# SKA-INAF/caesar-yolo

Measured on AMD Instinct MI355X. Metric: 512x512 tiles/sec over 16k x 16k FITS, higher is better.
Workload: dtype f16

## Files before the change

### caesar_yolo_amd/csrc/conv_igemm.hip

```cpp
#include "cy_kernels.h"
#include <cmath>
#include <cstdlib>
#include <cstring>
#include <vector>

namespace cy {

typedef _Float16 f16;
typedef f16 f16x8 __attribute__((ext_vector_type(8)));
typedef f16 f16x4 __attribute__((ext_vector_type(4)));
typedef float f32x4 __attribute__((ext_vector_type(4)));
typedef unsigned int u32x4 __attribute__((ext_vector_type(4)));
typedef unsigned int u32x2 __attribute__((ext_vector_type(2)));

#define CY_OOB 0xFFFFFF00u
#define CY_WAIT_VM(N) asm volatile("s_waitcnt vmcnt(%0)" ::"n"(N) : "memory")

#ifndef CY_STAMPS_ENABLED
#define CY_STAMPS_ENABLED 0
#endif
__device__ unsigned long long g_stamps[8];
constexpr int WG_STAMP_SLOTS = 4096;
__device__ unsigned long long g_wg_stamps[WG_STAMP_SLOTS * 4];
__device__ __forceinline__ unsigned long long stamp_now() {
// ... 955 lines not shown
            const unsigned off = poff[j] == CY_OOB ? CY_OOB : poff[j] + (unsigned)(ch * 128);
            char* dst = Pbuf + buf * P_BYTES + (wi < NWI ? wi : NWI) * 1024;
            __builtin_amdgcn_raw_ptr_buffer_load_lds(rs0, (lds_void*)dst, 16, off, 0, 0, 0);
        }
    };
    auto dma_w = [&](int n) {
        const int ch = n / 9, tap = n - ch * 9;
#pragma unroll
        for (int j = 0; j < WROUNDS; ++j) {
            const unsigned off = woff[j] + (unsigned)((ch * 9 + tap) * cpad * 128);
            char* dst = Wbuf + (n % RING) * W_BYTES + ((j * NW + wave) % WPIECES) * 1024;
            __builtin_amdgcn_raw_ptr_buffer_load_lds(rsw, (lds_void*)dst, 16, off, 0, 0, 0);
        }
    };

    f32x4 acc[NI][4];
#pragma unroll
    for (int ni = 0; ni < NI; ++ni)
#pragma unroll
        for (int mi = 0; mi < 4; ++mi) acc[ni][mi] = f32x4{0.f, 0.f, 0.f, 0.f};
    const int fr = lane & 15, fq = lane >> 4;
    f16x8 xa0[4], wb0[NI], xa1[4], wb1[NI];

    auto read_frags = [&](const char* P, const char* Wb, int kh, int kw, int kk, f16x8* xa, f16x8* wb) {
        const int qf = fq + 4 * kk;
#pragma unroll
        for (int mi = 0; mi < 4; ++mi) {
            const int r = (wm * 4 + mi + kh) * (TW + 2) + kw + fr;
            xa[mi] = *reinterpret_cast<const f16x8*>(P + r * 128 + ((qf ^ (r & 7)) << 4));
        }
#pragma unroll
        for (int ni = 0; ni < NI; ++ni) {
            const int r = wn * (NI * 16) + ni * 16 + fr;
            wb[ni] = *reinterpret_cast<const f16x8*>(Wb + r * 128 + ((qf ^ (r & 7)) << 4));
        }
    };
    auto mfma_all = [&](const f16x8* xa, const f16x8* wb) {
#pragma unroll
        for (int ni = 0; ni < NI; ++ni)
#pragma unroll
            for (int mi = 0; mi < 4; ++mi)
                acc[ni][mi] = __builtin_amdgcn_mfma_f32_16x16x32_f16(wb[ni], xa[mi], acc[ni][mi], 0, 0, 0);
    };

    dma_patch(0, 0);
    dma_w(0);
    if (total > 1) dma_w(1);
    CY_WAIT_VM(0);
    __builtin_amdgcn_s_barrier();
    if (grp == 1) __builtin_amdgcn_s_barrier();

    int it = 0;
#pragma unroll 1
    for (int ch = 0; ch < chunks; ++ch) {
        const char* P = Pbuf + (ch & 1) * P_BYTES;
#pragma unroll
        for (int tap = 0; tap < 9; ++tap, ++it) {
            const char* Wb = Wbuf + (it % RING) * W_BYTES;
            const int kh = tap / 3, kw = tap - kh * 3;
            const bool pre_p = tap == 1 && ch + 1 < chunks, pre_w = it + 2 < total;
            if (pre_w) dma_w(it + 2);
            if (pre_p) dma_patch((ch + 1) & 1, ch + 1);
            read_frags(P, Wb, kh, kw, 0, xa0, wb0);
            if (pre_p) { CY_WAIT_VM(WROUNDS + PROUNDS); }
            else if (pre_w) { CY_WAIT_VM(WROUNDS); }
            else { CY_WAIT_VM(0); }
            __builtin_amdgcn_sched_barrier(0);
            __builtin_amdgcn_s_barrier();
            read_frags(P, Wb, kh, kw, 1, xa1, wb1);
            __builtin_amdgcn_sched_barrier(0);
            if (a.dbg & 32) __builtin_amdgcn_s_setprio(1);
            mfma_all(xa0, wb0);
            asm volatile("s_waitcnt lgkmcnt(0)" ::: "memory");
            __builtin_amdgcn_sched_barrier(0);
            mfma_all(xa1, wb1);
            if (a.dbg & 32) __builtin_amdgcn_s_setprio(0);
            __builtin_amdgcn_sched_barrier(0);
            __builtin_amdgcn_s_barrier();
        }
    }
    if (grp == 0) __builtin_amdgcn_s_barrier();

    const int cbase = n0 + ((wn * NI) >> 2) * 64 + fq * 16 + ((wn * NI) & 3) * 4;
    float bv[NI * 4];
#pragma unroll
    for (int j = 0; j < NI * 4; ++j) bv[j] = a.bias[cbase + j];
#pragma unroll
    for (int mi = 0; mi < 4; ++mi) {
        const int y = y0 + wm * 4 + mi, x = x0 + fr;
        if (y >= H || x >= W) continue;
        const long pix = ((long)b * H + y) * W + x;
        float v[NI * 4];
#pragma unroll
        for (int ni = 0; ni < NI; ++ni)
#pragma unroll
            for (int j = 0; j < 4; ++j) {
                float t = acc[ni][mi][j] + bv[ni * 4 + j];
                if (a.act) t = silu_fast(t);
                v[ni * 4 + j] = t;
            }
        if (cbase + NI * 4 <= a.Cout) {
            f16* dst = reinterpret_cast<f16*>(a.out) + pix * a.out_ct + a.out_coff + cbase;
            if (a.res) {
                const f16* rp = reinterpret_cast<const f16*>(a.res) + pix * a.res_ct + a.res_coff + cbase;
#pragma unroll
                for (int h8 = 0; h8 < NI / 2; ++h8) {
                    const f16x8 rv = *reinterpret_cast<const f16x8*>(rp + 8 * h8);
#pragma unroll
                    for (int j = 0; j < 8; ++j) v[8 * h8 + j] += (float)rv[j];
                }
            }
#pragma unroll
            for (int h8 = 0; h8 < NI / 2; ++h8) {
                f16x8 o;
#pragma unroll
                for (int j = 0; j < 8; ++j) o[j] = (f16)v[8 * h8 + j];
                *reinterpret_cast<f16x8*>(dst + 8 * h8) = o;
            }
        } else {
#pragma unroll
            for (int j = 0; j < NI * 4; ++j) {
                const int c = cbase + j;
                if (c >= a.Cout) continue;
                float t = v[j];
                if (a.res) t += (float)(reinterpret_cast<const f16*>(a.res)[pix * a.res_ct + a.res_coff + c]);
                reinterpret_cast<f16*>(a.out)[pix * a.out_ct + a.out_coff + c] = (f16)t;
            }
        }
    }
}

template <int NI>
static hipError_t launch_pp(const ConvArgs& a, hipStream_t s) {
    constexpr int BN = 2 * NI * 16, PR = 18 * 18, NWI = (PR + 7) / 8;
    const size_t lds = 2 * (NWI + 1) * 1024 + 4 * BN * 128;
    static bool attr_set = false;
    if (!attr_set) {
        hipFuncSetAttribute(reinterpret_cast<const void*>(conv3x3_pp_kernel<NI>), hipFuncAttributeMaxDynamicSharedMemorySize, (int)lds);
        attr_set = true;
    }
    const int blocks = a.B * ((a.Hi + 15) / 16) * ((a.Wi + 15) / 16) * ((pad64(a.Cout) + BN - 1) / BN);
    hipLaunchKernelGGL((conv3x3_pp_kernel<NI>), dim3(blocks), dim3(512), lds, s, a);
    return hipGetLastError();
}

template <int KC, bool ACT, bool RES>
__global__ __launch_bounds__(512) void conv3x3_c64_kernel(const ConvArgs a) {
    constexpr int TH = 16, TW = 16, NG = 4, NI = 4;
    constexpr int RB = KC * 2, RPP = 1024 / RB, NCH = KC / 8, KK = KC / 32;
    constexpr int PR = (TH + 2) * (TW + 2), NWI = (PR + RPP - 1) / RPP, PROUNDS = (NWI + NG - 1) / NG;
    auto swz = [](int chunk, int row) { return KC == 64 ? (chunk ^ (row & 7)) : (chunk ^ (((row >> 2) & 1) << 1)); };
    constexpr int P_BYTES = (NWI + 1) * 1024;
    extern __shared__ __attribute__((aligned(16))) char smem[];
    typedef __attribute__((address_space(3))) void lds_void;
    const int tid = threadIdx.x, lane = tid & 63;
    const int wave = __builtin_amdgcn_readfirstlane(tid >> 6);
    const int grp = wave >> 2, wm = wave & 3;
    const int fr = lane & 15, fq = lane >> 4;
    const int H = a.Hi, W = a.Wi;
    const int tiles_x = (W + TW - 1) / TW, tiles_y = (H + TH - 1) / TH;
    const int npatch = a.B * tiles_y * tiles_x;
    const unsigned bias_bytes = (unsigned)((W + 1) * a.in0_ct) * 2u;
    const auto rs0 = __builtin_amdgcn_make_buffer_rsrc(const_cast<char*>(reinterpret_cast<const char*>(a.in0)) - bias_bytes, 0,
                                                       a.in0_bytes + 2 * bias_bytes, 0x00020000);

    constexpr int W_BYTES = 9 * 64 * RB, WPIECES = W_BYTES / 1024, PPT = 64 / RPP;
    char* const Wl = smem;
    char* const P = smem + W_BYTES + grp * P_BYTES;
    {
        const auto rsw = KC == 64 ? __builtin_amdgcn_make_buffer_rsrc(const_cast<void*>(a.wgt), 0, a.wgt_bytes, 0x00020000)
                                  : __builtin_amdgcn_make_buffer_rsrc(const_cast<void*>(a.wgt32), 0, a.wgt32_bytes, 0x00020000);
#pragma unroll
        for (int j = 0; j < (WPIECES + 7) / 8; ++j) {
            const int pc = j * 8 + wave;
            if (pc >= WPIECES) break;
            const int tap = pc / PPT, row = (pc % PPT) * RPP + lane / NCH;
            const int q = swz(lane % NCH, row);
            const unsigned off = (unsigned)((tap * 128 + row) * RB + q * 16);
            __builtin_amdgcn_raw_ptr_buffer_load_lds(rsw, (lds_void*)(Wl + pc * 1024), 16, off, 0, 0, 0);
        }
    }
    const int cbase = fq * 16;
    f32x2 bv[8];
#pragma unroll
    for (int j = 0; j < 8; ++j) bv[j] = f32x2{a.bias[cbase + 2 * j], a.bias[cbase + 2 * j + 1]};

    unsigned rel[PROUNDS];
#pragma unroll
    for (int j = 0; j < PROUNDS; ++j) {
        const int wi = j * NG + wm;
        const int r = wi * RPP + lane / NCH;
        const int ry = r / (TW + 2), rx = r - ry * (TW + 2);
        const int q = swz(lane % NCH, r);
        rel[j] = r < PR ? (unsigned)(((ry * W + rx) * a.in0_ct + q * 8) * 2) : CY_OOB;
    }
    const int rlane = lane / NCH;
    auto dma_patch = [&](int pidx) {
        const int tx = pidx % tiles_x, ty = (pidx / tiles_x) % tiles_y, b = pidx / (tiles_x * tiles_y);
        const int y0 = ty * TH, x0 = tx * TW;
        const unsigned so = bias_bytes + (unsigned)((((b * H + y0 - 1) * W + x0 - 1) * a.in0_ct + a.in0_coff) * 2);
        const bool interior = y0 >= 1 && x0 >= 1 && y0 + TH + 1 <= H && x0 + TW + 1 <= W;
        if (interior) {
#pragma unroll
            for (int j = 0; j < PROUNDS; ++j) {
                const int wi = j * NG + wm;
                dma_piece(rs0, (lds_ptr_t*)(P + (wi < NWI ? wi : NWI) * 1024), rel[j], so);
            }
        } else {
            const int ylo = y0 >= 1 ? 0 : 1, yhi = H - y0 + 1, xlo = x0 >= 1 ? 0 : 1, xhi = W - x0 + 1;
#pragma unroll
            for (int j = 0; j < PROUNDS; ++j) {
                const int wi = j * NG + wm;
                const int r = wi * RPP + rlane, ry = (r * 3641) >> 16, rx = r - ry * (TW + 2);
                const bool ok = ry >= ylo && ry < yhi && rx >= xlo && rx < xhi;
                dma_piece(rs0, (lds_ptr_t*)(P + (wi < NWI ? wi : NWI) * 1024), ok ? rel[j] : CY_OOB, so);
            }
        }
    };

    const int NP = (int)blockIdx.x < npatch ? (npatch - 1 - (int)blockIdx.x) / (int)gridDim.x + 1 : 0;
    if (grp < NP) dma_patch(blockIdx.x + grp * gridDim.x);
    __builtin_amdgcn_s_waitcnt(0x0F70);
    __builtin_amdgcn_s_barrier();

    const int R0 = wm * 4 * (TW + 2) + fr;
    unsigned xb[8], wb0[KK];
#pragma unroll
    for (int k8 = 0; k8 < 8; ++k8) xb[k8] = (unsigned)(R0 * RB + (swz(fq, (R0 + k8) & 7) << 4));
#pragma unroll
    for (int kk = 0; kk < KK; ++kk) wb0[kk] = (unsigned)(fr * RB + (swz(fq + 4 * kk, fr) << 4));
    f32x4 acc[NI][4];
    const bool vec_out = cbase + 16 <= a.Cout;
    const int out_lane = fr * a.out_ct + cbase, res_lane = fr * a.res_ct + cbase;
    for (int ph = 0; ph <= NP; ++ph) {
        if ((ph & 1) == grp) {
            if (ph < NP) {
#pragma unroll
                for (int ni = 0; ni < NI; ++ni)
#pragma unroll
                    for (int mi = 0; mi < 4; ++mi) acc[ni][mi] = f32x4{0.f, 0.f, 0.f, 0.f};
                f16x8 xa[2][4], wb[2][NI];
                auto load_group = [&](int g, f16x8* x, f16x8* w) {
                    const int tap = g / KK, kk = g % KK, kh = tap / 3, kw = tap - kh * 3;
#pragma unroll
                    for (int mi = 0; mi < 4; ++mi) {
                        const int c = (mi + kh) * (TW + 2) + kw;
                        x[mi] = *reinterpret_cast<const f16x8*>(P + xb[(c + 4 * kk) & 7] + c * RB);
                    }
#pragma unroll
                    for (int ni = 0; ni < NI; ++ni)
                        w[ni] = *reinterpret_cast<const f16x8*>(Wl + wb0[kk] + (tap * 64 + ni * 16) * RB);
                };
                load_group(0, xa[0], wb[0]);
#pragma unroll
                for (int g = 0; g < 9 * KK; ++g) {
                    if (g + 1 < 9 * KK) load_group(g + 1, xa[(g + 1) & 1], wb[(g + 1) & 1]);
                    __builtin_amdgcn_sched_barrier(0);
#pragma unroll
                    for (int ni = 0; ni < NI; ++ni)
#pragma unroll
                        for (int mi = 0; mi < 4; ++mi)
                            acc[ni][mi] = __builtin_amdgcn_mfma_f32_16x16x32_f16(wb[g & 1][ni], xa[g & 1][mi], acc[ni][mi], 0, 0, 0);
                    __builtin_amdgcn_sched_barrier(0);
                }
                asm volatile("s_waitcnt lgkmcnt(0)" ::: "memory");
            }
        } else if (ph >= 1) {
            f16x8 rres[4][2];
            const int pidx = blockIdx.x + (ph - 1) * gridDim.x;
            const int tx = pidx % tiles_x, ty = (pidx / tiles_x) % tiles_y, b = pidx / (tiles_x * tiles_y);
            const int yw = ty * TH + wm * 4, x = tx * TW + fr;
            const long rowpix = ((long)b * H + yw) * W + tx * TW;
            const bool xok = x < W;
            if (RES) {
#pragma unroll
                for (int mi = 0; mi < 4; ++mi) {
                    const bool ok = yw + mi < H && xok && vec_out;
                    const f16* rp = reinterpret_cast<const f16*>(a.res) + ((rowpix + (yw + mi < H ? (long)mi * W : 0)) * a.res_ct + a.res_coff) + (ok ? res_lane : 0);
                    rres[mi][0] = *reinterpret_cast<const f16x8*>(rp);
                    rres[mi][1] = *reinterpret_cast<const f16x8*>(rp + 8);
                }
            }
            if (ph + 1 < NP) dma_patch(blockIdx.x + (ph + 1) * gridDim.x);
            if (ACT) {
#pragma unroll
                for (int ni = 0; ni < NI; ++ni)
#pragma unroll
                    for (int mi = 0; mi < 4; ++mi)
#pragma unroll
                        for (int h = 0; h < 2; ++h) {
                            f32x2 t = f32x2{acc[ni][mi][2 * h], acc[ni][mi][2 * h + 1]} + bv[ni * 2 + h];
                            f32x2 e = t * f32x2{-1.44269504088896341f, -1.44269504088896341f};
                            e = f32x2{__builtin_amdgcn_exp2f(e[0]), __builtin_amdgcn_exp2f(e[1])} + f32x2{1.0f, 1.0f};
                            t = t * f32x2{__builtin_amdgcn_rcpf(e[0]), __builtin_amdgcn_rcpf(e[1])};
                            acc[ni][mi][2 * h] = t[0]; acc[ni][mi][2 * h + 1] = t[1];
                        }
            } else {
#pragma unroll
                for (int ni = 0; ni < NI; ++ni)
#pragma unroll
                    for (int mi = 0; mi < 4; ++mi)
#pragma unroll
                        for (int j = 0; j < 4; ++j) acc[ni][mi][j] += bv[ni * 2 + (j >> 1)][j & 1];
            }
#pragma unroll
            for (int mi = 0; mi < 4; ++mi) {
                if (yw + mi >= H) break;
                if (!xok) continue;
                if (vec_out) {
                    f16* dst = reinterpret_cast<f16*>(a.out) + ((rowpix + (long)mi * W) * a.out_ct + a.out_coff) + out_lane;
                    float v[16];
#pragma unroll
                    for (int ni = 0; ni < NI; ++ni)
#pragma unroll
                        for (int j = 0; j < 4; ++j) v[ni * 4 + j] = acc[ni][mi][j];
                    if (RES) {
#pragma unroll
                        for (int j = 0; j < 8; ++j) { v[j] += (float)rres[mi][0][j]; v[8 + j] += (float)rres[mi][1][j]; }
                    }
                    f16x8 o0, o1;
#pragma unroll
                    for (int j = 0; j < 8; ++j) { o0[j] = (f16)v[j]; o1[j] = (f16)v[8 + j]; }
                    *reinterpret_cast<f16x8*>(dst) = o0;
                    *reinterpret_cast<f16x8*>(dst + 8) = o1;
                } else {
                    const long pix = rowpix + (long)mi * W + fr;
#pragma unroll
                    for (int j = 0; j < 16; ++j) {
                        const int c = cbase + j;
                        if (c >= a.Cout) continue;
                        float t = acc[j >> 2][mi][j & 3];
                        if (RES) t += (float)(reinterpret_cast<const f16*>(a.res)[pix * a.res_ct + a.res_coff + c]);
                        reinterpret_cast<f16*>(a.out)[pix * a.out_ct + a.out_coff + c] = (f16)t;
                    }
                }
            }
            CY_WAIT_VM(0);
        }
        __builtin_amdgcn_sched_barrier(0);
        __builtin_amdgcn_s_barrier();
        __builtin_amdgcn_sched_barrier(0);
    }
}

template <int KC>
static hipError_t launch_c64(const ConvArgs& a, hipStream_t s) {
    constexpr int RPP = 1024 / (KC * 2), NWI = (18 * 18 + RPP - 1) / RPP;
    const size_t lds = 9 * 64 * KC * 2 + 2 * (NWI + 1) * 1024;
    static bool attr_set = false;
    if (!attr_set) {
        hipFuncSetAttribute(reinterpret_cast<const void*>(conv3x3_c64_kernel<KC, true, false>), hipFuncAttributeMaxDynamicSharedMemorySize, (int)lds);
        hipFuncSetAttribute(reinterpret_cast<const void*>(conv3x3_c64_kernel<KC, true, true>), hipFuncAttributeMaxDynamicSharedMemorySize, (int)lds);
        hipFuncSetAttribute(reinterpret_cast<const void*>(conv3x3_c64_kernel<KC, false, false>), hipFuncAttributeMaxDynamicSharedMemorySize, (int)lds);
        hipFuncSetAttribute(reinterpret_cast<const void*>(conv3x3_c64_kernel<KC, false, true>), hipFuncAttributeMaxDynamicSharedMemorySize, (int)lds);
        attr_set = true;
    }
    const int npatch = a.B * ((a.Hi + 15) / 16) * ((a.Wi + 15) / 16);
    const int grid = npatch < 256 ? npatch : 256;
    if (a.act && a.res) hipLaunchKernelGGL((conv3x3_c64_kernel<KC, true, true>), dim3(grid), dim3(512), lds, s, a);
    else if (a.act) hipLaunchKernelGGL((conv3x3_c64_kernel<KC, true, false>), dim3(grid), dim3(512), lds, s, a);
    else if (a.res) hipLaunchKernelGGL((conv3x3_c64_kernel<KC, false, true>), dim3(grid), dim3(512), lds, s, a);
    else hipLaunchKernelGGL((conv3x3_c64_kernel<KC, false, false>), dim3(grid), dim3(512), lds, s, a);
    return hipGetLastError();
}

__global__ __launch_bounds__(512) void conv3x3_halo2_kernel(const ConvArgs a) {
    constexpr int TH = 16, TW = 16, NW = 8, BN = 128;
    constexpr int PR = (TH + 2) * (TW + 2), NWI = (PR + 7) / 8, PROUNDS = (NWI + NW - 1) / NW;
    constexpr int P_BYTES = PROUNDS * NW * 1024, SLAB = BN * 128, W_BYTES = 2 * SLAB;
    extern __shared__ __attribute__((aligned(16))) char smem[];
    char* const Pbuf = smem;
    char* const Wbuf = smem + 2 * P_BYTES;
    typedef __attribute__((address_space(3))) void lds_void;
    const int tid = threadIdx.x, lane = tid & 63;
    const int wave = __builtin_amdgcn_readfirstlane(tid >> 6);
    const int wm = wave >> 1, wn = wave & 1;
    const int H = a.Hi, W = a.Wi;
    const int tiles_x = (W + TW - 1) / TW, tiles_y = (H + TH - 1) / TH;
    const int cpad = pad128(a.Cout);
    const int ntn = (pad64(a.Cout) + BN - 1) / BN;
    const int id = xcd_remap(blockIdx.x, gridDim.x);
    const int nt = id % ntn;
    int rest = id / ntn;
    const int tx = rest % tiles_x; rest /= tiles_x;
    const int ty = rest % tiles_y;
    const int b = rest / tiles_y;
    const int y0 = ty * TH, x0 = tx * TW, n0 = nt * BN;
    const int chunks = a.Cin / 64, pairs = chunks / 2;

    const auto rs0 = __builtin_amdgcn_make_buffer_rsrc(const_cast<void*>(a.in0), 0, a.in0_bytes, 0x00020000);
    const auto rsw = __builtin_amdgcn_make_buffer_rsrc(const_cast<void*>(a.wgt), 0, a.wgt_bytes, 0x00020000);
    unsigned poff[PROUNDS];
#pragma unroll
    for (int j = 0; j < PROUNDS; ++j) {
        const int r = (j * NW + wave) * 8 + (lane >> 3);
        const int ry = r / (TW + 2), rx = r - ry * (TW + 2);
        const int y = y0 + ry - 1, x = x0 + rx - 1;
        const int q = (lane & 7) ^ (r & 7);
        const bool ok = r < PR && (unsigned)y < (unsigned)H && (unsigned)x < (unsigned)W;
        poff[j] = ok ? (unsigned)(((b * H + y) * W + x) * a.in0_ct + a.in0_coff + q * 8) * 2u : CY_OOB;
    }
    unsigned woff[2];
#pragma unroll
    for (int j = 0; j < 2; ++j) {
        const int row = (j * NW + wave) * 8 + (lane >> 3);
        woff[j] = (unsigned)((n0 + row) * 128 + ((lane & 7) ^ (row & 7)) * 16);
    }
    auto dma_patch = [&](int buf, int ch) {
#pragma unroll
        for (int j = 0; j < PROUNDS; ++j) {
            __builtin_amdgcn_raw_ptr_buffer_load_lds(rs0, (lds_void*)(Pbuf + buf * P_BYTES + (j * NW + wave) * 1024), 16, poff[j], ch * 128, 0, 0);
        }
    };
    auto dma_slab = [&](int buf, int t, int ch, int tap) {
#pragma unroll
        for (int j = 0; j < 2; ++j) {
            __builtin_amdgcn_raw_ptr_buffer_load_lds(rsw, (lds_void*)(Wbuf + buf * W_BYTES + t * SLAB + (j * NW + wave) * 1024), 16, woff[j], (ch * 9 + tap) * cpad * 128, 0, 0);
        }
    };
    f32x4 acc[4][4];
#pragma unroll
    for (int ni = 0; ni < 4; ++ni)
#pragma unroll
        for (int mi = 0; mi < 4; ++mi) acc[ni][mi] = f32x4{0.f, 0.f, 0.f, 0.f};
    const int fr = lane & 15, fq = lane >> 4;
    auto compute = [&](const char* P, const char* Wb, int kh, int kw) {
#pragma unroll
        for (int kk = 0; kk < 2; ++kk) {
            const int qf = fq + 4 * kk;
            f16x8 xa[4], wb[4];
#pragma unroll
            for (int mi = 0; mi < 4; ++mi) {
                const int r = (wm * 4 + mi + kh) * (TW + 2) + kw + fr;
                xa[mi] = *reinterpret_cast<const f16x8*>(P + r * 128 + ((qf ^ (r & 7)) << 4));
            }
#pragma unroll
            for (int ni = 0; ni < 4; ++ni) {
                const int r = wn * 64 + ni * 16 + fr;
                wb[ni] = *reinterpret_cast<const f16x8*>(Wb + r * 128 + ((qf ^ (r & 7)) << 4));
            }
#pragma unroll
            for (int ni = 0; ni < 4; ++ni)
#pragma unroll
                for (int mi = 0; mi < 4; ++mi)
                    acc[ni][mi] = __builtin_amdgcn_mfma_f32_16x16x32_f16(wb[ni], xa[mi], acc[ni][mi], 0, 0, 0);
        }
    };

    dma_patch(0, 0);
    dma_slab(0, 0, 0, 0);
    dma_slab(0, 1, 0, 1);
    __syncthreads();
    int g = 0;
    const bool stamps = CY_STAMPS_ENABLED && (a.dbg & 64) != 0;
    unsigned long long acc_dma = 0, acc_cmp = 0, acc_wait = 0, acc_bar = 0;
    const unsigned long long t_begin = stamps ? stamp_now() : 0;
    unsigned long long t0s = t_begin;
#pragma unroll 1
    for (int cp = 0; cp < pairs; ++cp) {
#pragma unroll
        for (int st = 0; st < 9; ++st, ++g) {
            if (st < 8) {
                const int u0 = 2 * (st + 1), u1 = u0 + 1;
                dma_slab((g + 1) & 1, 0, 2 * cp + u0 / 9, u0 % 9);
                dma_slab((g + 1) & 1, 1, 2 * cp + u1 / 9, u1 % 9);
            } else if (cp + 1 < pairs) {
                dma_slab((g + 1) & 1, 0, 2 * cp + 2, 0);
                dma_slab((g + 1) & 1, 1, 2 * cp + 2, 1);
            }
            if (st == 0) dma_patch(1, 2 * cp + 1);
            if (st == 5 && cp + 1 < pairs) dma_patch(0, 2 * cp + 2);
            unsigned long long t1 = 0, t2 = 0, t3 = 0;
            if (stamps) { __builtin_amdgcn_sched_barrier(0); t1 = stamp_now(); __builtin_amdgcn_sched_barrier(0); }
#pragma unroll
            for (int t = 0; t < 2; ++t) {
                const int u = 2 * st + t, tap = u % 9;
                compute(Pbuf + (u / 9) * P_BYTES, Wbuf + (g & 1) * W_BYTES + t * SLAB, tap / 3, tap % 3);
            }
            if (stamps) {
                asm volatile("s_waitcnt lgkmcnt(0)" ::: "memory");
                __builtin_amdgcn_sched_barrier(0); t2 = stamp_now(); __builtin_amdgcn_sched_barrier(0);
                CY_WAIT_VM(0);
                __builtin_amdgcn_sched_barrier(0); t3 = stamp_now(); __builtin_amdgcn_sched_barrier(0);
            }
            __syncthreads();
            if (stamps) {
                __builtin_amdgcn_sched_barrier(0);
                const unsigned long long t4 = stamp_now();
                acc_dma += t1 - t0s; acc_cmp += t2 - t1; acc_wait += t3 - t2; acc_bar += t4 - t3;
                t0s = t4;
            }
        }
    }

    if (stamps && lane == 0) {
        const unsigned long long t_end = stamp_now();
        atomicAdd(&g_stamps[0], acc_dma); atomicAdd(&g_stamps[1], acc_cmp); atomicAdd(&g_stamps[2], acc_wait);
        atomicAdd(&g_stamps[3], acc_bar); atomicAdd(&g_stamps[4], t_end - t_begin); atomicAdd(&g_stamps[5], (unsigned long long)(pairs * 9));
        atomicAdd(&g_stamps[6], 1ull);
    }
    const int cbase = n0 + wn * 64 + fq * 16;
    float bv[16];
#pragma unroll
    for (int j = 0; j < 16; ++j) bv[j] = a.bias[cbase + j];
#pragma unroll
    for (int mi = 0; mi < 4; ++mi) {
        const int y = y0 + wm * 4 + mi, x = x0 + fr;
        if (y >= H || x >= W) continue;
        const long pix = ((long)b * H + y) * W + x;
// ... 293 lines not shown
    for (int mi = 0; mi < MIW; ++mi) {
        const int y = y0 + wm * RPW + (mi >> 1), x = DUAL ? fr : x0 + (mi & 1) * 16 + fr;
        const int bb = DUAL ? 2 * b + (mi & 1) : b;
        if (y >= H || x >= W || bb >= a.B) continue;
        const long pix = ((long)bb * H + y) * W + x;
        float v[16];
        bias_act16(acc[0][mi], acc[1][mi], acc[2][mi], acc[3][mi], bv, a.act != 0, v);
        if (cbase + 16 <= a.Cout) {
            f16* dst = reinterpret_cast<f16*>(a.out) + pix * a.out_ct + a.out_coff + cbase;
            if (res_vec) {
#pragma unroll
                for (int j = 0; j < 8; ++j) { v[j] += (float)rv[mi][0][j]; v[8 + j] += (float)rv[mi][1][j]; }
            }
            f16x8 o0, o1;
#pragma unroll
            for (int j = 0; j < 8; ++j) { o0[j] = (f16)v[j]; o1[j] = (f16)v[8 + j]; }
            *reinterpret_cast<f16x8*>(dst) = o0;
            *reinterpret_cast<f16x8*>(dst + 8) = o1;
        } else {
#pragma unroll
            for (int j = 0; j < 16; ++j) {
                const int c = cbase + j;
                if (c >= a.Cout) continue;
                float t = v[j];
                if (a.res) t += (float)(reinterpret_cast<const f16*>(a.res)[pix * a.res_ct + a.res_coff + c]);
                reinterpret_cast<f16*>(a.out)[pix * a.out_ct + a.out_coff + c] = (f16)t;
            }
        }
    }
    }
    if (stamps) {
        const unsigned long long t_st = stamp_real();
        asm volatile("s_waitcnt vmcnt(0)" ::: "memory");
        const unsigned long long t_end = stamp_real();
        if (tid == 0) {
            unsigned long long* rec = g_wg_stamps + (size_t)(blockIdx.x % WG_STAMP_SLOTS) * 4;
            rec[0] = t_loop - t_entry; rec[1] = t_epi - t_loop; rec[2] = t_st - t_epi; rec[3] = c_epi - c_loop;
        }
    }
}

template <int WN, bool DUAL = false, bool SPLIT = false>
static hipError_t launch_wide(const ConvArgs& a, hipStream_t s) {
    constexpr int PR = 18 * (DUAL ? 36 : 34), NPC = (PR + 15) / 16, PROUNDS = (NPC + 7) / 8, BN = 64 * WN;
    const size_t lds = 2 * PROUNDS * 8 * 1024 + 3 * 2 * BN * 64 + 1024;
    static bool attr_set = false;
    if (!attr_set) {
        hipFuncSetAttribute(reinterpret_cast<const void*>(conv3x3_wide_kernel<true, WN, DUAL, 2, SPLIT>), hipFuncAttributeMaxDynamicSharedMemorySize, (int)lds);
        attr_set = true;
    }
    const int bx = DUAL ? (a.B + 1) / 2 : a.B * ((a.Wi + 31) / 32);
    const int blocks = bx * ((a.Hi + 15) / 16) * ((pad64(a.Cout) + BN - 1) / BN);
    hipLaunchKernelGGL((conv3x3_wide_kernel<true, WN, DUAL, 2, SPLIT>), dim3(blocks), dim3(512), lds, s, a);
    return hipGetLastError();
}

struct StripGeo { int RS, IS, NE; unsigned long long mRS, mIS; };
__device__ __forceinline__ int strip_div(int e, unsigned long long m) { return (int)(((unsigned long long)(unsigned)e * m) >> 40); }

template <bool SPLIT, bool RES, int STRIP = 0>
__global__ __launch_bounds__(512) void conv3x3_widep_kernel(const ConvArgs a, const int total, const StripGeo sg) {
    constexpr int NST = 9, TH = 16, TW = 32, NW = 8, BN = 128, PWID = TW + 2;
    constexpr int NDW = 4;
    constexpr int RPW = 4, MIW = 8, WPS = 2 * (NW / NDW);
    constexpr int PR = (TH + 2) * PWID, NPC = (PR + 15) / 16, PROUNDS = STRIP ? STRIP : (NPC + NDW - 1) / NDW;
    constexpr int P_BYTES = PROUNDS * NDW * 1024, SLAB = BN * 64, W_BYTES = 2 * SLAB, RING = 3;
    extern __shared__ __attribute__((aligned(16))) char smem[];
    char* const Pbuf = smem;
    char* const Wbuf = smem + 2 * P_BYTES;
    const int tid = threadIdx.x, lane = tid & 63;
    const int wave = __builtin_amdgcn_readfirstlane(tid >> 6);
    const int wm = wave >> 1, wn = wave & 1;
    const int H = a.Hi, W = a.Wi;
    const int tiles_x = (W + TW - 1) / TW, tiles_y = (H + TH - 1) / TH;
    const int cpad = pad128(a.Cout);
    const int ntn = (pad64(a.Cout) + BN - 1) / BN;
    const int ppairs = a.Cin / 64;
    const int pairs = SPLIT ? a.split * ppairs : ppairs;
    const auto rs0 = __builtin_amdgcn_make_buffer_rsrc(const_cast<void*>(a.in0), 0, a.in0_bytes, 0x00020000);
    const auto rsw = __builtin_amdgcn_make_buffer_rsrc(const_cast<void*>(a.wgt32), 0, a.wgt32_bytes, 0x00020000);
    const auto rsb = __builtin_amdgcn_make_buffer_rsrc(const_cast<float*>(a.bias), 0, (unsigned)pad64(a.Cout) * 4u, 0x00020000);
    const auto rss = __builtin_amdgcn_make_buffer_rsrc(const_cast<float*>(SPLIT ? a.oscale : a.bias), 0, (unsigned)pad64(a.Cout) * 4u, 0x00020000);
    const unsigned out_bytes = (unsigned)((long)a.B * H * W * a.out_ct * 2);
    const auto rso = __builtin_amdgcn_make_buffer_rsrc(a.out, 0, out_bytes, 0x00020000);
    const auto rsr = __builtin_amdgcn_make_buffer_rsrc(const_cast<void*>(RES ? a.res : a.in0), 0,
                                                       RES ? (unsigned)((long)a.B * H * W * a.res_ct * 2) : 0u, 0x00020000);
    const int fr = lane & 15, fq = lane >> 4;

    int pb_, py0, px0, pn0;
    auto geometry = [&](int v) {
        const int id = xcd_remap(v, total);
        pn0 = (id % ntn) * BN;
        int rest = id / ntn;
        if constexpr (STRIP != 0) { px0 = rest * 512; py0 = 0; pb_ = 0; return; }
        px0 = (rest % tiles_x) * TW; rest /= tiles_x;
        py0 = (rest % tiles_y) * TH;
        pb_ = rest / tiles_y;
    };
    const bool no_dma = CY_STAMPS_ENABLED && (a.dbg & 1), no_rd = CY_STAMPS_ENABLED && (a.dbg & 2), no_mma = CY_STAMPS_ENABLED && (a.dbg & 4);
    const bool dmaw = wave < NDW && !no_dma;
    auto dma_patch = [&](int buf, int slab, int gb, int gy0, int gx0) {
        if (!dmaw) return;
        int l4 = lane >> 2;
        asm volatile("" : "+v"(l4));
        const unsigned lq = (unsigned)(lane & 3);
        unsigned slab_so = (unsigned)slab * 64u;
        if constexpr (SPLIT) {
            int lo;
            slab_so = (unsigned)x3_chunk(slab, 2 * ppairs, lo) * 64u;
            if (lo) slab_so += (unsigned)a.in0_lo * 2u;
        }
        if constexpr (STRIP != 0) {
            const int hl = 514 + 2 * sg.RS;
#pragma unroll
            for (int j = 0; j < PROUNDS; ++j) {
                const int le = (j * NDW + wave) * 16 + l4;
                const int e = gx0 - sg.RS - 1 + le;
                const bool in = le < hl && (unsigned)e < (unsigned)sg.NE;
                const int ec = in ? e : 0;
                const int bb = strip_div(ec, sg.mIS), r = ec - bb * sg.IS;
                const int y = strip_div(r, sg.mRS), x = r - y * sg.RS;
                const unsigned q = lq ^ (unsigned)(((le >> 2) & 1) << 1);
                const bool ok = in && y < H && x < W;
                const unsigned off = ok ? (unsigned)(((bb * H + y) * W + x) * a.in0_ct + a.in0_coff + (int)q * 8) * 2u : CY_OOB;
                dma_piece(rs0, (lds_ptr_t*)(Pbuf + buf * P_BYTES + (j * NDW + wave) * 1024), off, slab_so);
            }
            return;
        }
#pragma unroll
        for (int j = 0; j < PROUNDS; ++j) {
            const int r = (j * NDW + wave) * 16 + l4;
            const int ry = (r * 1928) >> 16, rx = r - ry * PWID;
            const int y = gy0 + ry - 1, x = gx0 + rx - 1;
            const unsigned q = lq ^ (unsigned)(((r >> 2) & 1) << 1);
            const bool ok = r < PR && (unsigned)y < (unsigned)H && (unsigned)x < (unsigned)W;
            const unsigned off = ok ? (unsigned)(((gb * H + y) * W + x) * a.in0_ct + a.in0_coff + (int)q * 8) * 2u : CY_OOB;
            dma_piece(rs0, (lds_ptr_t*)(Pbuf + buf * P_BYTES + (j * NDW + wave) * 1024), off, slab_so);
        }
    };
    unsigned woff = 0;
    auto weight_lane_offset = [&]() { const int row = wave * 32 + (lane >> 2); woff = (unsigned)(row * 64 + ((lane & 3) ^ (((row >> 2) & 1) << 1)) * 16); };
    auto dma_stage = [&](int ring, int slab0, int u0, int n0) {
        if (!dmaw) return;
#pragma unroll
        for (int t = 0; t < 2; ++t) {
            const int u = u0 + t, sl = slab0 + u / 9, tap = u % 9;
#pragma unroll
            for (int h = 0; h < 2; ++h)
                dma_piece(rsw, (lds_ptr_t*)(Wbuf + ring * W_BYTES + t * SLAB + (wave * 2 + h) * 1024), woff,
                          (unsigned)((sl * 9 + tap) * cpad * 64 + n0 * 64 + h * 1024));
        }
    };
    float* const bias_lds = reinterpret_cast<float*>(smem + 2 * P_BYTES + RING * W_BYTES);
    auto dma_bias = [&](int slot, int n0) {
        if (wave != 0) return;
        dma_piece(rsb, (lds_ptr_t*)(bias_lds + slot * 512), lane * 16 < BN * 4 ? (unsigned)(n0 * 4 + lane * 16) : CY_OOB, 0);
        if constexpr (SPLIT) dma_piece(rss, (lds_ptr_t*)(bias_lds + slot * 512 + 256), lane * 16 < BN * 4 ? (unsigned)(n0 * 4 + lane * 16) : CY_OOB, 0);
    };

    f32x4 acc[4][MIW];
    unsigned pb[STRIP ? 9 : 8], wl = 0;
    const int rw0 = wm * RPW * PWID;
    auto fragment_bases = [&]() {
        int lz = lane;
        asm volatile("" : "+v"(lz));
        const int r_ = lz & 15, q_ = lz >> 4;
        if constexpr (STRIP != 0) {
#pragma unroll
            for (int t = 0; t < 9; ++t) {
                const int R0 = (t / 3) * sg.RS + (t % 3) + wm * 128 + r_;
                pb[t] = (unsigned)(R0 * 64 + ((q_ ^ (((R0 >> 2) & 1) << 1)) << 4));
            }
        } else {
#pragma unroll
            for (int c = 0; c < 8; ++c)
                pb[c] = (unsigned)(rw0 * 64 + r_ * 64 + ((q_ ^ ((((c + r_ + (rw0 & 7)) >> 2) & 1) << 1)) << 4));
        }
        wl = (unsigned)(2 * P_BYTES + (wn * 64 + r_) * 64 + ((q_ ^ (((r_ >> 2) & 1) << 1)) << 4));
    };
    f16x8 xa[2][4], wb[2][4];
    auto load_x = [&](f16x8* dst, int pbuf_off, int kh, int kw, int half) {
        if (no_rd) return;
#pragma unroll
        for (int m = 0; m < 4; ++m) {
            const int mi = half * 4 + m;
            if constexpr (STRIP != 0) {
                dst[m] = *reinterpret_cast<const f16x8*>(smem + pb[kh * 3 + kw] + (pbuf_off + mi * 1024));
            } else {
                const int base = ((mi >> 1) + kh) * PWID + (mi & 1) * 16 + kw;
                dst[m] = *reinterpret_cast<const f16x8*>(smem + pb[base & 7] + (pbuf_off + base * 64));
            }
        }
    };
    auto load_w = [&](f16x8* dst, int wbuf_off) {
        if (no_rd) return;
#pragma unroll
        for (int ni = 0; ni < 4; ++ni) dst[ni] = *reinterpret_cast<const f16x8*>(smem + wl + (wbuf_off + ni * 1024));
    };
    auto mma = [&](const f16x8* w, const f16x8* x, int half) {
        if (no_mma) return;
#pragma unroll
        for (int ni = 0; ni < 4; ++ni)
#pragma unroll
            for (int m = 0; m < 4; ++m)
                acc[ni][half * 4 + m] = __builtin_amdgcn_mfma_f32_16x16x32_f16(w[ni], x[m], acc[ni][half * 4 + m], 0, 0, 0);
    };
    auto stage_compute = [&](int st) {
        const int u0 = 2 * st, u1 = u0 + 1, t0 = u0 % 9, t1 = u1 % 9;
        const int p0 = (u0 / 9) * P_BYTES, p1 = (u1 / 9) * P_BYTES, w0 = (st % 3) * W_BYTES, w1 = w0 + SLAB;
        load_w(wb[0], w0);
        load_x(xa[0], p0, t0 / 3, t0 % 3, 0);
        load_x(xa[1], p0, t0 / 3, t0 % 3, 1);
        mma(wb[0], xa[0], 0);
        __builtin_amdgcn_sched_barrier(0);
        load_w(wb[1], w1);
        load_x(xa[0], p1, t1 / 3, t1 % 3, 0);
        mma(wb[0], xa[1], 1);
        __builtin_amdgcn_sched_barrier(0);
        load_x(xa[1], p1, t1 / 3, t1 % 3, 1);
        mma(wb[1], xa[0], 0);
        __builtin_amdgcn_sched_barrier(0);
    };

    const bool stamps = CY_STAMPS_ENABLED && (a.dbg & 64) != 0;
    unsigned long long t_l0 = 0, t_l1 = 0, t_rw = 0, t_ep = 0;
    const unsigned long long t_begin = stamps ? stamp_real() : 0;
    int v = blockIdx.x, n = 0;
    if (v >= total) return;
    geometry(v);
    weight_lane_offset();
    dma_bias(0, pn0);
    dma_patch(0, 0, pb_, py0, px0);
    dma_stage(0, 0, 0, pn0);
    dma_stage(1, 0, 2, pn0);
    CY_WAIT_VM(WPS);
    __builtin_amdgcn_s_barrier();
#pragma unroll 1
    for (;;) {
        const int b = pb_, y0 = py0, x0 = px0, n0 = pn0;
        const int vn = v + (int)gridDim.x;
        const bool next = vn < total;
        if (stamps) {
            const unsigned long long t = stamp_real();
            if (n == 2 && tid == 0) {
                unsigned long long* rec = g_wg_stamps + (size_t)(blockIdx.x % WG_STAMP_SLOTS) * 4;
                rec[0] = t_rw - t_l1; rec[1] = t_l1 - t_l0; rec[2] = t_ep - t_rw;
            }
            t_l0 = t;
        }
        fragment_bases();
#pragma unroll
        for (int ni = 0; ni < 4; ++ni)
#pragma unroll
            for (int mi = 0; mi < MIW; ++mi) acc[ni][mi] = f32x4{0.f, 0.f, 0.f, 0.f};
#pragma unroll 1
        for (int cp = 0; cp < pairs; ++cp) {
            const bool more = cp + 1 < pairs;
            const bool chain = more || next;
#pragma unroll
            for (int st = 0; st < NST; ++st) {
                const bool has_w = st + 2 < NST || chain;
                if (st + 2 < NST) dma_stage((st + 2) % 3, 2 * cp, 2 * (st + 2), n0);
                else if (more) dma_stage((st + 2) % 3, 2 * cp + 2, 2 * (st + 2 - NST), n0);
                else if (next) dma_stage((st + 2) % 3, 0, 2 * (st + 2 - NST), pn0);
                if (st == 0) dma_patch(1, 2 * cp + 1, b, y0, x0);
                if (st == 1 && !more && next) { geometry(vn); dma_bias((n + 1) & 1, pn0); }
                if (st == 5 && more) dma_patch(0, 2 * cp + 2, b, y0, x0);
                if (st == 5 && !more && next) dma_patch(0, 0, pb_, py0, px0);
                stage_compute(st);
                asm volatile("s_waitcnt lgkmcnt(0)" ::: "memory");
                if (st == 0 || st == 1) { CY_WAIT_VM(WPS + PROUNDS); }
                else if (st == 5 || st == 6) { if (chain) { CY_WAIT_VM(WPS + PROUNDS); } else { CY_WAIT_VM(WPS); } }
                else if (has_w) { CY_WAIT_VM(WPS); }
                else { CY_WAIT_VM(0); }
                __builtin_amdgcn_sched_barrier(0);
                __builtin_amdgcn_s_barrier();
                __builtin_amdgcn_sched_barrier(0);
                mma(wb[1], xa[1], 1);
            }
        }
        if (stamps) t_l1 = stamp_real();
        const float* bl = bias_lds + (n & 1) * 512 + wn * 64 + fq * 16;
        float bv[16];
        if constexpr (!SPLIT) {
#pragma unroll
            for (int j = 0; j < 4; ++j) {
                const f32x4 t = *reinterpret_cast<const f32x4*>(bl + j * 4);
                bv[j * 4] = t[0]; bv[j * 4 + 1] = t[1]; bv[j * 4 + 2] = t[2]; bv[j * 4 + 3] = t[3];
            }
        }
        const int cbase = n0 + wn * 64 + fq * 16;
        const bool chan_ok = cbase + 16 <= a.Cout;
        const int xl = x0 + fr;
        const unsigned pix0 = (unsigned)((b * H + y0 + wm * RPW) * W + xl);
        const bool okx0 = xl < W && chan_ok, okx1 = xl + 16 < W && chan_ok;
        const unsigned cb2 = (unsigned)cbase * 2u;
        const int e0 = x0 + wm * 128 + fr;
        auto pixel = [&](int mi, unsigned& pix) -> bool {
            if constexpr (STRIP != 0) {
                const int e = e0 + 16 * mi;
                const int ec = e < sg.NE ? e : 0;
                const int bb = strip_div(ec, sg.mIS), r = ec - bb * sg.IS;
                const int yy = strip_div(r, sg.mRS), xx = r - yy * sg.RS;
                pix = (unsigned)((bb * H + yy) * W + xx);
                return e < sg.NE && yy < H && xx < W && chan_ok;
            } else {
                pix = pix0 + (unsigned)((mi >> 1) * W + (mi & 1) * 16);
                return (y0 + wm * RPW + (mi >> 1) < H) && ((mi & 1) ? okx1 : okx0);
            }
        };
        if constexpr (SPLIT) {
            f16x8 rq[3][4];
            auto res_load = [&](int mi) {
                unsigned pix;
                const bool ok = pixel(mi, pix);
                const unsigned ro = ok ? (pix * (unsigned)a.res_ct + (unsigned)a.res_coff) * 2u + cb2 : CY_OOB;
                rq[mi % 3][0] = __builtin_bit_cast(f16x8, load_b128(rsr, ro, 0));
                rq[mi % 3][1] = __builtin_bit_cast(f16x8, load_b128(rsr, ro, 16));
                rq[mi % 3][2] = __builtin_bit_cast(f16x8, load_b128(rsr, ro, a.res_lo * 2));
                rq[mi % 3][3] = __builtin_bit_cast(f16x8, load_b128(rsr, ro, a.res_lo * 2 + 16));
            };
            if (RES) { res_load(0); res_load(1); }
            if (stamps) t_rw = stamp_real();
#pragma unroll
            for (int mi = 0; mi < MIW; ++mi) {
                if (RES && mi + 2 < MIW) res_load(mi + 2);
                float bg[16], sc[16];
#pragma unroll
                for (int j = 0; j < 4; ++j) {
                    const f32x4 t = *reinterpret_cast<const f32x4*>(bl + j * 4), u = *reinterpret_cast<const f32x4*>(bl + 256 + j * 4);
                    bg[j * 4] = t[0]; bg[j * 4 + 1] = t[1]; bg[j * 4 + 2] = t[2]; bg[j * 4 + 3] = t[3];
                    sc[j * 4] = u[0]; sc[j * 4 + 1] = u[1]; sc[j * 4 + 2] = u[2]; sc[j * 4 + 3] = u[3];
                }
                float vv[16];
                scale_bias_act16(acc[0][mi], acc[1][mi], acc[2][mi], acc[3][mi], bg, sc, a.act != 0, vv);
                if (RES) {
#pragma unroll
                    for (int j = 0; j < 8; ++j) {
                        vv[j] += (float)rq[mi % 3][0][j] + (float)rq[mi % 3][2][j];
                        vv[8 + j] += (float)rq[mi % 3][1][j] + (float)rq[mi % 3][3][j];
                    }
                }
                f16x8 h0, h1, l0, l1;
#pragma unroll
                for (int j = 0; j < 8; ++j) {
                    h0[j] = (f16)vv[j]; h1[j] = (f16)vv[8 + j];
                    l0[j] = (f16)(vv[j] - (float)h0[j]); l1[j] = (f16)(vv[8 + j] - (float)h1[j]);
                }
                unsigned pix;
                const bool ok = pixel(mi, pix);
                const unsigned so = ok ? (pix * (unsigned)a.out_ct + (unsigned)a.out_coff) * 2u + cb2 : CY_OOB;
                __builtin_amdgcn_raw_buffer_store_b128(__builtin_bit_cast(u32x4, h0), rso, so, 0, 0);
                __builtin_amdgcn_raw_buffer_store_b128(__builtin_bit_cast(u32x4, h1), rso, so, 16, 0);
                __builtin_amdgcn_raw_buffer_store_b128(__builtin_bit_cast(u32x4, l0), rso, so, a.out_lo * 2, 0);
                __builtin_amdgcn_raw_buffer_store_b128(__builtin_bit_cast(u32x4, l1), rso, so, a.out_lo * 2 + 16, 0);
            }
        } else {
        f16x8 rv[MIW][2];
        if (RES) {
#pragma unroll
            for (int mi = 0; mi < MIW; ++mi) {
                unsigned pix;
                const bool ok = pixel(mi, pix);
                const unsigned ro = ok ? (pix * (unsigned)a.res_ct + (unsigned)a.res_coff) * 2u + cb2 : CY_OOB;
                rv[mi][0] = __builtin_bit_cast(f16x8, load_b128(rsr, ro, 0));
                rv[mi][1] = __builtin_bit_cast(f16x8, load_b128(rsr, ro, 16));
            }
            CY_WAIT_VM(0);
        }
        if (stamps) t_rw = stamp_real();
#pragma unroll
        for (int mi = 0; mi < MIW; ++mi) {
            float vv[16];
            bias_act16(acc[0][mi], acc[1][mi], acc[2][mi], acc[3][mi], bv, a.act != 0, vv);
            if (RES) {
#pragma unroll
                for (int j = 0; j < 8; ++j) { vv[j] += (float)rv[mi][0][j]; vv[8 + j] += (float)rv[mi][1][j]; }
            }
            f16x8 o0, o1;
#pragma unroll
            for (int j = 0; j < 8; ++j) { o0[j] = (f16)vv[j]; o1[j] = (f16)vv[8 + j]; }
            unsigned pix;
            const bool ok = pixel(mi, pix);
            const unsigned so = ok ? (pix * (unsigned)a.out_ct + (unsigned)a.out_coff) * 2u + cb2 : CY_OOB;
            __builtin_amdgcn_raw_buffer_store_b128(__builtin_bit_cast(u32x4, o0), rso, so, 0, 0);
            __builtin_amdgcn_raw_buffer_store_b128(__builtin_bit_cast(u32x4, o1), rso, so, 16, 0);
        }
        }
        if (stamps) t_ep = stamp_real();
        if (stamps && !next && tid == 0) g_wg_stamps[(size_t)(blockIdx.x % WG_STAMP_SLOTS) * 4 + 3] = t_ep - t_begin;
        if (!next) break;
        v = vn; ++n;
    }
}

template <int STRIP, bool SPLIT = false>
static hipError_t launch_widep_t(const ConvArgs& a, hipStream_t s, int total, const StripGeo& sg) {
    constexpr int PR = 18 * 34, NPC = (PR + 15) / 16, PROUNDS = STRIP ? STRIP : (NPC + 3) / 4;
    const size_t lds = 2 * PROUNDS * 4 * 1024 + 3 * 2 * 128 * 64 + 4096;
    static bool attr_set = false;
    if (!attr_set) {
        hipFuncSetAttribute(reinterpret_cast<const void*>(conv3x3_widep_kernel<SPLIT, false, STRIP>), hipFuncAttributeMaxDynamicSharedMemorySize, (int)lds);
        hipFuncSetAttribute(reinterpret_cast<const void*>(conv3x3_widep_kernel<SPLIT, true, STRIP>), hipFuncAttributeMaxDynamicSharedMemorySize, (int)lds);
        attr_set = true;
    }
    static const int ncu = [] { int dev = 0, n = 256; hipGetDevice(&dev); hipDeviceGetAttribute(&n, hipDeviceAttributeMultiprocessorCount, dev); return n > 0 ? n : 256; }();
    const int grid = total < ncu ? total : ncu;
    if (a.res) hipLaunchKernelGGL((conv3x3_widep_kernel<SPLIT, true, STRIP>), dim3(grid), dim3(512), lds, s, a, total, sg);
    else hipLaunchKernelGGL((conv3x3_widep_kernel<SPLIT, false, STRIP>), dim3(grid), dim3(512), lds, s, a, total, sg);
    return hipGetLastError();
}

static hipError_t launch_widep(const ConvArgs& a, hipStream_t s) {
    const int total = a.B * ((a.Wi + 31) / 32) * ((a.Hi + 15) / 16) * ((pad64(a.Cout) + 127) / 128);
    return a.split ? launch_widep_t<0, true>(a, s, total, StripGeo{}) : launch_widep_t<0>(a, s, total, StripGeo{});
}

static double wide2d_cover(int H, int W) { return (double)((H + 15) / 16 * 16) * ((W + 31) / 32 * 32) / ((double)H * W); }
static double strip_cover(int H, int W) { return (double)(H + 1) * (W + 1) / ((double)H * W); }
static bool strip_small(const ConvArgs& a) { return a.Wi >= 3 && a.Wi <= 12 && a.Hi >= 3 && a.Hi <= 126; }
static bool strip_fits(const ConvArgs& a) {
    return ((a.Wi >= 17 && a.Hi >= 17 && a.Wi <= 126) || strip_small(a)) && a.Cout % 16 == 0 && (long)a.B * (a.Hi + 1) * (a.Wi + 1) < (1L << 22);
}

static hipError_t launch_strip(const ConvArgs& a, hipStream_t s) {
    StripGeo sg;
    sg.RS = a.Wi + 1; sg.IS = (a.Hi + 1) * sg.RS; sg.NE = a.B * sg.IS;
    sg.mRS = ((1ull << 40) + sg.RS - 1) / sg.RS; sg.mIS = ((1ull << 40) + sg.IS - 1) / sg.IS;
    const int total = ((sg.NE + 511) / 512) * ((pad64(a.Cout) + 127) / 128);
    if (a.split) return a.Wi <= 62 ? launch_widep_t<10, true>(a, s, total, sg) : launch_widep_t<12, true>(a, s, total, sg);
    return a.Wi <= 62 ? launch_widep_t<10>(a, s, total, sg) : launch_widep_t<12>(a, s, total, sg);
}

template <int NB, int MI, int RING, bool K3, bool SPLIT = false, int NDW = 8, bool FUSE2 = false>
__global__ __launch_bounds__(512, (NB * MI <= 4 && RING == 2) ? 2 : 1) void conv1x1_direct_kernel(const ConvArgs a) {
    static_assert(!FUSE2 || (NB == 4 && !SPLIT), "back-to-back fusion: 256-channel tile, fp16 context");
    constexpr int NW = 8, BN = 64 * NB, BM = NW * MI * 16, W_BYTES = BN * 128, DIST = RING - 1;
    constexpr int WPW = BN / 8 / NDW, APW = 2 * MI, PER = WPW + APW;
    extern __shared__ __attribute__((aligned(16))) char smem[];
    const bool stamps = CY_STAMPS_ENABLED && (a.dbg & 64) != 0;
    const unsigned long long t_entry = stamps ? stamp_real() : 0;
    typedef __attribute__((address_space(3))) void lds_void;
    const int tid = threadIdx.x, lane = tid & 63;
    const int wave = __builtin_amdgcn_readfirstlane(tid >> 6);
    const int fr = lane & 15, fq = lane >> 4;
    const int HoWo = a.Ho * a.Wo, M = a.B * HoWo;
    const int cpad = pad128(a.Cout);
    const int ntn = (pad64(a.Cout) + BN - 1) / BN;
    const int id = xcd_remap(blockIdx.x, gridDim.x);
    const int m0 = (id / ntn) * BM, n0 = (id % ntn) * BN;
    constexpr int taps = K3 ? 9 : 1, pad = K3 ? 1 : 0, kk3 = K3 ? 3 : 1;
    const int pchunks = (a.Cin / 64) * taps, c0chunks = a.c1 ? a.c0 / 64 : pchunks;
    const int chunks = SPLIT ? a.split * pchunks : pchunks;
    const unsigned bias_bytes = K3 ? (unsigned)((a.Wi + 1) * a.in0_ct) * 2u : 0u;

    const auto rs0 = __builtin_amdgcn_make_buffer_rsrc(const_cast<char*>(reinterpret_cast<const char*>(a.in0)) - bias_bytes, 0,
                                                       a.in0_bytes + 2 * bias_bytes, 0x00020000);
    const auto rs1 = __builtin_amdgcn_make_buffer_rsrc(const_cast<void*>(a.c1 ? a.in1 : a.in0), 0,
                                                       a.c1 ? a.in1_bytes : a.in0_bytes, 0x00020000);
    const auto rsw = __builtin_amdgcn_make_buffer_rsrc(const_cast<void*>(a.wgt), 0, a.wgt_bytes, 0x00020000);
    unsigned v0[MI], v1[MI], vmask[MI];
#pragma unroll
    for (int mi = 0; mi < MI; ++mi) {
        const int m = m0 + (wave * MI + mi) * 16 + fr;
        v0[mi] = v1[mi] = CY_OOB;
        vmask[mi] = 0;
        if (m < M) {
            const int b = m / HoWo, r = m - b * HoWo, ho = r / a.Wo, wo = r - ho * a.Wo;
            int p0;
            if (a.up0) p0 = (b * (a.Hi >> 1) + (ho >> 1)) * (a.Wi >> 1) + (wo >> 1);
            else p0 = (b * a.Hi + ho * a.s) * a.Wi + wo * a.s;
            v0[mi] = (unsigned)(p0 * a.in0_ct + a.in0_coff + fq * 8) * 2u;
            v1[mi] = (unsigned)(m * a.in1_ct + a.in1_coff + fq * 8) * 2u;
            unsigned vm = 0;
#pragma unroll
            for (int kh = 0; kh < kk3; ++kh)
#pragma unroll
                for (int kw = 0; kw < kk3; ++kw)
                    if ((unsigned)(ho * a.s + kh - pad) < (unsigned)a.Hi && (unsigned)(wo * a.s + kw - pad) < (unsigned)a.Wi)
                        vm |= 1u << (kh * kk3 + kw);
            vmask[mi] = vm;
        }
    }
    const bool no_dma = CY_STAMPS_ENABLED && (a.dbg & 1), no_rd = CY_STAMPS_ENABLED && (a.dbg & 2), no_mma = CY_STAMPS_ENABLED && (a.dbg & 4),
               no_px = CY_STAMPS_ENABLED && (a.dbg & 8);
    const bool reqw = wave < NDW;
    const unsigned woff0 = (unsigned)((n0 + wave * 8 + (lane >> 3)) * 128 + ((lane & 7) ^ (lane >> 3)) * 16);
    u32x4 xa[RING][MI][2];
    int ltap = 0, lslab = 0;
    auto load_a = [&](int slot, int cv) {
        if (no_px) return;
        int lo = 0;
        const int c = SPLIT ? x3_chunk(cv, pchunks, lo) : cv;
        const unsigned lo0 = SPLIT && lo ? (unsigned)a.in0_lo * 2u : 0u, lo1 = SPLIT && lo ? (unsigned)a.in1_lo * 2u : 0u;
        if (c >= c0chunks) {
#pragma unroll
            for (int mi = 0; mi < MI; ++mi)
#pragma unroll
                for (int kk = 0; kk < 2; ++kk)
                    xa[slot][mi][kk] = load_b128(rs1, v1[mi], ((c - c0chunks) * 64 + kk * 32) * 2 + lo1);
        } else if constexpr (!K3) {
#pragma unroll
            for (int mi = 0; mi < MI; ++mi)
#pragma unroll
                for (int kk = 0; kk < 2; ++kk)
                    xa[slot][mi][kk] = load_b128(rs0, v0[mi], (c * 64 + kk * 32) * 2 + lo0);
        } else {
            const int kh = ltap / 3, kw = ltap - kh * 3;
            const unsigned so = bias_bytes + (unsigned)((((kh - 1) * a.Wi + (kw - 1)) * a.in0_ct + lslab * 64) * 2) + lo0;
#pragma unroll
            for (int mi = 0; mi < MI; ++mi) {
                const unsigned vo = ((vmask[mi] >> ltap) & 1u) ? v0[mi] : CY_OOB;
#pragma unroll
                for (int kk = 0; kk < 2; ++kk) xa[slot][mi][kk] = load_b128(rs0, vo, so + kk * 64);
            }
            if (++ltap == 9) { ltap = 0; ++lslab; if (SPLIT && lslab * 9 == pchunks) lslab = 0; }
        }
    };
    auto dma_w = [&](int slot, int c) {
        if ((NDW < NW && !reqw) || no_dma) return;
#pragma unroll
        for (int j = 0; j < WPW; ++j)
            dma_piece(rsw, (lds_ptr_t*)(smem + slot * W_BYTES + (j * NDW + wave) * 1024), woff0, c * cpad * 128 + j * NDW * 1024);
    };
    auto wait_w = [&](int n) {
        if (NDW < NW && !reqw) return;
        if (n == APW + 2 * PER) { CY_WAIT_VM(APW + 2 * PER); }
        else if (n == APW + PER) { CY_WAIT_VM(APW + PER); }
        else { CY_WAIT_VM(APW); }
    };
    f32x4 acc[NB * 4][MI];
#pragma unroll
    for (int ni = 0; ni < NB * 4; ++ni)
#pragma unroll
        for (int mi = 0; mi < MI; ++mi) acc[ni][mi] = f32x4{0.f, 0.f, 0.f, 0.f};
    auto compute_x = [&](int slot, const u32x4 (&xs)[MI][2]) {
        const char* Wb = smem + slot * W_BYTES;
        f16x8 wb[2][4];
        auto load_wb = [&](f16x8* dst, int gi) {
            if (no_rd) return;
            const int kk = gi / NB, g = gi % NB, qf = fq + 4 * kk;
#pragma unroll
            for (int ni = 0; ni < 4; ++ni) {
                const int r = g * 64 + ni * 16 + fr;
                dst[ni] = *reinterpret_cast<const f16x8*>(Wb + r * 128 + ((qf ^ (r & 7)) << 4));
            }
        };
        load_wb(wb[0], 0);
#pragma unroll
        for (int gi = 0; gi < 2 * NB; ++gi) {
            const int kk = gi / NB, g = gi % NB;
            if (gi + 1 < 2 * NB) load_wb(wb[(gi + 1) & 1], gi + 1);
// ... 767 lines not shown
            if (n < cout && k < 27) { const int tap = k / 3, c = k % 3; v = W[((size_t)n * 3 + c) * 9 + tap]; }
            o[row * 32 + k] = (f16)v;
        }
    }
}

constexpr int SD_TH = 8, SD_TW = 32, SD_PH = 2 * SD_TH + 1, SD_PW = 2 * SD_TW + 1, SD_EVEN = SD_TW + 1;
constexpr int SD_ROWS = SD_PH * SD_PW, SD_FRAGS = (SD_ROWS + 15) / 16, SD_LDS = SD_FRAGS * 16 * 128;

__device__ __forceinline__ u32x2 load_b64(__amdgpu_buffer_rsrc_t rs, unsigned voff) {
    return __builtin_amdgcn_raw_buffer_load_b64(rs, voff, 0, 0);
}

__global__ __launch_bounds__(512) void stem_down_kernel(const StemDownArgs a) {
    extern __shared__ __attribute__((aligned(16))) char smem[];
    const int tid = threadIdx.x, lane = tid & 63, fr = lane & 15, fq = lane >> 4;
    const int wave = __builtin_amdgcn_readfirstlane(tid >> 6);
    const int wn = wave & 1, wm = wave >> 1;
    const int tiles_x = (a.Wo + SD_TW - 1) / SD_TW, tiles_y = (a.Ho + SD_TH - 1) / SD_TH;
    int id = xcd_remap(blockIdx.x, gridDim.x);
    const int tx = id % tiles_x; id /= tiles_x;
    const int ty = id % tiles_y;
    const int b = id / tiles_y;
    const int oy0 = ty * SD_TH, ox0 = tx * SD_TW;
    const int sy0 = 2 * oy0 - 1, sx0 = 2 * ox0 - 1;
    const auto rsi = __builtin_amdgcn_make_buffer_rsrc(const_cast<void*>(a.in), 0, a.in_bytes, 0x00020000);
    const auto rsw = __builtin_amdgcn_make_buffer_rsrc(const_cast<void*>(a.wgt32), 0, a.wgt32_bytes, 0x00020000);

    constexpr int SD_RING = 4;
    f16x8 wa[SD_RING][4];
    const unsigned wl = (unsigned)((wn * 64 + fr) * 64 + fq * 16);
    auto load_wa = [&](f16x8* dst, int step) {
        const int h = step & 1, tap = step >> 1;
#pragma unroll
        for (int ni = 0; ni < 4; ++ni) dst[ni] = __builtin_bit_cast(f16x8, load_b128(rsw, wl + ni * 1024, (h * 9 + tap) * 8192));
    };
#pragma unroll
    for (int st = 0; st < SD_RING - 1; ++st) load_wa(wa[st], st);

    if (!(a.dbg & 1)) {
        const f16* wp = reinterpret_cast<const f16*>(a.wpk2);
        f16x8 sw0[4], sw1[4];
#pragma unroll
        for (int ni = 0; ni < 4; ++ni) {
            sw0[ni] = *reinterpret_cast<const f16x8*>(wp + (ni * 16 + fr) * 64 + fq * 8);
            sw1[ni] = *reinterpret_cast<const f16x8*>(wp + (ni * 16 + fr) * 64 + 32 + fq * 8);
        }
        float bv[16];
#pragma unroll
        for (int j = 0; j < 16; ++j) bv[j] = a.bias0[fq * 16 + j];
        const int t0 = 2 * fq, t1 = 2 * fq + 1;
        const int dh0 = t0 / 3 - 1, dw0 = t0 % 3 - 1, dh1 = t1 / 3 - 1, dw1 = t1 % 3 - 1;
        const int d0 = (dh0 * a.Wi + dw0) * 8, d1 = (dh1 * a.Wi + dw1) * 8, d2 = (a.Wi + 1) * 8;
        constexpr int NG = (SD_FRAGS + 7) / 8;
        u32x2 q0[NG], q1[NG], q2[NG];
        unsigned inmask = 0;
#pragma unroll
        for (int gi = 0; gi < NG; ++gi) {
            const int g = gi * 8 + wave, p = g * 16 + fr;
            const int sy = p / SD_PW, q = p - sy * SD_PW;
            const int sx = q < SD_EVEN ? 2 * q : 2 * (q - SD_EVEN) + 1;
            const int Y = sy0 + sy, X = sx0 + sx;
            const bool inmap = p < SD_ROWS && (unsigned)Y < (unsigned)a.H1 && (unsigned)X < (unsigned)a.W1;
            inmask |= inmap ? (1u << gi) : 0u;
            const int hc = 2 * Y, wc = 2 * X;
            const int base = ((b * a.Hi + hc) * a.Wi + wc) * 8;
            const bool ok0 = inmap && ((hc + dh0) | (wc + dw0)) >= 0, ok1 = inmap && ((hc + dh1) | (wc + dw1)) >= 0;
            q0[gi] = load_b64(rsi, ok0 ? (unsigned)(base + d0) : CY_OOB);
            q1[gi] = load_b64(rsi, ok1 ? (unsigned)(base + d1) : CY_OOB);
            q2[gi] = load_b64(rsi, (inmap && fq == 0) ? (unsigned)(base + d2) : CY_OOB);
        }
#pragma unroll
        for (int gi = 0; gi < NG; ++gi) {
            const int g = gi * 8 + wave;
            if (g >= SD_FRAGS) break;
            const int p = g * 16 + fr;
            const bool inmap = (inmask >> gi) & 1u;
            const u32x4 u0 = {q0[gi].x, q0[gi].y & 0xFFFFu, q1[gi].x, q1[gi].y & 0xFFFFu};
            const u32x4 u1 = {q2[gi].x, q2[gi].y & 0xFFFFu, 0u, 0u};
            const f16x8 x0 = __builtin_bit_cast(f16x8, u0), x1 = __builtin_bit_cast(f16x8, u1);
            f32x4 acc[4];
#pragma unroll
            for (int ni = 0; ni < 4; ++ni) {
                acc[ni] = __builtin_amdgcn_mfma_f32_16x16x32_f16(sw0[ni], x0, f32x4{0.f, 0.f, 0.f, 0.f}, 0, 0, 0);
                acc[ni] = __builtin_amdgcn_mfma_f32_16x16x32_f16(sw1[ni], x1, acc[ni], 0, 0, 0);
            }
            f16x8 o0, o1;
            float v16[16];
            bias_act16(acc[0], acc[1], acc[2], acc[3], bv, true, v16);
#pragma unroll
            for (int j = 0; j < 8; ++j) { o0[j] = (f16)v16[j]; o1[j] = (f16)v16[8 + j]; }
            const unsigned keep = inmap ? 0xFFFFFFFFu : 0u;
            const u32x4 k4 = {keep, keep, keep, keep};
            char* row = smem + p * 128;
            *reinterpret_cast<u32x4*>(row + (((2 * fq) ^ (p & 7)) << 4)) = __builtin_bit_cast(u32x4, o0) & k4;
            *reinterpret_cast<u32x4*>(row + (((2 * fq + 1) ^ (p & 7)) << 4)) = __builtin_bit_cast(u32x4, o1) & k4;
        }
    }
    __syncthreads();

    f32x4 acc[4][4];
#pragma unroll
    for (int ni = 0; ni < 4; ++ni)
#pragma unroll
        for (int m = 0; m < 4; ++m) acc[ni][m] = f32x4{0.f, 0.f, 0.f, 0.f};
    const int pl = wm * 4 * SD_PW + fr;
    if (!(a.dbg & 2))
#pragma unroll
    for (int step = 0; step < 18; ++step) {
        const int tap = step >> 1, h = step & 1, kh = tap / 3, kw = tap % 3;
        if (step + SD_RING - 1 < 18) load_wa(wa[(step + SD_RING - 1) % SD_RING], step + SD_RING - 1);
        __builtin_amdgcn_sched_barrier(0);
        f16x8 xb[4];
#pragma unroll
        for (int m = 0; m < 4; ++m) {
            const int cm = (2 * (m >> 1) + kh) * SD_PW + (m & 1) * 16 + (kw == 1 ? SD_EVEN : (kw == 2 ? 1 : 0));
            const int p = pl + cm;
            xb[m] = *reinterpret_cast<const f16x8*>(smem + p * 128 + (((h * 4 + fq) ^ (p & 7)) << 4));
        }
#pragma unroll
        for (int ni = 0; ni < 4; ++ni)
#pragma unroll
            for (int m = 0; m < 4; ++m)
                acc[ni][m] = __builtin_amdgcn_mfma_f32_16x16x32_f16(wa[step % SD_RING][ni], xb[m], acc[ni][m], 0, 0, 0);
        __builtin_amdgcn_sched_barrier(0);
    }

    const int cbase = wn * 64 + fq * 16;
    float bv[16];
#pragma unroll
    for (int j = 0; j < 16; ++j) bv[j] = a.bias1[cbase + j];
#pragma unroll
    for (int m = 0; m < 4; ++m) {
        const int oy = oy0 + wm * 2 + (m >> 1), ox = ox0 + (m & 1) * 16 + fr;
        if (oy >= a.Ho || ox >= a.Wo || (a.dbg & 4)) continue;
        const long pix = ((long)b * a.Ho + oy) * a.Wo + ox;
        f16x8 o0, o1;
        float v16[16];
        bias_act16(acc[0][m], acc[1][m], acc[2][m], acc[3][m], bv, true, v16);
#pragma unroll
        for (int j = 0; j < 8; ++j) { o0[j] = (f16)v16[j]; o1[j] = (f16)v16[8 + j]; }
        f16* dst = reinterpret_cast<f16*>(a.out) + pix * a.out_ct + a.out_coff + cbase;
        *reinterpret_cast<f16x8*>(dst) = o0;
        *reinterpret_cast<f16x8*>(dst + 8) = o1;
    }
}

constexpr int S2_TH = 8, S2_TW = 16, S2_PH = 2 * S2_TH + 1, S2_PW = 2 * S2_TW + 1, S2_EVEN = S2_TW + 1;
constexpr int S2_ROWS = S2_PH * S2_PW, S2_FRAGS = (S2_ROWS + 15) / 16, S2_BUF = S2_FRAGS * 16 * 128, S2_LDS = 2 * S2_BUF;
static_assert(S2_FRAGS % 4 == 0, "fragments split evenly over the four waves of a group");

__global__ __launch_bounds__(512) void stem_down2_kernel(const StemDownArgs a) {
    extern __shared__ __attribute__((aligned(16))) char smem[];
    const int tid = threadIdx.x, lane = tid & 63, fr = lane & 15, fq = lane >> 4;
    const int wave = __builtin_amdgcn_readfirstlane(tid >> 6);
    const int grp = wave >> 2, w4 = wave & 3, wn = w4 & 1, wm = w4 >> 1;
    char* const buf = smem + grp * S2_BUF;
    const int tiles_x = (a.Wo + S2_TW - 1) / S2_TW, tiles_y = (a.Ho + S2_TH - 1) / S2_TH;
    const int npatch = a.B * tiles_y * tiles_x;
    const int NP = (int)blockIdx.x < npatch ? (npatch - 1 - (int)blockIdx.x) / (int)gridDim.x + 1 : 0;
    const auto rsi = __builtin_amdgcn_make_buffer_rsrc(const_cast<void*>(a.in), 0, a.in_bytes, 0x00020000);
    const auto rsw = __builtin_amdgcn_make_buffer_rsrc(const_cast<void*>(a.wgt32), 0, a.wgt32_bytes, 0x00020000);

    constexpr int RING = 4;
    f16x8 wa[RING][2];
    const unsigned wl = (unsigned)((w4 * 32 + fr) * 64 + fq * 16);
    auto load_wa = [&](f16x8* dst, int step) {
        const int h = step & 1, tap = step >> 1;
#pragma unroll
        for (int ni = 0; ni < 2; ++ni) dst[ni] = __builtin_bit_cast(f16x8, load_b128(rsw, wl + ni * 1024, (h * 9 + tap) * 8192));
    };
    const f16* wp = reinterpret_cast<const f16*>(a.wpk2);
    const int t0 = 2 * fq, t1 = 2 * fq + 1;
    const int dh0 = t0 / 3 - 1, dw0 = t0 % 3 - 1, dh1 = t1 / 3 - 1, dw1 = t1 % 3 - 1;
    const int d0 = (dh0 * a.Wi + dw0) * 8, d1 = (dh1 * a.Wi + dw1) * 8, d2 = (a.Wi + 1) * 8;

    auto coords = [&](int n, int& b, int& oy0, int& ox0) {
        int id = (int)blockIdx.x + n * (int)gridDim.x;
        const int tx = id % tiles_x; id /= tiles_x;
        oy0 = (id % tiles_y) * S2_TH; ox0 = tx * S2_TW; b = id / tiles_y;
    };

    auto fill = [&](int n) {
        int b, oy0, ox0;
        coords(n, b, oy0, ox0);
        const int sy0 = 2 * oy0 - 1, sx0 = 2 * ox0 - 1;
        f16x8 sw0[4], sw1[4];
#pragma unroll
        for (int ni = 0; ni < 4; ++ni) {
            sw0[ni] = *reinterpret_cast<const f16x8*>(wp + (ni * 16 + fr) * 64 + fq * 8);
            sw1[ni] = *reinterpret_cast<const f16x8*>(wp + (ni * 16 + fr) * 64 + 32 + fq * 8);
        }
        float bv0[16];
#pragma unroll
        for (int j = 0; j < 16; ++j) bv0[j] = a.bias0[fq * 16 + j];
        constexpr int NG = S2_FRAGS / 4;
        u32x2 q0[NG], q1[NG], q2[NG];
        unsigned inmask = 0;
#pragma unroll
        for (int gi = 0; gi < NG; ++gi) {
            const int g = gi * 4 + w4, p = g * 16 + fr;
            const int sy = p / S2_PW, q = p - sy * S2_PW;
            const int sx = q < S2_EVEN ? 2 * q : 2 * (q - S2_EVEN) + 1;
            const int Y = sy0 + sy, X = sx0 + sx;
            const bool inmap = p < S2_ROWS && (unsigned)Y < (unsigned)a.H1 && (unsigned)X < (unsigned)a.W1;
            inmask |= inmap ? (1u << gi) : 0u;
            const int hc = 2 * Y, wc = 2 * X;
            const int base = ((b * a.Hi + hc) * a.Wi + wc) * 8;
            const bool ok0 = inmap && ((hc + dh0) | (wc + dw0)) >= 0, ok1 = inmap && ((hc + dh1) | (wc + dw1)) >= 0;
            q0[gi] = load_b64(rsi, ok0 ? (unsigned)(base + d0) : CY_OOB);
            q1[gi] = load_b64(rsi, ok1 ? (unsigned)(base + d1) : CY_OOB);
            q2[gi] = load_b64(rsi, (inmap && fq == 0) ? (unsigned)(base + d2) : CY_OOB);
        }
#pragma unroll
        for (int gi = 0; gi < NG; ++gi) {
            const int g = gi * 4 + w4, p = g * 16 + fr;
            const bool inmap = (inmask >> gi) & 1u;
            const u32x4 u0 = {q0[gi].x, q0[gi].y & 0xFFFFu, q1[gi].x, q1[gi].y & 0xFFFFu};
            const u32x4 u1 = {q2[gi].x, q2[gi].y & 0xFFFFu, 0u, 0u};
            const f16x8 x0 = __builtin_bit_cast(f16x8, u0), x1 = __builtin_bit_cast(f16x8, u1);
            f32x4 acc[4];
#pragma unroll
            for (int ni = 0; ni < 4; ++ni) {
                acc[ni] = __builtin_amdgcn_mfma_f32_16x16x32_f16(sw0[ni], x0, f32x4{0.f, 0.f, 0.f, 0.f}, 0, 0, 0);
                acc[ni] = __builtin_amdgcn_mfma_f32_16x16x32_f16(sw1[ni], x1, acc[ni], 0, 0, 0);
            }
            f16x8 o0, o1;
            float v16[16];
            bias_act16(acc[0], acc[1], acc[2], acc[3], bv0, true, v16);
#pragma unroll
            for (int j = 0; j < 8; ++j) { o0[j] = (f16)v16[j]; o1[j] = (f16)v16[8 + j]; }
            const unsigned keep = inmap ? 0xFFFFFFFFu : 0u;
            const u32x4 k4 = {keep, keep, keep, keep};
            char* row = buf + p * 128;
            *reinterpret_cast<u32x4*>(row + (((2 * fq) ^ (p & 7)) << 4)) = __builtin_bit_cast(u32x4, o0) & k4;
            *reinterpret_cast<u32x4*>(row + (((2 * fq + 1) ^ (p & 7)) << 4)) = __builtin_bit_cast(u32x4, o1) & k4;
        }
#pragma unroll
        for (int st = 0; st < RING - 1; ++st) load_wa(wa[st], st);
    };

    auto conv_store = [&](int n) {
        int b, oy0, ox0;
        coords(n, b, oy0, ox0);
        f32x4 acc[2][8];
#pragma unroll
        for (int ni = 0; ni < 2; ++ni)
#pragma unroll
            for (int m = 0; m < 8; ++m) acc[ni][m] = f32x4{0.f, 0.f, 0.f, 0.f};
        unsigned xrow[8];
#pragma unroll
        for (int c = 0; c < 8; ++c) xrow[c] = (unsigned)(fr * 128 + ((fq ^ ((fr + c) & 7)) << 4));
#pragma unroll
        for (int step = 0; step < 18; ++step) {
            const int tap = step >> 1, h = step & 1, kh = tap / 3, kw = tap % 3;
            if (step + RING - 1 < 18) load_wa(wa[(step + RING - 1) % RING], step + RING - 1);
            __builtin_amdgcn_sched_barrier(0);
#pragma unroll
            for (int mh = 0; mh < 2; ++mh) {
                f16x8 xb[4];
#pragma unroll
                for (int m4 = 0; m4 < 4; ++m4) {
                    const int m = mh * 4 + m4;
                    const int cm = (2 * m + kh) * S2_PW + (kw == 1 ? S2_EVEN : (kw == 2 ? 1 : 0));
                    xb[m4] = *reinterpret_cast<const f16x8*>(buf + ((xrow[cm & 7] ^ (unsigned)(h * 64)) + cm * 128));
                }
#pragma unroll
                for (int ni = 0; ni < 2; ++ni)
#pragma unroll
                    for (int m4 = 0; m4 < 4; ++m4)
                        acc[ni][mh * 4 + m4] = __builtin_amdgcn_mfma_f32_16x16x32_f16(wa[step % RING][ni], xb[m4], acc[ni][mh * 4 + m4], 0, 0, 0);
                __builtin_amdgcn_sched_barrier(0);
            }
        }
        const int cbase = (w4 >> 1) * 64 + fq * 16 + (w4 & 1) * 8;
        f32x2 bv[4];
#pragma unroll
        for (int j = 0; j < 4; ++j) bv[j] = f32x2{a.bias1[cbase + 2 * j], a.bias1[cbase + 2 * j + 1]};
#pragma unroll
        for (int m = 0; m < 8; ++m) {
            const int oy = oy0 + m, ox = ox0 + fr;
            if (oy >= a.Ho || ox >= a.Wo) continue;
            const long pix = ((long)b * a.Ho + oy) * a.Wo + ox;
            f16x8 o;
#pragma unroll
            for (int ni = 0; ni < 2; ++ni)
#pragma unroll
                for (int hh = 0; hh < 2; ++hh) {
                    f32x2 t = f32x2{acc[ni][m][2 * hh], acc[ni][m][2 * hh + 1]} + bv[ni * 2 + hh];
                    f32x2 e = t * f32x2{-1.44269504088896341f, -1.44269504088896341f};
                    e = f32x2{__builtin_amdgcn_exp2f(e[0]), __builtin_amdgcn_exp2f(e[1])} + f32x2{1.0f, 1.0f};
                    t = t * f32x2{__builtin_amdgcn_rcpf(e[0]), __builtin_amdgcn_rcpf(e[1])};
                    o[ni * 4 + 2 * hh] = (f16)t[0]; o[ni * 4 + 2 * hh + 1] = (f16)t[1];
                }
            *reinterpret_cast<f16x8*>(reinterpret_cast<f16*>(a.out) + pix * a.out_ct + a.out_coff + cbase) = o;
        }
    };

    auto phase_barrier = [&]() {
        __builtin_amdgcn_sched_barrier(0);
        __syncthreads();
        __builtin_amdgcn_sched_barrier(0);
    };
    if (grp) phase_barrier();
#pragma unroll 1
    for (int n = grp; n < NP; n += 2) {
        fill(n);
        phase_barrier();
        conv_store(n);
        phase_barrier();
    }
    if (((NP + grp) & 1) == 0) phase_barrier();
}

long stem_down_blocks(const StemDownArgs& a) {
    return (long)a.B * ((a.Ho + SD_TH - 1) / SD_TH) * ((a.Wo + SD_TW - 1) / SD_TW);
}

hipError_t launch_stem_down(const StemDownArgs& a, hipStream_t s) {
    if (a.Hi != 2 * a.H1 || a.Wi != 2 * a.W1) return hipErrorInvalidValue;
    static bool attr_set = false;
    if (!attr_set) {
        hipFuncSetAttribute(reinterpret_cast<const void*>(stem_down_kernel), hipFuncAttributeMaxDynamicSharedMemorySize, SD_LDS);
        attr_set = true;
    }
    StemDownArgs b2 = a; b2.dbg = dev_knob("CY_SD_DBG", 0);
    const int v = env_knob("CY_STEM_V", 0);
    const long np = (long)a.B * ((a.Ho + S2_TH - 1) / S2_TH) * ((a.Wo + S2_TW - 1) / S2_TW);
    if (v == 2 || (v == 0 && np >= 512)) {
        static bool set2 = false;
        if (!set2) { hipFuncSetAttribute(reinterpret_cast<const void*>(stem_down2_kernel), hipFuncAttributeMaxDynamicSharedMemorySize, S2_LDS); set2 = true; }
        hipLaunchKernelGGL(stem_down2_kernel, dim3((unsigned)(np < 256 ? np : 256)), dim3(512), S2_LDS, s, b2);
        return hipGetLastError();
    }
    hipLaunchKernelGGL(stem_down_kernel, dim3((unsigned)stem_down_blocks(a)), dim3(512), SD_LDS, s, b2);
    return hipGetLastError();
}

void pack_stem_weights2(const float* W, int cout, void* dst) {
    f16* o = reinterpret_cast<f16*>(dst);
    for (int row = 0; row < 64; ++row) {
        const int ni = (row >> 4) & 3, rr = row & 15;
        const int n = (rr >> 2) * 16 + ni * 4 + (rr & 3);
        for (int k = 0; k < 64; ++k) {
            const int tap = k < 32 ? k / 4 : 8, c = k < 32 ? k % 4 : k - 32;
            float v = 0.0f;
            if (n < cout && c < 3 && k < 36) v = W[((size_t)n * 3 + c) * 9 + tap];
            o[row * 64 + k] = (f16)v;
        }
    }
}

template <typename T>
__global__ __launch_bounds__(256) void pool5_kernel(const PoolArgs a) {
    constexpr int V = 16 / sizeof(T);
    typedef T vec __attribute__((ext_vector_type(V)));
    const int cv = a.C / V;
    const long total = (long)a.B * a.H * a.W * cv;
    for (long idx = (long)xcd_contiguous(blockIdx.x, gridDim.x) * 256 + threadIdx.x; idx < total; idx += (long)gridDim.x * 256) {
        const int c = (int)(idx % cv) * V;
        const long pix = idx / cv;
        const int w = (int)(pix % a.W), h = (int)((pix / a.W) % a.H), b = (int)(pix / ((long)a.W * a.H));
        const T* base = reinterpret_cast<const T*>(a.src) + a.src_coff + c;
        vec m = *reinterpret_cast<const vec*>(base + (((long)b * a.H + h) * a.W + w) * a.ct);
#pragma unroll
        for (int dh = -2; dh <= 2; ++dh) {
            int hh = h + dh;
            hh = hh < 0 ? 0 : (hh >= a.H ? a.H - 1 : hh);
#pragma unroll
            for (int dw = -2; dw <= 2; ++dw) {
                if (dh == 0 && dw == 0) continue;
                int ww = w + dw;
                ww = ww < 0 ? 0 : (ww >= a.W ? a.W - 1 : ww);
                const vec v = *reinterpret_cast<const vec*>(base + (((long)b * a.H + hh) * a.W + ww) * a.ct);
#pragma unroll
                for (int j = 0; j < V; ++j) m[j] = v[j] > m[j] ? v[j] : m[j];
            }
        }
        *reinterpret_cast<vec*>(reinterpret_cast<T*>(a.dst) + pix * a.ct + a.dst_coff + c) = m;
    }
}

__global__ __launch_bounds__(256) void pool5_x3_kernel(const PoolArgs a) {
    const int cv = a.C / 8;
    const long total = (long)a.B * a.H * a.W * cv;
    for (long idx = (long)xcd_contiguous(blockIdx.x, gridDim.x) * 256 + threadIdx.x; idx < total; idx += (long)gridDim.x * 256) {
        const int c = (int)(idx % cv) * 8;
        const long pix = idx / cv;
        const int w = (int)(pix % a.W), h = (int)((pix / a.W) % a.H), b = (int)(pix / ((long)a.W * a.H));
        float m[8]; f16x8 mh, ml;
        bool first = true;
        for (int dh = -2; dh <= 2; ++dh)
            for (int dw = -2; dw <= 2; ++dw) {
                const int hh = h + dh, ww = w + dw;
                if ((unsigned)hh >= (unsigned)a.H || (unsigned)ww >= (unsigned)a.W) continue;
                const f16* sp = reinterpret_cast<const f16*>(a.src) + (((long)b * a.H + hh) * a.W + ww) * a.ct + a.src_coff + c;
                const f16x8 vh = *reinterpret_cast<const f16x8*>(sp), vl = *reinterpret_cast<const f16x8*>(sp + a.lo);
#pragma unroll
                for (int j = 0; j < 8; ++j) {
                    const float v = (float)vh[j] + (float)vl[j];
                    if (first || v > m[j]) { m[j] = v; mh[j] = vh[j]; ml[j] = vl[j]; }
                }
                first = false;
            }
        f16* dp = reinterpret_cast<f16*>(a.dst) + pix * a.ct + a.dst_coff + c;
        *reinterpret_cast<f16x8*>(dp) = mh;
        *reinterpret_cast<f16x8*>(dp + a.lo) = ml;
    }
}

hipError_t launch_pool5(Precision p, const PoolArgs& a, hipStream_t s) {
    if (p == PREC_F16X3) {
        if (a.C % 8 || a.lo <= 0) return hipErrorInvalidValue;
        const long total = (long)a.B * a.H * a.W * (a.C / 8);
        hipLaunchKernelGGL(pool5_x3_kernel, dim3((unsigned)((total + 255) / 256)), dim3(256), 0, s, a);
        return hipGetLastError();
    }
    const int V = p == PREC_F16 ? 8 : 4;
    if (a.C % V) return hipErrorInvalidValue;
    const long total = (long)a.B * a.H * a.W * (a.C / V);
    const int grid = (int)((total + 255) / 256);
    if (p == PREC_F16) hipLaunchKernelGGL(pool5_kernel<f16>, dim3(grid), dim3(256), 0, s, a);
    else hipLaunchKernelGGL(pool5_kernel<float>, dim3(grid), dim3(256), 0, s, a);
    return hipGetLastError();
}

}
```

### caesar_yolo_amd/csrc/cy_kernels.h

```cpp
#pragma once
#include <hip/hip_runtime.h>
#include <stdint.h>
#include <stdlib.h>

namespace cy {

#ifndef CY_DEV_KNOBS
#define CY_DEV_KNOBS 0
#endif
inline int env_knob(const char* name, int dflt) { const char* e = getenv(name); return e ? atoi(e) : dflt; }
inline int dev_knob(const char* name, int dflt) { return CY_DEV_KNOBS ? env_knob(name, dflt) : dflt; }

enum Precision { PREC_F16 = 0, PREC_F32 = 1, PREC_F16X3 = 2 };

struct ConvArgs {
    const void* in0; int in0_ct, in0_coff, c0, up0;
    const void* in1; int in1_ct, in1_coff, c1;
    const void* wgt;
    const void* wgt32; uint32_t wgt32_bytes;
    const float* bias;
    void* out; int out_ct, out_coff;
    int out_bs, out_ro;
    int out_f32;
    const void* res; int res_ct, res_coff;
    int B, Hi, Wi, Ho, Wo, Cin, Cout, k, s, act;
    uint32_t in0_bytes, in1_bytes, wgt_bytes;
    int dbg;
    int split, in0_lo, in1_lo, out_lo, res_lo;
    const float* oscale;
    const void* wgt2; uint32_t wgt2_bytes; const float* bias2; int act2, cout2;
    void* out2; int out2_ct, out2_coff;
};

struct StemArgs {
    const void* in; void* out; const float* w; const float* bias;
    const void* wpk;
    int B, Hi, Wi, Ho, Wo, Cout, out_ct, out_coff;
    int out_lo;
};

struct StemDownArgs {
    const void* in; uint32_t in_bytes; int B, Hi, Wi;
    const void* wpk2; const float* bias0;
    const void* wgt32; uint32_t wgt32_bytes; const float* bias1;
    void* out; int out_ct, out_coff;
    int H1, W1, Ho, Wo;
    int dbg;
};

struct BneckArgs {
    const void* in; int in_ct, in_coff; uint32_t in_bytes;
    void* out; int out_ct, out_coff;
    const void* wfrag;
    const float* bias1; const float* bias2;
    int B, H, W, shortcut;
    int dbg;
};
constexpr size_t BNECK_WFRAG_BYTES = 2 * 4 * 18 * 1024;
hipError_t launch_bneck64(const BneckArgs& a, hipStream_t s);
void pack_bneck_weights(const float* W1, const float* W2, void* dst);

struct PoolArgs {
    const void* src; void* dst; int ct, src_coff, dst_coff, C, B, H, W;
    int lo;
};

struct DwArgs {
    const void* in; int in_ct, in_coff; void* out; int out_ct, out_coff; const void* res; int res_ct, res_coff;
    const float* w; const float* bias; int B, H, W, C, act;
    int blk, gstride, goff;
    int in_lo, out_lo, res_lo;
    int xcd;
};
struct AttnArgs {
    const void* qkv; int ct, coff; void* out; int out_ct, out_coff; int B, N, heads, kd, hd; float scale;
    int lo, out_lo;
};
hipError_t launch_dwconv(Precision p, const DwArgs& a, hipStream_t s);
hipError_t launch_attention(Precision p, const AttnArgs& a, hipStream_t s);

hipError_t launch_conv(Precision p, const ConvArgs& a, hipStream_t s);
enum ConvVariant { CONV_GENERIC_128 = 0, CONV_GENERIC_64, CONV_HALO8_128, CONV_PP_64, CONV_C64_PERSIST, CONV_GENERIC_BIG, CONV_WIDE_128, CONV_DIRECT_256, CONV_DIRECT_128, CONV_WIDE_64, CONV_WIDE_DUAL, CONV_STRIP_128, CONV_HEAD_1X1, CONV_NUM_VARIANTS };
int conv_variant(Precision p, const ConvArgs& a);
const char* conv_variant_name(int v);
bool head_pair_ok(Precision p, const ConvArgs& a, const ConvArgs& b);
hipError_t launch_head_pair(Precision p, const ConvArgs& a, const ConvArgs& b, hipStream_t s);
void debug_read_stamps(unsigned long long* out8, bool reset);
void debug_read_wg_stamps(unsigned long long* out, int n);
void debug_read_pre_stamps(unsigned long long* out8, bool reset);
void debug_fastdiv(const double* d_a, const double* d_b, double* d_fast, double* d_ref, int n);
hipError_t launch_stem(Precision p, const StemArgs& a, hipStream_t s);
hipError_t launch_stem_down(const StemDownArgs& a, hipStream_t s);
long stem_down_blocks(const StemDownArgs& a);
bool batch_invariant();
void pack_stem_weights2(const float* W, int cout, void* dst);
hipError_t launch_pool5(Precision p, const PoolArgs& a, hipStream_t s);

size_t packed_weight_bytes(Precision p, int cout, int cin, int k, int chunk_bytes = 128);
void pack_weights(Precision p, const float* W, int cout, int cin, int k, void* dst, int chunk_bytes = 128);
void pack_weights_fused2(const float* W2, int cout2, int cin2, void* dst);
int x3_passes(const float* W, int cout, int cin, int k, const float* scale);
size_t packed_weight_bytes_x3(int cout, int cin, int k, int chunk_bytes = 128, int passes = 3);
void pack_weights_x3(const float* W, int cout, int cin, int k, void* dst, float* oscale, int chunk_bytes = 128, int passes = 3, const float* scale = nullptr);
hipError_t launch_x3_split(const float* in, void* out, long npix, int C, hipStream_t s);
hipError_t launch_x3_merge(const void* in, float* out, long npix, int C, hipStream_t s);
void pack_stem_weights(const float* W, int cout, void* dst);
__device__ __forceinline__ int xcd_contiguous(int bid, int nwg) {
    const int q = nwg >> 3, r = nwg & 7, x = bid & 7;
    return (x < r ? x * (q + 1) : r * (q + 1) + (x - r) * q) + (bid >> 3);
}
__host__ __device__ inline int pad64(int c) { return (c + 63) / 64 * 64; }
__host__ __device__ inline int pad128(int c) { return (c + 127) / 128 * 128; }

struct DecodeArgs {
    const float* pred;
    int B, A, nc;
    int lvl_h[3], lvl_w[3];
    float conf;
    float* cand;
    int* cand_anchor;
    int* cand_count;
    int cap;
};
hipError_t launch_decode(const DecodeArgs& a, hipStream_t s);

struct NmsArgs {
    const float* cand; const int* cand_anchor; const int* cand_count; int cap;
    int B; float iou; int max_det;
    float gain; int padw, padh, w0, h0;
    float* det;
    int* det_anchor;
    int* det_count;
    uint64_t* keys;
    uint64_t* mask;
    int* counters;
};
hipError_t launch_nms(const NmsArgs& a, hipStream_t s);

struct MergeArgs {
    const float* det; const int* det_count; int B, max_det;
    float score_thr; double soft, hard;
    float* out; int* out_count; int* out_src;
    int* err;
    int* counters;
};
hipError_t launch_iou_merge(const MergeArgs& a, hipStream_t s);
hipError_t launch_compact_records(const float* g, long long rows, const long long* perm, int T, int stride, int* hdr, float* out, hipStream_t s);

enum PreOp { OP_BKG = 1, OP_SHIFT = 2, OP_CLIP = 3, OP_ZSCALE = 4, OP_HISTEQ = 5, OP_MINMAX = 6 };
struct PreStage { int op; double p0, p1, p2; int flag; };
constexpr int MAX_STAGES = 8;
constexpr int MAX_PRE_BATCH = 256;
struct PreProgram { int n; PreStage st[MAX_STAGES]; };
struct PreArgs {
    const float* mosaic; int MH, MW;
    int txy[2 * 256];
    int B, th, tw;
    PreProgram prog[3]; int nprog;
    double* params;
    double* histeq;
    int* status;
    void* out; int out_prec; int H, W, top, left;
    double* scratch;
    int new_h, new_w;
    int* counters;
    int variant;
    int fuse01;
};
hipError_t launch_preproc(const PreArgs& a, hipStream_t s);
hipError_t launch_preproc_planes(const PreArgs& a, hipStream_t s);
hipError_t launch_letterbox_pack(const PreArgs& a, hipStream_t s);
hipError_t launch_mosaic_prepare(float* data, size_t n, int big_endian, hipStream_t s);

struct AugView {
    void* out;
    int ch, cw, Hp, Wp;
    int flip;
};
struct AugPackArgs {
    const float* src; int B, H, W;
    AugView v[3]; int nview;
    int out_prec;
};
hipError_t launch_augment_pack(const AugPackArgs& a, hipStream_t s);

struct AugDecodeView {
    const float* pred; int A; int lvl_h[3], lvl_w[3];
    float s; int flip; int lo, hi, off;
};
struct AugDecodeArgs {
    AugDecodeView v[3]; int nview;
    int B, nc; float conf; float W0;
    float* cand; int* cand_anchor; int* cand_count; int cap;
};
hipError_t launch_decode_augmented(const AugDecodeArgs& a, hipStream_t s);

constexpr int MEAS_FIELDS = 12;
struct MeasureArgs {
    const float* img; int MH, MW;
    const int* win;
// ... 23 lines not shown
```

### caesar_yolo_amd/csrc/cy_runtime.hip

```cpp
#include "../../include/caesar_yolo_hip.h"
#include "cy_kernels.h"
#include "cy_plan.h"
#include <algorithm>
#include <cmath>
#include <cstdio>
#include <cstdlib>
#include <cstring>
#include <string>
#include <vector>

using namespace cy;

struct DevConv { void* w = nullptr; float* bias = nullptr; size_t wbytes = 0; float* stem_w = nullptr; void* w32 = nullptr; size_t w32bytes = 0;
                 float* oscale = nullptr;
                 void* w2f = nullptr; size_t w2fbytes = 0;
                 int passes = 3;
                 float* dw_w = nullptr;
                 void* bneck = nullptr; };

struct cy_ctx {
    int device = 0;
    cy_config cfg{};
    Precision prec = PREC_F16;
    std::string err;
    bool loaded = false;
    Plan plan;
    std::vector<std::string> names;
    std::vector<DevConv> dconv;
    char* ws = nullptr; size_t ws_bytes = 0;
    char* ws2 = nullptr; size_t ws2_bytes = 0; hipStream_t s_fwd2 = nullptr; hipEvent_t ev_split[2] = {nullptr, nullptr};
    char* ws3 = nullptr; size_t ws3_bytes = 0; hipStream_t s_small = nullptr;
    std::vector<size_t> toff; std::vector<size_t> tbytes;
    int lastB = 0, lastH = 0, lastW = 0;
    struct StageBufs {
        void* netin = nullptr; float* pred = nullptr;
        float* cand = nullptr; int* cand_anchor = nullptr; int* cand_count = nullptr; uint64_t* keys = nullptr;
        float* det = nullptr; int* det_anchor = nullptr; int* det_count = nullptr; int* merge_err = nullptr; int* out_src = nullptr;
        double* pre_params = nullptr; double* pre_histeq = nullptr; double* pre_scratch = nullptr;
    } sb[3];
    int slot = 0;
    StageBufs& S() { return sb[slot]; }
    struct AugBufs {
        void* view[2] = {nullptr, nullptr}; float* pred[2] = {nullptr, nullptr}; float* src32 = nullptr;
        float* cand = nullptr; int* cand_anchor = nullptr; uint64_t* keys = nullptr;
    } ab[3];
    bool aug = false;
    int acap = 0, acap_pow2 = 0;
    AugBufs& AB() { return ab[slot]; }
    size_t pre_scratch_elems = 0;
    int cap = 0, cap_pow2 = 0;
    hipStream_t s_pre = nullptr, s_post = nullptr;
    hipEvent_t ev_call = nullptr, ev_pre[3] = {nullptr, nullptr, nullptr}, ev_fwd[3] = {nullptr, nullptr, nullptr}, ev_post[3] = {nullptr, nullptr, nullptr};
    unsigned long batches = 0;
    unsigned long small_batches = 0;
    bool mosaic_dirty = true;
    const void* seen_mosaic[16] = {nullptr}; int n_seen = 0;
    int* counters = nullptr;
    double measure_ms = -1.0;
    double islands_ms = -1.0;
    bool profiling = false;
    bool split_last = false;
    bool stem_fused_last = false;
    int pw_fused_conv = -1;
    bool bneck_fused_last = false;
    int prof_stride = 1; unsigned long fwd_calls = 0;
    std::vector<hipEvent_t> ev_pool; size_t ev_used = 0;
    struct ProfRec { size_t e0, e1; int kind; double flops; int conv; int lane; };
    std::vector<ProfRec> prof;
};

namespace {
thread_local std::string g_err;
int fail(cy_ctx* c, int code, const std::string& m) { if (c) c->err = m; g_err = m; return code; }
#define HIPCHK(c, x) do { hipError_t e_ = (x); if (e_ != hipSuccess) return fail(c, CY_ERR_HIP, std::string(#x) + ": " + hipGetErrorString(e_)); } while (0)
inline size_t align_up(size_t v, size_t a) { return (v + a - 1) / a * a; }
inline size_t esize(Precision p) { return p == PREC_F16 ? 2 : 4; }
inline Precision io_prec(Precision p) { return p == PREC_F16X3 ? PREC_F32 : p; }
inline int cand_capacity(int n) { const int r = (n + 63) / 64 * 64; return r > CY_MAX_CAND ? CY_MAX_CAND : r; }
std::vector<float> dw_weights(const float* W, int C) {
    std::vector<float> dw(9 * (size_t)C);
    for (int ch = 0; ch < C; ++ch) for (int t = 0; t < 9; ++t) dw[(size_t)t * C + ch] = W[(size_t)ch * 9 + t];
    return dw;
}
const char* const ATTN_TOO_LARGE = "attention map too large for this kernel (stride-32 map of the input must have <= 10240 pixels)";

struct EntryScratch {
    std::vector<void*> p;
    ~EntryScratch() { for (void* q : p) hipFree(q); }
    hipError_t alloc(size_t bytes, void** out) {
        *out = nullptr;
        const hipError_t e = hipMalloc(out, bytes);
        if (e == hipSuccess) p.push_back(*out);
        return e;
    }
    hipError_t split(const void* t, long npix, int ct, void** out, hipStream_t s) {
        hipError_t e = alloc((size_t)npix * ct * 4, out);
        return e == hipSuccess ? launch_x3_split(reinterpret_cast<const float*>(t), *out, npix, ct, s) : e;
    }
};
int entry_done(cy_ctx* c, hipError_t e, hipStream_t s) {
    const hipError_t e2 = hipStreamSynchronize(s);
    if (e != hipSuccess) return fail(c, CY_ERR_HIP, hipGetErrorString(e));
    if (e2 != hipSuccess) return fail(c, CY_ERR_HIP, hipGetErrorString(e2));
    return CY_OK;
}
inline bool ch8(int v) { return v >= 0 && v % 8 == 0; }

int py_round_half_even(double x) {
    double f = std::floor(x), d = x - f;
    if (d > 0.5) return (int)f + 1;
    if (d < 0.5) return (int)f;
    return (((long)f) % 2 == 0) ? (int)f : (int)f + 1;
}

size_t tensor_elems_per_tile(const Plan& p, int H, int W) {
    size_t t = 0;
    for (auto& x : p.tensors) t += (size_t)(H >> x.level) * (W >> x.level) * x.C;
    return t;
}

void free_all(cy_ctx* c) {
    for (auto e : c->ev_pool) hipEventDestroy(e);
    c->ev_pool.clear(); c->ev_used = 0; c->prof.clear();
    for (auto& d : c->dconv) { if (d.w) hipFree(d.w); if (d.bias) hipFree(d.bias); if (d.stem_w) hipFree(d.stem_w); if (d.w32) hipFree(d.w32); if (d.dw_w) hipFree(d.dw_w); if (d.bneck) hipFree(d.bneck); if (d.oscale) hipFree(d.oscale); if (d.w2f) hipFree(d.w2f); }
    c->dconv.clear();
    if (c->ws) hipFree(c->ws);
    c->ws = nullptr;
    if (c->ws2) hipFree(c->ws2);
    c->ws2 = nullptr; c->ws2_bytes = 0;
    if (c->s_fwd2) { hipStreamDestroy(c->s_fwd2); c->s_fwd2 = nullptr; }
    if (c->ws3) hipFree(c->ws3);
    c->ws3 = nullptr; c->ws3_bytes = 0;
    c->s_small = nullptr;
    for (auto& e : c->ev_split) if (e) { hipEventDestroy(e); e = nullptr; }
    for (auto& b : c->sb) {
        void* ptrs[] = {b.netin, b.pred, b.cand, b.cand_anchor, b.cand_count, b.keys, b.det, b.det_anchor, b.det_count,
                        b.merge_err, b.out_src, b.pre_params, b.pre_histeq, b.pre_scratch};
        for (void* p : ptrs) if (p) hipFree(p);
        b = cy_ctx::StageBufs();
    }
    for (auto& b : c->ab) {
        void* ptrs[] = {b.view[0], b.view[1], b.pred[0], b.pred[1], b.src32, b.cand, b.cand_anchor, b.keys};
        for (void* p : ptrs) if (p) hipFree(p);
        b = cy_ctx::AugBufs();
    }
    c->aug = false; c->acap = 0; c->acap_pow2 = 0;
    if (c->counters) { hipFree(c->counters); c->counters = nullptr; }
    if (c->s_pre) { hipStreamDestroy(c->s_pre); c->s_pre = nullptr; }
    if (c->s_post) { hipStreamDestroy(c->s_post); c->s_post = nullptr; }
    hipEvent_t* evs[] = {&c->ev_call, &c->ev_pre[0], &c->ev_pre[1], &c->ev_pre[2], &c->ev_fwd[0], &c->ev_fwd[1], &c->ev_fwd[2], &c->ev_post[0], &c->ev_post[1], &c->ev_post[2]};
    for (hipEvent_t* e : evs) if (*e) { hipEventDestroy(*e); *e = nullptr; }
    c->batches = 0; c->small_batches = 0;
}

struct Reader {
    const unsigned char* p; size_t n, o = 0; bool bad = false;
    uint32_t u32() { if (o + 4 > n) { bad = true; return 0; } uint32_t v; memcpy(&v, p + o, 4); o += 4; return v; }
    std::string str(uint32_t len) { if (o + len > n) { bad = true; return ""; } std::string s((const char*)p + o, len); o += (len + 3) / 4 * 4; return s; }
    const float* f32(size_t cnt) { if (o + 4 * cnt > n) { bad = true; return nullptr; } const float* r = (const float*)(p + o); o += 4 * cnt; return r; }
};

int parse_plan_v2(cy_ctx* c, Reader& r, Plan* plan, uint32_t* nconv_out, std::vector<std::string>* names, uint32_t* version) {
    *version = r.u32();
    if (*version != 2 && *version != 3) return fail(c, CY_ERR_IO, "unsupported CYW2 version");
    if (r.o + 12 > r.n) return fail(c, CY_ERR_IO, "truncated weight file");
    plan->arch = std::string((const char*)r.p + r.o, strnlen((const char*)r.p + r.o, 8)); r.o += 8;
    plan->scale = (char)r.p[r.o]; r.o += 4;
    const uint32_t nc = r.u32(), nnames = r.u32(), nt = r.u32(), nops = r.u32(), nconv = r.u32();
    for (int l = 0; l < 3; ++l) plan->feat_level[l] = (int)r.u32();
    if (r.bad || nc < 1 || nc > 1000 || nt < 2 || nt > 4096 || nops < 1 || nops > 8192 || nconv < 1 || nconv > 4096)
        return fail(c, CY_ERR_IO, "implausible CYW2 header");
    plan->nc = (int)nc;
    for (uint32_t i = 0; i < nnames; ++i) { uint32_t l = r.u32(); names->push_back(r.str(l)); }
    for (uint32_t i = 0; i < nt; ++i) { const int lev = (int)r.u32(), C = (int)r.u32(); plan->tensors.push_back({lev, C}); }
    for (uint32_t i = 0; i < nops; ++i) {
        int v[20];
        for (int j = 0; j < 20; ++j) v[j] = (int)r.u32();
        Op o{};
        o.kind = (OpKind)v[0]; o.conv = v[1]; o.in0 = v[2]; o.in0_coff = v[3]; o.c0 = v[4]; o.up0 = v[5];
        o.in1 = v[6]; o.in1_coff = v[7]; o.c1 = v[8]; o.out = v[9]; o.out_coff = v[10]; o.res = v[11]; o.res_coff = v[12];
        o.pred_level = v[13]; o.pred_coff = v[14]; o.p0 = v[15]; o.p1 = v[16]; o.p2 = v[17]; o.p3 = v[18];
        auto tok = [&](int t, bool opt) { return (opt && t < 0) || (t >= 0 && t < (int)nt); };
        if (r.bad || v[0] < 0 || v[0] > OPK_ATTN || !tok(o.in0, false) || !tok(o.in1, true) || !tok(o.out, true) || !tok(o.res, true) ||
            (o.kind != OPK_POOL && o.kind != OPK_ATTN && (o.conv < 0 || o.conv >= (int)nconv)) ||
            (o.out < 0 && (o.pred_level < 0 || o.pred_level > 2)))
            return fail(c, CY_ERR_IO, "malformed op in CYW2 plan");
        plan->ops.push_back(o);
    }
    if (r.bad) return fail(c, CY_ERR_IO, "truncated weight file");
    for (auto& t : plan->tensors) if (t.level < 0 || t.level > 5 || t.C < 1 || t.C > 65536) return fail(c, CY_ERR_IO, "malformed tensor in CYW2 plan");
    *nconv_out = nconv;
    plan->ok = true;
    return CY_OK;
}

bool bneck_pair(const Plan& p, size_t i) {
    if (i + 1 >= p.ops.size()) return false;
    const Op& o = p.ops[i]; const Op& n = p.ops[i + 1];
    if (o.kind != OPK_CONV || n.kind != OPK_CONV || o.conv < 0 || n.conv < 0 || o.out < 0 || n.out < 0) return false;
    const ConvDesc& d1 = p.convs[o.conv]; const ConvDesc& d2 = p.convs[n.conv];
    auto c64 = [](const ConvDesc& d) { return d.k == 3 && d.s == 1 && d.cin == 64 && d.cout == 64 && d.act && d.groups == 1; };
    if (!c64(d1) || !c64(d2)) return false;
    if (o.in1 >= 0 || o.up0 || o.res >= 0 || o.c0 != 64 || n.in1 >= 0 || n.up0 || n.c0 != 64) return false;
    if (n.in0 != o.out || n.in0_coff != o.out_coff) return false;
    if (p.tensors[o.in0].level != p.tensors[o.out].level || p.tensors[o.in0].level != p.tensors[n.out].level) return false;
    if (n.res >= 0 && (n.res != o.in0 || n.res_coff != o.in0_coff)) return false;
    if (n.out == o.in0 && n.out_coff == o.in0_coff) return false;
    for (size_t j = i + 2; j < p.ops.size(); ++j) {
        const Op& q = p.ops[j];
        if (q.in0 == o.out || q.in1 == o.out || q.res == o.out) return false;
        if (q.out == o.out) return q.out_coff == o.out_coff && q.conv >= 0 && p.convs[q.conv].cout == 64;
    }
    return true;
}

bool pw_pair(const Plan& p, size_t i) {
    if (i + 1 >= p.ops.size()) return false;
    const Op& o = p.ops[i]; const Op& n = p.ops[i + 1];
    if (o.kind != OPK_CONV || n.kind != OPK_CONV || o.conv < 0 || n.conv < 0 || o.out < 0 || n.out < 0) return false;
    const ConvDesc& d1 = p.convs[o.conv]; const ConvDesc& d2 = p.convs[n.conv];
    if (d1.groups != 1 || d2.groups != 1 || d1.cout != 256 || !d1.act || d1.cin % 64) return false;
    if (!((d1.k == 3 && d1.s == 2 && d1.cin >= 128) || (d1.k == 1 && d1.s == 1))) return false;
    if (d2.k != 1 || d2.s != 1 || d2.cin != 256 || d2.cout > 256 || d2.cout % 16) return false;
    if (o.in1 >= 0 || o.up0 || o.res >= 0 || n.in1 >= 0 || n.up0 || n.res >= 0 || n.c0 != 256) return false;
    if (n.in0 != o.out || n.in0_coff != o.out_coff || p.tensors[o.out].level != p.tensors[n.out].level) return false;
    if (n.out == o.out) return false;
    int readers = 0;
    for (const Op& q : p.ops) readers += (q.in0 == o.out) + (q.in1 == o.out) + (q.res == o.out);
    if (readers != 1) return false;
    for (size_t j = i + 2; j < p.ops.size(); ++j)
        if (p.ops[j].out == o.out) break;
    return true;
}

std::string validate_plan(const Plan& p) {
    auto T = [&](int t) -> const Tensor& { return p.tensors[t]; };
    auto inside = [&](int t, int coff, int n) { return coff >= 0 && n >= 1 && (long)coff + n <= T(t).C; };
    for (size_t i = 0; i < p.ops.size(); ++i) {
        const Op& o = p.ops[i];
        const std::string at = " in op " + std::to_string(i);
        if (o.kind == OPK_POOL) {
            if (o.out < 0 || !inside(o.in0, o.in0_coff, o.c0) || !inside(o.out, o.out_coff, o.c0) || T(o.in0).level != T(o.out).level)
                return "pool slice outside its tensor" + at;
            continue;
        }
        if (o.kind == OPK_ATTN) {
            const long need = (long)o.p0 * (2L * o.p1 + o.p2);
            if (o.out < 0 || o.p0 < 1 || o.p1 < 1 || o.p2 < 1 || need > 65536 || !inside(o.in0, o.in0_coff, (int)need) ||
                (long)o.p0 * o.p2 > 65536 || !inside(o.out, o.out_coff, o.p0 * o.p2))
                return "attention slice outside its tensor" + at;
            continue;
        }
        const ConvDesc& d = p.convs[o.conv];
        if (o.kind == OPK_DWCONV) {
            const int last = d.cout - 1;
            const long cin_last = o.p0 > 0 ? (long)(last / o.p0) * o.p1 + o.p2 + last % o.p0 : last;
            if (o.out < 0 || o.p0 < 0 || o.p1 < 0 || o.p2 < 0 || (o.p0 > 0 && o.p0 % 8) || o.in0_coff < 0 ||
                o.in0_coff + cin_last + 1 > T(o.in0).C || !inside(o.out, o.out_coff, d.cout) ||
                (o.res >= 0 && !inside(o.res, o.res_coff, d.cout)))
                return "depth-wise slice outside its tensor" + at;
            continue;
        }
        if (o.kind == OPK_STEM) {
            if (o.out < 0 || !inside(o.out, o.out_coff, d.cout) || T(o.in0).C != 4 || d.cin != 3) return "malformed stem" + at;
            continue;
        }
        if (!inside(o.in0, o.in0_coff, o.c0) || (o.in1 >= 0 ? !inside(o.in1, o.in1_coff, o.c1) : o.c1 != 0) || o.c0 + o.c1 != d.cin)
            return "conv input slice does not match " + d.name + at;
        if (o.in1 >= 0 && (d.k != 1 || o.c0 % 64)) return "two-segment input needs a 1x1 conv and a 64-aligned boundary" + at;
        if (o.up0 && (d.k != 1 || T(o.in0).level < 1)) return "upsampled input needs a 1x1 conv" + at;
        if (o.out >= 0 && !inside(o.out, o.out_coff, d.cout)) return "conv output slice outside its tensor" + at;
        if (o.out < 0 && (o.pred_coff < 0 || o.pred_coff + d.cout > 64 + p.nc)) return "head slice outside the prediction row" + at;
        if (o.res >= 0 && (!inside(o.res, o.res_coff, d.cout) || (o.out >= 0 && T(o.res).level != T(o.out).level)))
            return "residual slice outside its tensor" + at;
    }
    return "";
}

int upload_weights(cy_ctx* c, const void* buf, size_t nbytes) {
    Reader r{(const unsigned char*)buf, nbytes};
    if (nbytes < 24 || (memcmp(buf, "CYW1", 4) != 0 && memcmp(buf, "CYW2", 4) != 0)) return fail(c, CY_ERR_IO, "not a CYW weight file");
    const bool v2 = memcmp(buf, "CYW2", 4) == 0;
    r.o = 4;
    Plan plan;
    uint32_t nc = 0, nconv = 0, fver = 0;
    std::vector<std::string> names;
    bool has_flags = false;
    if (v2) {
        plan.ok = false;
        int rc = parse_plan_v2(c, r, &plan, &nconv, &names, &fver);
        if (rc) return rc;
        nc = (uint32_t)plan.nc;
        has_flags = fver == 3;
    } else {
        fver = r.u32();
        if (fver != 1 && fver != 2) return fail(c, CY_ERR_IO, "unsupported CYW version");
        has_flags = fver == 2;
        const char scale = (char)r.p[r.o]; r.o += 4;
        nc = r.u32(); nconv = r.u32();
        const uint32_t nnames = r.u32();
        plan = build_plan(scale, (int)nc);
        if (!plan.ok) return fail(c, CY_ERR_UNSUPPORTED, plan.err);
        if (plan.convs.size() != nconv) return fail(c, CY_ERR_IO, "weight file conv count does not match the graph");
        for (uint32_t i = 0; i < nnames; ++i) { uint32_t l = r.u32(); names.push_back(r.str(l)); }
    }
    HIPCHK(c, hipSetDevice(c->device));
    free_all(c);
    c->dconv.resize(nconv);
    std::vector<const float*> Wsrc(nconv, nullptr);
    std::vector<char> packed;
    int stem_conv = -1;
    for (auto& o : plan.ops) if (o.kind == OPK_STEM) stem_conv = o.conv;
    for (uint32_t i = 0; i < nconv; ++i) {
        const uint32_t co = r.u32(), ci = r.u32(), k = r.u32(), s = r.u32(), act = r.u32();
        const uint32_t groups = v2 ? r.u32() : 1u;
        const uint32_t flags = has_flags ? r.u32() : 0u;
        const uint32_t nl = r.u32();
        const std::string name = r.str(nl);
        if (r.bad) return fail(c, CY_ERR_IO, "truncated weight file");
        if (v2) {
            if (co < 1 || ci < 1 || groups < 1 || ci % groups || (k != 1 && k != 3) || (s != 1 && s != 2))
                return fail(c, CY_ERR_IO, "malformed conv header: " + name);
            ConvDesc d; d.name = name; d.cin = (int)ci; d.cout = (int)co; d.k = (int)k; d.s = (int)s; d.act = (int)act; d.groups = (int)groups;
            plan.convs.push_back(d);
        } else {
            const ConvDesc& d = plan.convs[i];
            if (name != d.name || (int)co != d.cout || (int)ci != d.cin || (int)k != d.k || (int)s != d.s || (int)act != d.act)
                return fail(c, CY_ERR_IO, "weight file layer " + name + " does not match graph layer " + d.name);
        }
        const float* W = r.f32((size_t)co * (ci / groups) * k * k);
        const float* b = r.f32(co);
        const float* wscale = (flags & 1u) ? r.f32(co) : nullptr;
        if (r.bad) return fail(c, CY_ERR_IO, "truncated weight file");
        Wsrc[i] = W;
        DevConv& dc = c->dconv[i];
        const int cp = (co + 127) / 128 * 128;
        std::vector<float> bias(cp, 0.0f);
        memcpy(bias.data(), b, 4 * co);
        HIPCHK(c, hipMalloc(&dc.bias, 4 * cp));
        HIPCHK(c, hipMemcpy(dc.bias, bias.data(), 4 * cp, hipMemcpyHostToDevice));
        if (groups > 1) {
            if (groups != ci || co != ci || k != 3 || s != 1 || co % 8) return fail(c, CY_ERR_UNSUPPORTED, "only depth-wise 3x3 stride-1 grouped convs are supported: " + name);
            const std::vector<float> dw = dw_weights(W, (int)co);
            HIPCHK(c, hipMalloc(&dc.dw_w, 4 * dw.size()));
            HIPCHK(c, hipMemcpy(dc.dw_w, dw.data(), 4 * dw.size(), hipMemcpyHostToDevice));
            continue;
        }
        if ((int)i == stem_conv) {
            if (co > 64 || co % 16) return fail(c, CY_ERR_UNSUPPORTED, "stem width not supported by the gfx950 stem kernel");
            std::vector<float> sw(27 * co);
            for (uint32_t o = 0; o < co; ++o) for (int cch = 0; cch < 3; ++cch) for (int t = 0; t < 9; ++t)
                sw[(size_t)(t * 3 + cch) * co + o] = W[((size_t)o * 3 + cch) * 9 + t];
            HIPCHK(c, hipMalloc(&dc.stem_w, 4 * sw.size()));
            HIPCHK(c, hipMemcpy(dc.stem_w, sw.data(), 4 * sw.size(), hipMemcpyHostToDevice));
            if (c->prec == PREC_F16 && co == 64) {
                std::vector<char> pk(64 * 32 * 2 + 64 * 64 * 2);
                pack_stem_weights(W, (int)co, pk.data());
                pack_stem_weights2(W, (int)co, pk.data() + 64 * 32 * 2);
                HIPCHK(c, hipMalloc(&dc.w, pk.size()));
                HIPCHK(c, hipMemcpy(dc.w, pk.data(), pk.size(), hipMemcpyHostToDevice));
            }
            continue;
        }
        if (ci % 8) return fail(c, CY_ERR_UNSUPPORTED, "conv input channels must be a multiple of 8: " + name);
        if (c->prec == PREC_F16X3) {
            std::vector<float> osc(cp);
            dc.passes = env_knob("CY_X3_PASSES", 0) == 3 ? 3 : x3_passes(W, (int)co, (int)ci, (int)k, wscale);
            dc.wbytes = packed_weight_bytes_x3(co, ci, k, 128, dc.passes);
            packed.resize(dc.wbytes);
            pack_weights_x3(W, co, ci, k, packed.data(), osc.data(), 128, dc.passes, wscale);
            HIPCHK(c, hipMalloc(&dc.w, dc.wbytes));
            HIPCHK(c, hipMemcpy(dc.w, packed.data(), dc.wbytes, hipMemcpyHostToDevice));
            HIPCHK(c, hipMalloc(&dc.oscale, 4 * cp));
            HIPCHK(c, hipMemcpy(dc.oscale, osc.data(), 4 * cp, hipMemcpyHostToDevice));
            if (k == 3 && s == 1 && ci % 64 == 0) {
                dc.w32bytes = packed_weight_bytes_x3(co, ci, k, 64, dc.passes);
                packed.resize(dc.w32bytes);
                pack_weights_x3(W, co, ci, k, packed.data(), osc.data(), 64, dc.passes, wscale);
                HIPCHK(c, hipMalloc(&dc.w32, dc.w32bytes));
                HIPCHK(c, hipMemcpy(dc.w32, packed.data(), dc.w32bytes, hipMemcpyHostToDevice));
            }
            continue;
        }
        dc.wbytes = packed_weight_bytes(c->prec, co, ci, k);
        packed.resize(dc.wbytes);
        pack_weights(c->prec, W, co, ci, k, packed.data());
        HIPCHK(c, hipMalloc(&dc.w, dc.wbytes));
        HIPCHK(c, hipMemcpy(dc.w, packed.data(), dc.wbytes, hipMemcpyHostToDevice));
        if (c->prec == PREC_F16 && k == 3 && ((s == 1 && ((ci % 64 == 0 && co >= 33) || (ci == 32 && co <= 64))) || (s == 2 && ci == 64 && co == 128))) {
            dc.w32bytes = packed_weight_bytes(c->prec, co, ci, k, 64);
            packed.resize(dc.w32bytes);
            pack_weights(c->prec, W, co, ci, k, packed.data(), 64);
            HIPCHK(c, hipMalloc(&dc.w32, dc.w32bytes));
            HIPCHK(c, hipMemcpy(dc.w32, packed.data(), dc.w32bytes, hipMemcpyHostToDevice));
        }
    }
    if (v2) {
        const std::string bad = validate_plan(plan);
        if (!bad.empty()) { free_all(c); return fail(c, CY_ERR_IO, "malformed CYW2 plan: " + bad); }
    }
    if (c->prec == PREC_F16) {
        for (size_t i = 0; i + 1 < plan.ops.size(); ++i) {
            if (!pw_pair(plan, i)) continue;
            const int c2 = plan.ops[i + 1].conv;
            const ConvDesc& d2 = plan.convs[c2];
            DevConv& dc2 = c->dconv[c2];
            dc2.w2fbytes = packed_weight_bytes(PREC_F16, d2.cout, d2.cin, 1);
            std::vector<char> pk(dc2.w2fbytes);
            pack_weights_fused2(Wsrc[c2], d2.cout, d2.cin, pk.data());
            HIPCHK(c, hipMalloc(&dc2.w2f, dc2.w2fbytes));
            HIPCHK(c, hipMemcpy(dc2.w2f, pk.data(), dc2.w2fbytes, hipMemcpyHostToDevice));
        }
        std::vector<char> wf(BNECK_WFRAG_BYTES);
        for (size_t i = 0; i + 1 < plan.ops.size(); ++i) {
            if (!bneck_pair(plan, i)) continue;
            const int c1 = plan.ops[i].conv, c2 = plan.ops[i + 1].conv;
            pack_bneck_weights(Wsrc[c1], Wsrc[c2], wf.data());
            HIPCHK(c, hipMalloc(&c->dconv[c1].bneck, wf.size()));
            HIPCHK(c, hipMemcpy(c->dconv[c1].bneck, wf.data(), wf.size(), hipMemcpyHostToDevice));
        }
    }
    c->plan = plan; c->names = names;
    const cy_config& g = c->cfg;
    const size_t es = esize(c->prec);
    size_t act = 0;
    for (auto& t : plan.tensors) act += align_up((size_t)g.max_batch * (g.max_h >> t.level) * (g.max_w >> t.level) * t.C * es, 256);
    c->ws_bytes = act;
    HIPCHK(c, hipMalloc(&c->ws, c->ws_bytes));
    const int A = cy_num_anchors(g.max_h, g.max_w);
    c->cap = cand_capacity(g.max_cand > 0 ? g.max_cand : A);
    c->cap_pow2 = 1; while (c->cap_pow2 < c->cap) c->cap_pow2 <<= 1;
    const size_t Bm = g.max_batch;
    c->pre_scratch_elems = Bm * 3 * (size_t)g.max_h * g.max_w;
    for (auto& b : c->sb) {
        HIPCHK(c, hipMalloc(&b.netin, Bm * g.max_h * g.max_w * 4 * es));
        HIPCHK(c, hipMalloc(&b.pred, Bm * A * (64 + nc) * sizeof(float)));
        HIPCHK(c, hipMalloc(&b.cand, Bm * c->cap * 6 * sizeof(float)));
        HIPCHK(c, hipMalloc(&b.cand_anchor, Bm * c->cap * sizeof(int)));
        HIPCHK(c, hipMalloc(&b.cand_count, Bm * sizeof(int)));
        HIPCHK(c, hipMalloc(&b.keys, Bm * c->cap_pow2 * sizeof(uint64_t)));
        HIPCHK(c, hipMalloc(&b.det, Bm * CY_MAX_DET * 6 * sizeof(float)));
        HIPCHK(c, hipMalloc(&b.det_anchor, Bm * CY_MAX_DET * sizeof(int)));
        HIPCHK(c, hipMalloc(&b.det_count, Bm * sizeof(int)));
        HIPCHK(c, hipMalloc(&b.merge_err, Bm * sizeof(int)));
        HIPCHK(c, hipMalloc(&b.out_src, Bm * CY_MAX_DET * sizeof(int)));
        HIPCHK(c, hipMalloc(&b.pre_params, Bm * 3 * CY_MAX_STAGES * 4 * sizeof(double)));
        HIPCHK(c, hipMalloc(&b.pre_histeq, Bm * 3 * 520 * sizeof(double)));
        HIPCHK(c, hipMalloc(&b.pre_scratch, c->pre_scratch_elems * sizeof(double)));
    }
    HIPCHK(c, hipMalloc(&c->counters, 4 * sizeof(int)));
    HIPCHK(c, hipMemset(c->counters, 0, 4 * sizeof(int)));
    int prio_lo = 0, prio_hi = 0;
    hipDeviceGetStreamPriorityRange(&prio_lo, &prio_hi);
    HIPCHK(c, hipStreamCreateWithPriority(&c->s_pre, hipStreamNonBlocking, prio_lo));
    HIPCHK(c, hipStreamCreateWithPriority(&c->s_post, hipStreamNonBlocking, prio_lo));
    hipEvent_t* evs[] = {&c->ev_call, &c->ev_pre[0], &c->ev_pre[1], &c->ev_pre[2], &c->ev_fwd[0], &c->ev_fwd[1], &c->ev_fwd[2], &c->ev_post[0], &c->ev_post[1], &c->ev_post[2]};
    for (hipEvent_t* e : evs) HIPCHK(c, hipEventCreateWithFlags(e, hipEventDisableTiming));
    c->loaded = true;
    return CY_OK;
}

int layout_tensors(cy_ctx* c, int B, int H, int W, size_t capacity) {
    const size_t es = esize(c->prec);
    c->toff.assign(c->plan.tensors.size(), 0);
    c->tbytes.assign(c->plan.tensors.size(), 0);
    size_t off = 0;
    for (size_t i = 0; i < c->plan.tensors.size(); ++i) {
        const Tensor& t = c->plan.tensors[i];
        const size_t b = (size_t)B * (H >> t.level) * (W >> t.level) * t.C * es;
        c->toff[i] = off; c->tbytes[i] = b;
        off += align_up(b, 256);
        if (b >= 0xFFFFFF00ull) return fail(c, CY_ERR_ARG, "a tensor exceeds the 4 GiB buffer-addressing limit; lower the batch");
    }
    if (off > capacity) return fail(c, CY_ERR_ARG, "batch/shape exceeds the workspace sized at cy_create");
    c->lastB = B; c->lastH = H; c->lastW = W;
    return CY_OK;
}
}

extern "C" {

int cy_create(int device, const cy_config* cfg, cy_ctx** out) {
    if (!cfg || !out) return fail(nullptr, CY_ERR_ARG, "null argument");
    if (cfg->max_batch < 1 || cfg->max_h < 32 || cfg->max_w < 32 || cfg->max_h % 32 || cfg->max_w % 32)
        return fail(nullptr, CY_ERR_ARG, "max_batch >= 1 and max_h/max_w multiples of 32 required");
    if (cfg->precision != CY_F16 && cfg->precision != CY_F32 && cfg->precision != CY_F16X3) return fail(nullptr, CY_ERR_ARG, "bad precision");
    const int A = cy_num_anchors(cfg->max_h, cfg->max_w);
    if (A > CY_MAX_CAND)
        return fail(nullptr, CY_ERR_ARG, "max_h x max_w = " + std::to_string(cfg->max_h) + " x " + std::to_string(cfg->max_w) + ": " +
                                             std::to_string(A) + " anchors, more than CY_MAX_CAND = " + std::to_string(CY_MAX_CAND) +
                                             " (16-bit anchor field of the NMS sort key)");
    if (cfg->max_cand > CY_MAX_CAND)
        return fail(nullptr, CY_ERR_ARG, "max_cand " + std::to_string(cfg->max_cand) + " exceeds CY_MAX_CAND = " + std::to_string(CY_MAX_CAND) +
                                             " (16-bit slot field of the NMS sort key)");
    int n = 0;
    const hipError_t e = hipGetDeviceCount(&n);
    if (e != hipSuccess || device < 0 || device >= n)
        return fail(nullptr, CY_ERR_HIP, std::string("no such HIP device (this library has no CPU fallback): hipGetDeviceCount -> ") +
                                             hipGetErrorString(e) + ", " + std::to_string(n) + " device(s), requested " + std::to_string(device));
    cy_ctx* c = new cy_ctx();
    c->device = device; c->cfg = *cfg; c->prec = cfg->precision == CY_F16 ? PREC_F16 : (cfg->precision == CY_F16X3 ? PREC_F16X3 : PREC_F32);
    *out = c;
    return CY_OK;
}

int cy_destroy(cy_ctx* c) {
    if (!c) return CY_OK;
    hipSetDevice(c->device);
    free_all(c);
    delete c;
    return CY_OK;
}

const char* cy_last_error(const cy_ctx* c) { return c ? c->err.c_str() : g_err.c_str(); }

int cy_load_weights_mem(cy_ctx* c, const void* buf, size_t nbytes) {
    if (!c || !buf) return fail(c, CY_ERR_ARG, "null argument");
    return upload_weights(c, buf, nbytes);
}

int cy_load_weights(cy_ctx* c, const char* path) {
    if (!c || !path) return fail(c, CY_ERR_ARG, "null argument");
    FILE* f = fopen(path, "rb");
    if (!f) return fail(c, CY_ERR_IO, std::string("cannot open ") + path);
    fseek(f, 0, SEEK_END); long n = ftell(f); fseek(f, 0, SEEK_SET);
    std::vector<char> buf(n);
    const size_t got = fread(buf.data(), 1, n, f);
    fclose(f);
    if ((long)got != n) return fail(c, CY_ERR_IO, "short read");
    return upload_weights(c, buf.data(), buf.size());
}

int cy_num_classes(const cy_ctx* c) { return c && c->loaded ? c->plan.nc : -1; }
int cy_weight_passes(const cy_ctx* c, int* out2) {
    if (!c || !c->loaded || !out2) return CY_ERR_ARG;
    out2[0] = out2[1] = 0;
    if (c->prec == PREC_F16X3)
        for (const auto& d : c->dconv) if (d.oscale) out2[d.passes == 2 ? 0 : 1] += 1;
    return CY_OK;
}
const char* cy_class_name(const cy_ctx* c, int i) {
    if (!c || !c->loaded || i < 0 || i >= (int)c->names.size()) return nullptr;
    return c->names[i].c_str();
}

int cy_plan_num_convs(char scale, int nc) { Plan p = build_plan(scale, nc); return p.ok ? (int)p.convs.size() : CY_ERR_ARG; }
int cy_plan_conv_desc(char scale, int nc, int idx, cy_conv_desc* out) {
    Plan p = build_plan(scale, nc);
    if (!p.ok || !out || idx < 0 || idx >= (int)p.convs.size()) return CY_ERR_ARG;
    const ConvDesc& d = p.convs[idx];
    memset(out, 0, sizeof(*out));
    strncpy(out->name, d.name.c_str(), sizeof(out->name) - 1);
    out->cin = d.cin; out->cout = d.cout; out->k = d.k; out->s = d.s; out->act = d.act;
    return CY_OK;
}

int cy_letterbox_geometry(int h0, int w0, int imgsz, cy_letterbox* o) {
    if (!o || h0 < 1 || w0 < 1 || imgsz < 32) return CY_ERR_ARG;
    const double r = std::fmin((double)imgsz / h0, (double)imgsz / w0);
    o->new_w = py_round_half_even(w0 * r); o->new_h = py_round_half_even(h0 * r);
    double dw = (imgsz - o->new_w) % 32, dh = (imgsz - o->new_h) % 32;
    if (dw < 0) dw += 32;
    if (dh < 0) dh += 32;
    dw /= 2; dh /= 2;
    o->top = py_round_half_even(dh - 0.1); o->left = py_round_half_even(dw - 0.1);
    const int bottom = py_round_half_even(dh + 0.1), right = py_round_half_even(dw + 0.1);
    o->H = o->new_h + o->top + bottom; o->W = o->new_w + o->left + right;
    return CY_OK;
}

int cy_num_anchors(int H, int W) { int n = 0; for (int s = 8; s <= 32; s *= 2) n += ((H + s - 1) / s) * ((W + s - 1) / s); return n; }
size_t cy_pred_elems(const cy_ctx* c, int B, int H, int W) {
    return c && c->loaded ? (size_t)B * cy_num_anchors(H, W) * (64 + c->plan.nc) : 0;
}

int cy_mosaic_prepare(cy_ctx* c, float* d_data, size_t n, int big_endian, void* stream) {
    if (!c || !d_data) return fail(c, CY_ERR_ARG, "null argument");
    HIPCHK(c, launch_mosaic_prepare(d_data, n, big_endian, (hipStream_t)stream));
    c->mosaic_dirty = true;
    return CY_OK;
}

static int forward_on(cy_ctx* c, const void* d_netin, int B, int H, int W, float* d_pred, hipStream_t s, char* ws, size_t ws_cap,
                      bool may_profile);

int cy_forward(cy_ctx* c, const void* d_netin, int B, int H, int W, float* d_pred, void* stream) {
    if (!c || !c->loaded) return fail(c, CY_ERR_STATE, "weights not loaded");
    c->split_last = false;
    return forward_on(c, d_netin, B, H, W, d_pred, (hipStream_t)stream, c->ws, c->ws_bytes, true);
}

static int ensure_side_forward_stream(cy_ctx* c) {
    if (c->s_fwd2) return CY_OK;
    HIPCHK(c, hipStreamCreateWithFlags(&c->s_fwd2, hipStreamNonBlocking));
    return CY_OK;
}
static int ensure_second_workspace(cy_ctx* c) {
    if (c->ws2) return CY_OK;
    c->ws2_bytes = c->ws_bytes / 2 + (1u << 20);
    HIPCHK(c, hipMalloc(&c->ws2, c->ws2_bytes));
    int rc = ensure_side_forward_stream(c);
    if (rc) return rc;
    for (auto& ev : c->ev_split) HIPCHK(c, hipEventCreateWithFlags(&ev, hipEventDisableTiming));
    return CY_OK;
}
static int ensure_small_lane(cy_ctx* c) {
    if (c->ws3) return CY_OK;
    c->ws3_bytes = c->ws_bytes / 3 + (1u << 20);
    HIPCHK(c, hipMalloc(&c->ws3, c->ws3_bytes));
    int rc = ensure_side_forward_stream(c);
    if (rc) return rc;
    c->s_small = c->s_fwd2;
    return CY_OK;
}
static int dual_mode() { const char* e = getenv("CY_DUAL_FORWARD"); return e ? atoi(e) : 1; }

static int forward_split(cy_ctx* c, const void* d_netin, int B, int H, int W, float* d_pred, hipStream_t sm) {
    const int mode = dual_mode();
    const bool split = c->prec == PREC_F16 && mode != 0 && B >= 2 && (mode > 1 || (B >= 64 && B < 240));
    c->split_last = split;
    if (!split) return forward_on(c, d_netin, B, H, W, d_pred, sm, c->ws, c->ws_bytes, true);
    int rc0 = ensure_second_workspace(c);
    if (rc0) return rc0;
    const int h = B - B / 2;
    const size_t in_half = (size_t)h * H * W * 4 * esize(c->prec);
    const size_t pred_half = (size_t)h * cy_num_anchors(H, W) * (64 + c->plan.nc);
    HIPCHK(c, hipEventRecord(c->ev_split[0], sm));
    HIPCHK(c, hipStreamWaitEvent(c->s_fwd2, c->ev_split[0], 0));
    int rc = forward_on(c, d_netin, h, H, W, d_pred, sm, c->ws, c->ws_bytes, true);
    if (rc) return rc;
    rc = forward_on(c, (const char*)d_netin + in_half, B - h, H, W, d_pred + pred_half, c->s_fwd2, c->ws2, c->ws2_bytes, false);
    if (rc) return rc;
    HIPCHK(c, hipEventRecord(c->ev_split[1], c->s_fwd2));
    HIPCHK(c, hipStreamWaitEvent(sm, c->ev_split[1], 0));
    return CY_OK;
}

static int forward_on(cy_ctx* c, const void* d_netin, int B, int H, int W, float* d_pred, hipStream_t s, char* ws, size_t ws_cap,
                      bool may_profile) {
    if (!d_netin || !d_pred || B < 1 || H % 32 || W % 32 || H < 32 || W < 32) return fail(c, CY_ERR_ARG, "bad forward arguments");
    int rc = layout_tensors(c, B, H, W, ws_cap);
    if (rc) return rc;
    const Plan& p = c->plan;
    const size_t es = esize(c->prec);
    const bool x3 = c->prec == PREC_F16X3;
    const int cm = x3 ? 2 : 1;
    const int A = cy_num_anchors(H, W);
    int a_off[3], acc = 0;
    for (int l = 0; l < 3; ++l) { a_off[l] = acc; acc += (H >> (3 + l)) * (W >> (3 + l)); }
    auto tptr = [&](int t) -> char* { return t == 0 ? (char*)const_cast<void*>(d_netin) : ws + c->toff[t]; };
    auto stamp = [&]() -> size_t {
        if (c->ev_used == c->ev_pool.size()) { hipEvent_t e; hipEventCreate(&e); c->ev_pool.push_back(e); }
        hipEventRecord(c->ev_pool[c->ev_used], s);
        return c->ev_used++;
    };
    const bool prof_now = may_profile && c->profiling && (c->fwd_calls++ % (unsigned long)c->prof_stride) == 0;
    size_t ev_prev = prof_now ? stamp() : 0;
    int cur_conv = -1;
    auto prof_done = [&](int kind, double flops) {
        if (!prof_now) return;
        const size_t e = stamp();
        c->prof.push_back({ev_prev, e, kind, flops, cur_conv, (c->ws3 && ws == c->ws3) ? 1 : 0});
        ev_prev = e;
    };
    const int fuse_env = getenv("CY_STEM_FUSE") ? atoi(getenv("CY_STEM_FUSE")) : 1;
    auto stem_fusable = [&](const Op& o, const Op& n) -> bool {
        if (c->prec != PREC_F16 || !fuse_env || o.kind != OPK_STEM || n.kind != OPK_CONV || n.conv < 0 || n.out < 0) return false;
        const ConvDesc& d0 = p.convs[o.conv]; const ConvDesc& d = p.convs[n.conv];
        if (d0.cout != 64 || !c->dconv[o.conv].w || !c->dconv[n.conv].w32) return false;
        if (d.k != 3 || d.s != 2 || d.cin != 64 || d.cout != 128 || !d.act) return false;
        if (n.in0 != o.out || n.in0_coff != o.out_coff || n.c0 != 64 || n.in1 >= 0 || n.res >= 0 || n.up0) return false;
        if (p.tensors[o.out].C != 64) return false;
        int readers = 0;
        for (const Op& q : p.ops) readers += (q.in0 == o.out) + (q.in1 == o.out) + (q.res == o.out);
        return readers == 1;
    };
    c->stem_fused_last = false;
    c->pw_fused_conv = -1;
    const int pw_env = env_knob("CY_FUSE_PW", 1);

    struct HeadPend { ConvArgs a; double flops; int conv; bool on; };
    HeadPend pend[3] = {};
    const int bneck_env = env_knob("CY_BNECK_FUSE", 0);
    auto run_op = [&](const Op& o, const Op* next, bool* fused) -> int {
        cur_conv = o.conv;
        if (bneck_env && c->prec == PREC_F16 && o.kind == OPK_CONV && next && c->dconv[o.conv].bneck &&
            bneck_pair(p, (size_t)(&o - p.ops.data()))) {
            const Op& n = *next;
            const Tensor& ti = p.tensors[o.in0]; const Tensor& to = p.tensors[n.out];
            BneckArgs a{};
            a.in = tptr(o.in0); a.in_ct = ti.C; a.in_coff = o.in0_coff;
            a.B = B; a.H = H >> ti.level; a.W = W >> ti.level;
            a.in_bytes = (uint32_t)((size_t)B * a.H * a.W * ti.C * es);
            a.out = tptr(n.out); a.out_ct = to.C; a.out_coff = n.out_coff;
            a.wfrag = c->dconv[o.conv].bneck; a.bias1 = c->dconv[o.conv].bias; a.bias2 = c->dconv[n.conv].bias;
            a.shortcut = n.res >= 0;
            HIPCHK(c, launch_bneck64(a, s));
            prof_done(CONV_NUM_VARIANTS + 4, 2.0 * (2.0 * B * a.H * a.W * 64.0 * 64.0 * 9.0));
            *fused = true; c->bneck_fused_last = true;
            return CY_OK;
        }
        if (o.kind == OPK_STEM && next && stem_fusable(o, *next)) {
            const Op& n = *next;
            const Tensor& ti = p.tensors[o.in0]; const Tensor& t1 = p.tensors[o.out]; const Tensor& to = p.tensors[n.out];
            StemDownArgs a{};
            a.B = B; a.Hi = H >> ti.level; a.Wi = W >> ti.level; a.H1 = H >> t1.level; a.W1 = W >> t1.level;
            a.Ho = a.H1 / 2; a.Wo = a.W1 / 2;
            a.in = tptr(o.in0); a.in_bytes = (uint32_t)((size_t)B * a.Hi * a.Wi * ti.C * es);
            a.wpk2 = reinterpret_cast<const char*>(c->dconv[o.conv].w) + 64 * 32 * 2; a.bias0 = c->dconv[o.conv].bias;
            a.wgt32 = c->dconv[n.conv].w32; a.wgt32_bytes = (uint32_t)c->dconv[n.conv].w32bytes; a.bias1 = c->dconv[n.conv].bias;
            a.out = tptr(n.out); a.out_ct = to.C; a.out_coff = n.out_coff;
            if (ti.C == 4 && (fuse_env > 1 || batch_invariant() || stem_down_blocks(a) >= 256)) {
                HIPCHK(c, launch_stem_down(a, s));
                prof_done(CONV_NUM_VARIANTS, 2.0 * B * a.H1 * a.W1 * 64 * 27.0 + 2.0 * B * a.Ho * a.Wo * 128.0 * 64 * 9);
                *fused = true; c->stem_fused_last = true;
                return CY_OK;
            }
        }
        if (o.kind == OPK_STEM) {
            const Tensor& ti = p.tensors[o.in0]; const Tensor& to = p.tensors[o.out];
            StemArgs a{};
            a.in = tptr(o.in0); a.out = tptr(o.out); a.w = c->dconv[o.conv].stem_w; a.bias = c->dconv[o.conv].bias; a.wpk = c->dconv[o.conv].w;
            a.B = B; a.Hi = H >> ti.level; a.Wi = W >> ti.level; a.Ho = H >> to.level; a.Wo = W >> to.level;
            a.Cout = p.convs[o.conv].cout; a.out_ct = cm * to.C; a.out_coff = o.out_coff; a.out_lo = x3 ? to.C : 0;
            HIPCHK(c, launch_stem(c->prec, a, s));
            prof_done(CONV_NUM_VARIANTS, 2.0 * B * a.Ho * a.Wo * a.Cout * 27.0);
        } else if (o.kind == OPK_POOL) {
            const Tensor& t = p.tensors[o.in0];
            PoolArgs a{};
            a.src = tptr(o.in0); a.dst = tptr(o.out); a.ct = cm * t.C; a.src_coff = o.in0_coff; a.dst_coff = o.out_coff; a.lo = x3 ? t.C : 0;
            a.C = o.c0; a.B = B; a.H = H >> t.level; a.W = W >> t.level;
            HIPCHK(c, launch_pool5(c->prec, a, s));
            prof_done(CONV_NUM_VARIANTS + 1, 0.0);
        } else if (o.kind == OPK_DWCONV) {
            const ConvDesc& d = p.convs[o.conv];
            const Tensor& ti = p.tensors[o.in0]; const Tensor& to = p.tensors[o.out];
            DwArgs a{};
            a.in = tptr(o.in0); a.in_ct = cm * ti.C; a.in_coff = o.in0_coff; a.out = tptr(o.out); a.out_ct = cm * to.C; a.out_coff = o.out_coff;
            a.in_lo = ti.C; a.out_lo = to.C;
            if (o.res >= 0) { a.res = tptr(o.res); a.res_ct = cm * p.tensors[o.res].C; a.res_coff = o.res_coff; a.res_lo = p.tensors[o.res].C; }
            a.w = c->dconv[o.conv].dw_w; a.bias = c->dconv[o.conv].bias;
            a.B = B; a.H = H >> ti.level; a.W = W >> ti.level; a.C = d.cout; a.act = d.act;
            a.blk = o.p0; a.gstride = o.p1; a.goff = o.p2;
            if (!a.w || ti.level != to.level) return fail(c, CY_ERR_STATE, "malformed depth-wise op");
            HIPCHK(c, launch_dwconv(c->prec, a, s));
            prof_done(CONV_NUM_VARIANTS + 2, 2.0 * B * a.H * a.W * (double)a.C * 9.0);
        } else if (o.kind == OPK_ATTN) {
            const Tensor& ti = p.tensors[o.in0]; const Tensor& to = p.tensors[o.out];
            AttnArgs a{};
            a.qkv = tptr(o.in0); a.ct = cm * ti.C; a.coff = o.in0_coff; a.out = tptr(o.out); a.out_ct = cm * to.C; a.out_coff = o.out_coff;
            a.lo = ti.C; a.out_lo = to.C;
            a.B = B; a.N = (H >> ti.level) * (W >> ti.level); a.heads = o.p0; a.kd = o.p1; a.hd = o.p2;
            a.scale = 1.0f / sqrtf((float)a.kd);
            if (a.heads < 1 || ti.level != to.level) return fail(c, CY_ERR_STATE, "malformed attention op");
            hipError_t e = launch_attention(c->prec, a, s);
            if (e == hipErrorInvalidValue) return fail(c, CY_ERR_UNSUPPORTED, ATTN_TOO_LARGE);
            HIPCHK(c, e);
            prof_done(CONV_NUM_VARIANTS + 3, 2.0 * B * a.heads * (double)a.N * a.N * (a.kd + a.hd));
        } else {
            const ConvDesc& d = p.convs[o.conv];
            ConvArgs a{};
            const Tensor& t0 = p.tensors[o.in0];
            auto span = [&](int t) -> uint32_t {
                const Tensor& tt = p.tensors[t];
                return (uint32_t)((size_t)B * (H >> tt.level) * (W >> tt.level) * tt.C * es);
            };
            a.in0 = tptr(o.in0); a.in0_ct = cm * t0.C; a.in0_coff = o.in0_coff; a.c0 = o.c0; a.up0 = o.up0;
            a.in0_bytes = span(o.in0);
            a.split = x3 ? c->dconv[o.conv].passes : 0; a.in0_lo = t0.C; a.oscale = c->dconv[o.conv].oscale;
            int lev_in = o.up0 ? t0.level - 1 : t0.level;
            if (o.in1 >= 0) {
                const Tensor& t1 = p.tensors[o.in1];
                a.in1 = tptr(o.in1); a.in1_ct = cm * t1.C; a.in1_coff = o.in1_coff; a.c1 = o.c1; a.in1_bytes = span(o.in1); a.in1_lo = t1.C;
                lev_in = t1.level;
            }
            a.wgt = c->dconv[o.conv].w; a.wgt_bytes = (uint32_t)c->dconv[o.conv].wbytes; a.bias = c->dconv[o.conv].bias;
            a.wgt32 = c->dconv[o.conv].w32; a.wgt32_bytes = (uint32_t)c->dconv[o.conv].w32bytes;
            a.B = B; a.Hi = H >> lev_in; a.Wi = W >> lev_in; a.k = d.k; a.s = d.s; a.act = d.act;
            a.Ho = d.s == 2 ? a.Hi / 2 : a.Hi; a.Wo = d.s == 2 ? a.Wi / 2 : a.Wi;
            a.Cin = d.cin; a.Cout = d.cout;
            if (o.out >= 0) {
                const Tensor& to = p.tensors[o.out];
                a.out = tptr(o.out); a.out_ct = cm * to.C; a.out_coff = o.out_coff; a.out_bs = a.Ho * a.Wo; a.out_ro = 0; a.out_f32 = 0; a.out_lo = to.C;
            } else {
                a.out = d_pred; a.out_ct = 64 + p.nc; a.out_coff = o.pred_coff; a.out_bs = A; a.out_ro = a_off[o.pred_level]; a.out_f32 = 1;
            }
            if (o.res >= 0) { a.res = tptr(o.res); a.res_ct = cm * p.tensors[o.res].C; a.res_coff = o.res_coff; a.res_lo = p.tensors[o.res].C; }
            double flops = 2.0 * B * a.Ho * a.Wo * (double)a.Cout * a.Cin * a.k * a.k;
            if (pw_env && c->prec == PREC_F16 && next && next->conv >= 0 && c->dconv[next->conv].w2f && conv_variant(c->prec, a) == CONV_DIRECT_256 &&
                pw_pair(p, (size_t)(&o - p.ops.data()))) {
                const Op& n = *next;
                const ConvDesc& d2 = p.convs[n.conv];
                const Tensor& to2 = p.tensors[n.out];
                a.wgt2 = c->dconv[n.conv].w2f; a.wgt2_bytes = (uint32_t)c->dconv[n.conv].w2fbytes; a.bias2 = c->dconv[n.conv].bias;
                a.act2 = d2.act; a.cout2 = d2.cout;
                a.out2 = tptr(n.out); a.out2_ct = to2.C; a.out2_coff = n.out_coff;
                flops += 2.0 * B * a.Ho * a.Wo * (double)d2.cout * d2.cin;
                *fused = true; c->pw_fused_conv = o.conv;
            }
            if (o.out < 0 && o.pred_coff == 0 && c->prec != PREC_F32 && env_knob("CY_HEAD_PAIR", 1) && conv_variant(c->prec, a) == CONV_HEAD_1X1) {
                HeadPend& h = pend[o.pred_level];
                if (h.on) { cur_conv = h.conv; HIPCHK(c, launch_conv(c->prec, h.a, s)); prof_done(conv_variant(c->prec, h.a), h.flops); cur_conv = o.conv; }
                h.a = a; h.flops = flops; h.conv = o.conv; h.on = true;
                return CY_OK;
            }
            if (o.out < 0 && o.pred_coff == 64 && pend[o.pred_level].on) {
                HeadPend& h = pend[o.pred_level];
                h.on = false;
                if (head_pair_ok(c->prec, h.a, a)) {
                    HIPCHK(c, launch_head_pair(c->prec, h.a, a, s));
                    prof_done(CONV_HEAD_1X1, flops + h.flops);
                    return CY_OK;
                }
                cur_conv = h.conv; HIPCHK(c, launch_conv(c->prec, h.a, s)); prof_done(conv_variant(c->prec, h.a), h.flops); cur_conv = o.conv;
            }
            HIPCHK(c, launch_conv(c->prec, a, s));
            prof_done(conv_variant(c->prec, a), flops);
        }
        return CY_OK;
    };
    for (size_t i = 0; i < p.ops.size(); ++i) {
        bool fused = false;
        rc = run_op(p.ops[i], i + 1 < p.ops.size() ? &p.ops[i + 1] : nullptr, &fused);
        if (rc) return rc;
        if (fused) ++i;
    }
    for (HeadPend& h : pend)
        if (h.on) { h.on = false; cur_conv = h.conv; HIPCHK(c, launch_conv(c->prec, h.a, s)); prof_done(conv_variant(c->prec, h.a), h.flops); }
    return CY_OK;
}

int cy_profile_enable(cy_ctx* c, int on) {
    if (!c) return CY_ERR_ARG;
    c->profiling = on != 0;
    c->prof_stride = on > 1 ? on : 1;
    c->fwd_calls = 0;
    c->prof.clear(); c->ev_used = 0;
    return CY_OK;
}

static int profile_summary_lane(cy_ctx* c, cy_prof_entry* out, int cap, int lane);
int cy_profile_summary(cy_ctx* c, cy_prof_entry* out, int cap) { return profile_summary_lane(c, out, cap, -1); }
int cy_profile_summary_lane(cy_ctx* c, cy_prof_entry* out, int cap, int lane) { return profile_summary_lane(c, out, cap, lane); }

static int profile_summary_lane(cy_ctx* c, cy_prof_entry* out, int cap, int lane) {
    const int n = CONV_NUM_VARIANTS + 5;
    if (!c || !out || cap < n) return fail(c, CY_ERR_ARG, "bad arguments");
    HIPCHK(c, hipDeviceSynchronize());
    for (int k = 0; k < n; ++k) {
        memset(&out[k], 0, sizeof(out[k]));
        static const char* const extra[5] = {"stem_kernel", "pool5_kernel", "dwconv3x3_kernel", "attention_kernel",
                                             "bneck64_kernel fused 3x3+3x3 64ch bottleneck, weights in registers"};
        const char* nm = k < CONV_NUM_VARIANTS ? conv_variant_name(k) : extra[k - CONV_NUM_VARIANTS];
        strncpy(out[k].kernel, nm, sizeof(out[k].kernel) - 1);
    }
    for (const auto& r : c->prof) {
        if (lane >= 0 && r.lane != lane) continue;
        float ms = 0.f;
        if (hipEventElapsedTime(&ms, c->ev_pool[r.e0], c->ev_pool[r.e1]) != hipSuccess) continue;
        out[r.kind].ms += ms; out[r.kind].flops += r.flops; out[r.kind].launches += 1;
    }
    return n;
}

int cy_profile_layers(cy_ctx* c, cy_prof_entry* out, int cap) {
    if (!c || !c->loaded || !out) return fail(c, CY_ERR_ARG, "bad arguments");
    const int n = (int)c->plan.convs.size();
    if (cap < n) return fail(c, CY_ERR_ARG, "need one entry per conv");
    HIPCHK(c, hipDeviceSynchronize());
    for (int i = 0; i < n; ++i) { memset(&out[i], 0, sizeof(out[i])); strncpy(out[i].kernel, c->plan.convs[i].name.c_str(), sizeof(out[i].kernel) - 1); }
    for (const auto& r : c->prof) {
        if (r.conv < 0) continue;
        float ms = 0.f;
        if (hipEventElapsedTime(&ms, c->ev_pool[r.e0], c->ev_pool[r.e1]) != hipSuccess) continue;
        out[r.conv].ms += ms; out[r.conv].flops += r.flops; out[r.conv].launches += 1;
    }
    return n;
}

int cy_debug_read_conv(cy_ctx* c, const char* conv_name, float* h_out, size_t cap, int* dims4) {
    if (!c || !c->loaded || !conv_name || !h_out) return fail(c, CY_ERR_ARG, "bad arguments");
    if (c->lastB == 0) return fail(c, CY_ERR_STATE, "no forward has run");
    if (c->split_last) return fail(c, CY_ERR_STATE, "the last batch ran as two half-batches (CY_DUAL_FORWARD=0 keeps it in one workspace)");
    const Plan& p = c->plan;
    for (const Op& o : p.ops) {
        if (o.conv < 0 || p.convs[o.conv].name != conv_name) continue;
        if (o.out < 0) return fail(c, CY_ERR_UNSUPPORTED, "head outputs are read from d_pred");
        if (c->bneck_fused_last && c->dconv[o.conv].bneck && env_knob("CY_BNECK_FUSE", 0))
            return fail(c, CY_ERR_STATE, "this bottleneck ran fused: its cv1 output was not materialised; unset CY_BNECK_FUSE");
        if (o.conv == c->pw_fused_conv && c->pw_fused_conv >= 0 && env_knob("CY_FUSE_PW", 1))
            return fail(c, CY_ERR_STATE, "this layer ran fused with the 1x1 convolution behind it: its output was not materialised; CY_FUSE_PW=0 runs the two layers apart");
        if (o.kind == OPK_STEM && c->stem_fused_last)
            return fail(c, CY_ERR_STATE, "the stem output was not materialised (fused into the next layer's kernel); set CY_STEM_FUSE=0");
        const Tensor& t = p.tensors[o.out];
        const int Ho = c->lastH >> t.level, Wo = c->lastW >> t.level, C = p.convs[o.conv].cout, B = c->lastB;
        const size_t n = (size_t)B * C * Ho * Wo;
        if (n > cap) return fail(c, CY_ERR_ARG, "output buffer too small");
        HIPCHK(c, hipDeviceSynchronize());
        std::vector<char> host(c->tbytes[o.out]);
        HIPCHK(c, hipMemcpy(host.data(), c->ws + c->toff[o.out], host.size(), hipMemcpyDeviceToHost));
        for (int b = 0; b < B; ++b) for (int h = 0; h < Ho; ++h) for (int w = 0; w < Wo; ++w) for (int ch = 0; ch < C; ++ch) {
            const size_t src = (((size_t)b * Ho + h) * Wo + w) * t.C + o.out_coff + ch;
            float v;
            if (c->prec == PREC_F16X3) {
                const _Float16* hp = reinterpret_cast<_Float16*>(host.data()) + (((size_t)b * Ho + h) * Wo + w) * 2 * t.C + o.out_coff + ch;
                v = (float)hp[0] + (float)hp[t.C];
            } else v = c->prec == PREC_F16 ? (float)reinterpret_cast<_Float16*>(host.data())[src]
                                           : reinterpret_cast<float*>(host.data())[src];
            h_out[(((size_t)b * C + ch) * Ho + h) * Wo + w] = v;
        }
        if (dims4) { dims4[0] = B; dims4[1] = C; dims4[2] = Ho; dims4[3] = Wo; }
        return CY_OK;
    }
    return fail(c, CY_ERR_ARG, std::string("no such conv: ") + conv_name);
}

int cy_conv_bn_silu(cy_ctx* c, const void* d_in, int B, int Hi, int Wi, int Cin, const float* h_w, const float* h_b,
                    int Cout, int k, int s, int act, const void* d_res, void* d_out, void* stream) {
    if (!c || !d_in || !h_w || !h_b || !d_out) return fail(c, CY_ERR_ARG, "null argument");
    if ((k != 1 && k != 3) || (s != 1 && s != 2) || Cin % 8 || B < 1) return fail(c, CY_ERR_ARG, "unsupported conv geometry");
    HIPCHK(c, hipSetDevice(c->device));
    if (c->prec == PREC_F16X3) {
        hipStream_t st = (hipStream_t)stream;
        const int pad = k / 2, Ho = (Hi + 2 * pad - k) / s + 1, Wo = (Wi + 2 * pad - k) / s + 1, cp = (Cout + 127) / 128 * 128;
        const size_t nin = (size_t)B * Hi * Wi, nout = (size_t)B * Ho * Wo;
        const int passes = env_knob("CY_X3_PASSES", 0) == 3 ? 3 : x3_passes(h_w, Cout, Cin, k, nullptr);
        const size_t wb = packed_weight_bytes_x3(Cout, Cin, k, 128, passes), wb32 = (k == 3 && s == 1 && Cin % 64 == 0) ? packed_weight_bytes_x3(Cout, Cin, k, 64, passes) : 0;
        std::vector<char> packed(wb), p32(wb32);
        std::vector<float> osc(cp), bias(cp, 0.0f);
        pack_weights_x3(h_w, Cout, Cin, k, packed.data(), osc.data(), 128, passes);
        if (wb32) pack_weights_x3(h_w, Cout, Cin, k, p32.data(), osc.data(), 64, passes);
        memcpy(bias.data(), h_b, 4 * Cout);
        void *dw = nullptr, *dw32 = nullptr, *xin = nullptr, *xres = nullptr, *xout = nullptr; float *db = nullptr, *dsc = nullptr;
        auto cleanup = [&]() { for (void* q : {dw, dw32, xin, xres, xout, (void*)db, (void*)dsc}) if (q) hipFree(q); };
        hipError_t e = hipMalloc(&dw, wb);
        if (e == hipSuccess && wb32) e = hipMalloc(&dw32, wb32);
        if (e == hipSuccess) e = hipMalloc(&db, 4 * cp);
        if (e == hipSuccess) e = hipMalloc(&dsc, 4 * cp);
        if (e == hipSuccess) e = hipMalloc(&xin, nin * Cin * 4);
        if (e == hipSuccess) e = hipMalloc(&xout, nout * Cout * 4);
        if (e == hipSuccess && d_res) e = hipMalloc(&xres, nout * Cout * 4);
        if (e == hipSuccess) e = hipMemcpy(dw, packed.data(), wb, hipMemcpyHostToDevice);
        if (e == hipSuccess && wb32) e = hipMemcpy(dw32, p32.data(), wb32, hipMemcpyHostToDevice);
        if (e == hipSuccess) e = hipMemcpy(db, bias.data(), 4 * cp, hipMemcpyHostToDevice);
        if (e == hipSuccess) e = hipMemcpy(dsc, osc.data(), 4 * cp, hipMemcpyHostToDevice);
        if (e == hipSuccess) e = launch_x3_split(reinterpret_cast<const float*>(d_in), xin, (long)nin, Cin, st);
        if (e == hipSuccess && d_res) e = launch_x3_split(reinterpret_cast<const float*>(d_res), xres, (long)nout, Cout, st);
        if (e == hipSuccess) {
            ConvArgs a{};
            a.in0 = xin; a.in0_ct = 2 * Cin; a.c0 = Cin; a.in0_bytes = (uint32_t)(nin * Cin * 4); a.in0_lo = Cin;
            a.wgt = dw; a.wgt_bytes = (uint32_t)wb; a.bias = db; a.wgt32 = dw32; a.wgt32_bytes = (uint32_t)wb32; a.oscale = dsc; a.split = passes;
            a.B = B; a.Hi = Hi; a.Wi = Wi; a.Ho = Ho; a.Wo = Wo; a.Cin = Cin; a.Cout = Cout; a.k = k; a.s = s; a.act = act;
            a.out = xout; a.out_ct = 2 * Cout; a.out_lo = Cout; a.out_bs = Ho * Wo;
            if (d_res) { a.res = xres; a.res_ct = 2 * Cout; a.res_lo = Cout; }
            e = launch_conv(c->prec, a, st);
        }
        if (e == hipSuccess) e = launch_x3_merge(xout, reinterpret_cast<float*>(d_out), (long)nout, Cout, st);
        const hipError_t e2 = hipStreamSynchronize(st);
        cleanup();
        if (e != hipSuccess) return fail(c, CY_ERR_HIP, hipGetErrorString(e));
        if (e2 != hipSuccess) return fail(c, CY_ERR_HIP, hipGetErrorString(e2));
        return CY_OK;
    }
    const size_t es = esize(c->prec);
    const size_t wb = packed_weight_bytes(c->prec, Cout, Cin, k);
    std::vector<char> packed(wb);
    pack_weights(c->prec, h_w, Cout, Cin, k, packed.data());
    const int cp = (Cout + 127) / 128 * 128;
    std::vector<float> bias(cp, 0.0f);
    memcpy(bias.data(), h_b, 4 * Cout);
    void* dw = nullptr; float* db = nullptr;
    HIPCHK(c, hipMalloc(&dw, wb));
    HIPCHK(c, hipMalloc(&db, 4 * cp));
    HIPCHK(c, hipMemcpy(dw, packed.data(), wb, hipMemcpyHostToDevice));
    HIPCHK(c, hipMemcpy(db, bias.data(), 4 * cp, hipMemcpyHostToDevice));
    void* dw32 = nullptr; size_t wb32 = 0;
    if (c->prec == PREC_F16 && k == 3 && s == 1 && ((Cin % 64 == 0 && Cout >= 33) || (Cin == 32 && Cout <= 64))) {
        wb32 = packed_weight_bytes(c->prec, Cout, Cin, k, 64);
        std::vector<char> p32(wb32);
        pack_weights(c->prec, h_w, Cout, Cin, k, p32.data(), 64);
        HIPCHK(c, hipMalloc(&dw32, wb32));
        HIPCHK(c, hipMemcpy(dw32, p32.data(), wb32, hipMemcpyHostToDevice));
    }
    ConvArgs a{};
    const int pad = k / 2;
    a.in0 = d_in; a.in0_ct = Cin; a.c0 = Cin; a.in0_bytes = (uint32_t)((size_t)B * Hi * Wi * Cin * es);
    a.wgt = dw; a.wgt_bytes = (uint32_t)wb; a.bias = db; a.wgt32 = dw32; a.wgt32_bytes = (uint32_t)wb32;
    a.B = B; a.Hi = Hi; a.Wi = Wi; a.Ho = (Hi + 2 * pad - k) / s + 1; a.Wo = (Wi + 2 * pad - k) / s + 1;
    a.Cin = Cin; a.Cout = Cout; a.k = k; a.s = s; a.act = act;
    a.out = d_out; a.out_ct = Cout; a.out_bs = a.Ho * a.Wo;
    if (d_res) { a.res = d_res; a.res_ct = Cout; }
    hipError_t e = launch_conv(c->prec, a, (hipStream_t)stream);
    hipError_t e2 = hipStreamSynchronize((hipStream_t)stream);
    hipFree(dw); hipFree(db); if (dw32) hipFree(dw32);
    if (e != hipSuccess) return fail(c, CY_ERR_HIP, hipGetErrorString(e));
    if (e2 != hipSuccess) return fail(c, CY_ERR_HIP, hipGetErrorString(e2));
    return CY_OK;
}

int cy_bottleneck64(cy_ctx* c, const void* d_in, int B, int H, int W, const float* h_w1, const float* h_b1, const float* h_w2,
                    const float* h_b2, int shortcut, void* d_out, void* stream) {
    if (!c || !d_in || !h_w1 || !h_b1 || !h_w2 || !h_b2 || !d_out || B < 1 || H < 1 || W < 1) return fail(c, CY_ERR_ARG, "bad arguments");
    if (c->prec != PREC_F16) return fail(c, CY_ERR_UNSUPPORTED, "the fused bottleneck kernel exists in the fp16 context only");
    HIPCHK(c, hipSetDevice(c->device));
    std::vector<char> wf(BNECK_WFRAG_BYTES);
    pack_bneck_weights(h_w1, h_w2, wf.data());
    void* dw = nullptr; float* db = nullptr;
    HIPCHK(c, hipMalloc(&dw, wf.size()));
    HIPCHK(c, hipMalloc(&db, 128 * sizeof(float)));
    HIPCHK(c, hipMemcpy(dw, wf.data(), wf.size(), hipMemcpyHostToDevice));
    HIPCHK(c, hipMemcpy(db, h_b1, 64 * sizeof(float), hipMemcpyHostToDevice));
    HIPCHK(c, hipMemcpy(db + 64, h_b2, 64 * sizeof(float), hipMemcpyHostToDevice));
    BneckArgs a{};
    a.in = d_in; a.in_ct = 64; a.in_coff = 0; a.in_bytes = (uint32_t)((size_t)B * H * W * 64 * 2);
    a.out = d_out; a.out_ct = 64; a.out_coff = 0; a.wfrag = dw; a.bias1 = db; a.bias2 = db + 64;
    a.B = B; a.H = H; a.W = W; a.shortcut = shortcut != 0;
    hipError_t e = launch_bneck64(a, (hipStream_t)stream);
    hipError_t e2 = hipStreamSynchronize((hipStream_t)stream);
    hipFree(dw); hipFree(db);
    if (e != hipSuccess) return fail(c, CY_ERR_HIP, hipGetErrorString(e));
    if (e2 != hipSuccess) return fail(c, CY_ERR_HIP, hipGetErrorString(e2));
    return CY_OK;
}

int cy_dwconv3x3(cy_ctx* c, const void* d_in, int B, int H, int W, int C, int in_ct, int in_coff, const float* h_w, const float* h_b,
                 int act, int blk, int gstride, int goff, const void* d_res, int res_ct, int res_coff, void* d_out, int out_ct,
                 int out_coff, void* stream) {
    if (!c || !d_in || !h_w || !h_b || !d_out) return fail(c, CY_ERR_ARG, "null argument");
    if (B < 1 || H < 1 || W < 1 || C < 8 || C % 8 || blk < 0) return fail(c, CY_ERR_ARG, "unsupported depth-wise geometry");
    const int last = blk ? ((C - 1) / blk) * gstride + goff + (C - 1) % blk : C - 1;
    if (!ch8(in_ct) || !ch8(in_coff) || !ch8(out_ct) || !ch8(out_coff) || !ch8(blk) || (blk && (!ch8(gstride) || !ch8(goff))) ||
        in_coff + last >= in_ct || out_coff + C > out_ct || (d_res && (!ch8(res_ct) || !ch8(res_coff) || res_coff + C > res_ct)))
        return fail(c, CY_ERR_ARG, "channel slice outside its tensor, or an offset / stride not a multiple of 8");
    if (d_out == d_in || d_out == d_res) return fail(c, CY_ERR_ARG, "the output must not alias the input or the residual");
    HIPCHK(c, hipSetDevice(c->device));
    hipStream_t st = (hipStream_t)stream;
    const bool x3 = c->prec == PREC_F16X3;
    const int cm = x3 ? 2 : 1;
    const long npix = (long)B * H * W;
    const std::vector<float> dw = dw_weights(h_w, C);
    EntryScratch sc;
    void *wd = nullptr, *bd = nullptr, *in = const_cast<void*>(d_in), *res = const_cast<void*>(d_res), *out = d_out;
    hipError_t e = sc.alloc(4 * dw.size(), &wd);
    if (e == hipSuccess) e = sc.alloc(4 * (size_t)C, &bd);
    if (e == hipSuccess) e = hipMemcpy(wd, dw.data(), 4 * dw.size(), hipMemcpyHostToDevice);
    if (e == hipSuccess) e = hipMemcpy(bd, h_b, 4 * (size_t)C, hipMemcpyHostToDevice);
    if (e == hipSuccess && x3) e = sc.split(d_in, npix, in_ct, &in, st);
    if (e == hipSuccess && x3 && d_res) e = sc.split(d_res, npix, res_ct, &res, st);
    if (e == hipSuccess && x3) e = sc.split(d_out, npix, out_ct, &out, st);
    if (e == hipSuccess) {
        DwArgs a{};
        a.in = in; a.in_ct = cm * in_ct; a.in_coff = in_coff; a.out = out; a.out_ct = cm * out_ct; a.out_coff = out_coff;
        a.in_lo = in_ct; a.out_lo = out_ct;
        if (d_res) { a.res = res; a.res_ct = cm * res_ct; a.res_coff = res_coff; a.res_lo = res_ct; }
        a.w = reinterpret_cast<const float*>(wd); a.bias = reinterpret_cast<const float*>(bd);
        a.B = B; a.H = H; a.W = W; a.C = C; a.act = act != 0;
        a.blk = blk; a.gstride = gstride; a.goff = goff;
        e = launch_dwconv(c->prec, a, st);
    }
    if (e == hipSuccess && x3) e = launch_x3_merge(out, reinterpret_cast<float*>(d_out), npix, out_ct, st);
    return entry_done(c, e, st);
}

int cy_attention(cy_ctx* c, const void* d_qkv, int B, int N, int ct, int coff, int heads, int kd, int hd, void* d_out, int out_ct,
                 int out_coff, void* stream) {
    if (!c || !d_qkv || !d_out) return fail(c, CY_ERR_ARG, "null argument");
    if (B < 1 || N < 1 || heads < 1 || kd < 1 || kd > 64 || hd < 1) return fail(c, CY_ERR_ARG, "unsupported attention geometry");
    if (coff < 0 || coff + heads * (2 * kd + hd) > ct || out_coff < 0 || out_coff + heads * hd > out_ct)
        return fail(c, CY_ERR_ARG, "channel slice outside its tensor");
    if (d_out == d_qkv) return fail(c, CY_ERR_ARG, "the output must not alias the input");
    HIPCHK(c, hipSetDevice(c->device));
    hipStream_t st = (hipStream_t)stream;
    const bool x3 = c->prec == PREC_F16X3;
    const int cm = x3 ? 2 : 1;
    const long npix = (long)B * N;
    EntryScratch sc;
    void *qkv = const_cast<void*>(d_qkv), *out = d_out;
    hipError_t e = hipSuccess;
    if (x3) e = sc.split(d_qkv, npix, ct, &qkv, st);
    if (e == hipSuccess && x3) e = sc.split(d_out, npix, out_ct, &out, st);
    if (e == hipSuccess) {
        AttnArgs a{};
        a.qkv = qkv; a.ct = cm * ct; a.coff = coff; a.out = out; a.out_ct = cm * out_ct; a.out_coff = out_coff;
        a.lo = ct; a.out_lo = out_ct;
        a.B = B; a.N = N; a.heads = heads; a.kd = kd; a.hd = hd;
        a.scale = 1.0f / sqrtf((float)a.kd);
        e = launch_attention(c->prec, a, st);
        if (e == hipErrorInvalidValue) {
            entry_done(c, hipSuccess, st);
            return fail(c, CY_ERR_UNSUPPORTED, ATTN_TOO_LARGE);
        }
    }
    if (e == hipSuccess && x3) e = launch_x3_merge(out, reinterpret_cast<float*>(d_out), npix, out_ct, st);
    return entry_done(c, e, st);
}

int cy_maxpool5(cy_ctx* c, const void* d_src, int B, int H, int W, int C, int ct, int src_coff, void* d_dst, int dst_coff,
                void* stream) {
    if (!c || !d_src || !d_dst) return fail(c, CY_ERR_ARG, "null argument");
    if (B < 1 || H < 1 || W < 1 || C < 8 || C % 8) return fail(c, CY_ERR_ARG, "unsupported pool geometry");
    if (!ch8(ct) || !ch8(src_coff) || !ch8(dst_coff) || src_coff + C > ct || dst_coff + C > ct)
        return fail(c, CY_ERR_ARG, "channel slice outside its tensor, or an offset / stride not a multiple of 8");
    if (d_src == d_dst && src_coff < dst_coff + C && dst_coff < src_coff + C) return fail(c, CY_ERR_ARG, "overlapping source and destination slices");
    HIPCHK(c, hipSetDevice(c->device));
    hipStream_t st = (hipStream_t)stream;
    const bool x3 = c->prec == PREC_F16X3;
    const int cm = x3 ? 2 : 1;
    const long npix = (long)B * H * W;
    EntryScratch sc;
    void *src = const_cast<void*>(d_src), *dst = d_dst;
    hipError_t e = hipSuccess;
    if (x3) e = sc.split(d_dst, npix, ct, &dst, st);
    if (e == hipSuccess && x3) { if (d_src == d_dst) src = dst; else e = sc.split(d_src, npix, ct, &src, st); }
    if (e == hipSuccess) {
        PoolArgs a{};
        a.src = src; a.dst = dst; a.ct = cm * ct; a.src_coff = src_coff; a.dst_coff = dst_coff; a.lo = x3 ? ct : 0;
        a.C = C; a.B = B; a.H = H; a.W = W;
        e = launch_pool5(c->prec, a, st);
    }
    if (e == hipSuccess && x3) e = launch_x3_merge(dst, reinterpret_cast<float*>(d_dst), npix, ct, st);
    return entry_done(c, e, st);
}

int cy_debug_stamps(unsigned long long* out8, int reset) {
    if (!out8) return CY_ERR_ARG;
    if (reset < 0) { debug_read_wg_stamps(out8, -reset); return CY_OK; }
    if (reset >= 2) debug_read_pre_stamps(out8, reset == 3);
    else debug_read_stamps(out8, reset != 0);
    return CY_OK;
}

int cy_debug_fastdiv(const double* d_a, const double* d_b, double* d_fast, double* d_ref, int n) {
    if (!d_a || !d_b || !d_fast || !d_ref || n < 1) return CY_ERR_ARG;
    debug_fastdiv(d_a, d_b, d_fast, d_ref, n);
    return hipGetLastError() == hipSuccess ? CY_OK : CY_ERR_HIP;
}

int cy_debug_cand_counts(cy_ctx* c, int* h_out, int B) {
    if (!c || !c->loaded || !h_out || B < 1 || B > c->cfg.max_batch) return fail(c, CY_ERR_ARG, "bad arguments");
    HIPCHK(c, hipDeviceSynchronize());
    HIPCHK(c, hipMemcpy(h_out, c->S().cand_count, (size_t)B * sizeof(int), hipMemcpyDeviceToHost));
    return CY_OK;
}

int cy_preproc_params(cy_ctx* c, double* h_out, int B) {
// ... 559 lines not shown
```

Baseline: 9143.

## Replace static patch striding with atomic work-stealing tile claims in persistent conv kernels

The persistent conv kernels (c64, widep, stem_down2) now take their next tile from a global atomic counter instead of a fixed blockIdx + n*gridDim stride. Each launch gets its own claim slot, zeroed per forward pass with a memset. Ticket values are passed between wave groups through LDS so the next patch can be prefetched. The goal is to even out load imbalance across workgroups, especially on the tail, at the cost of extra atomics, barriers and memsets, and new ordering hazards.

```diff
diff --git a/caesar_yolo_amd/csrc/conv_igemm.hip b/caesar_yolo_amd/csrc/conv_igemm.hip
--- a/caesar_yolo_amd/csrc/conv_igemm.hip
+++ b/caesar_yolo_amd/csrc/conv_igemm.hip
@@ -1131,6 +1131,7 @@
     auto swz = [](int chunk, int row) { return KC == 64 ? (chunk ^ (row & 7)) : (chunk ^ (((row >> 2) & 1) << 1)); };
     constexpr int P_BYTES = (NWI + 1) * 1024;
     extern __shared__ __attribute__((aligned(16))) char smem[];
+    __shared__ volatile int tk[2];
     typedef __attribute__((address_space(3))) void lds_void;
     const int tid = threadIdx.x, lane = tid & 63;
     const int wave = __builtin_amdgcn_readfirstlane(tid >> 6);
@@ -1139,6 +1140,8 @@
     const int H = a.Hi, W = a.Wi;
     const int tiles_x = (W + TW - 1) / TW, tiles_y = (H + TH - 1) / TH;
     const int npatch = a.B * tiles_y * tiles_x;
+    int tkt = 0;
+    if (tid == 256) tkt = atomicAdd(a.claim, 1);
     const unsigned bias_bytes = (unsigned)((W + 1) * a.in0_ct) * 2u;
     const auto rs0 = __builtin_amdgcn_make_buffer_rsrc(const_cast<char*>(reinterpret_cast<const char*>(a.in0)) - bias_bytes, 0,
                                                        a.in0_bytes + 2 * bias_bytes, 0x00020000);
@@ -1197,8 +1200,11 @@
         }
     };
 
-    const int NP = (int)blockIdx.x < npatch ? (npatch - 1 - (int)blockIdx.x) / (int)gridDim.x + 1 : 0;
-    if (grp < NP) dma_patch(blockIdx.x + grp * gridDim.x);
+    if (tid == 256) tk[1] = (int)gridDim.x + tkt;
+    asm volatile("s_waitcnt lgkmcnt(0)" ::: "memory");
+    __builtin_amdgcn_s_barrier();
+    int p_prev = -1, p_cur = blockIdx.x, p_next = __builtin_amdgcn_readfirstlane(tk[1]);
+    if (grp == 0 ? p_cur < npatch : p_next < npatch) dma_patch(grp == 0 ? p_cur : p_next);
     __builtin_amdgcn_s_waitcnt(0x0F70);
     __builtin_amdgcn_s_barrier();
 
@@ -1211,9 +1217,10 @@
     f32x4 acc[NI][4];
     const bool vec_out = cbase + 16 <= a.Cout;
     const int out_lane = fr * a.out_ct + cbase, res_lane = fr * a.res_ct + cbase;
-    for (int ph = 0; ph <= NP; ++ph) {
+    for (int ph = 0;; ++ph) {
+        const bool live = p_cur < npatch;
         if ((ph & 1) == grp) {
-            if (ph < NP) {
+            if (live) {
 #pragma unroll
                 for (int ni = 0; ni < NI; ++ni)
 #pragma unroll
@@ -1245,8 +1252,9 @@
                 asm volatile("s_waitcnt lgkmcnt(0)" ::: "memory");
             }
         } else if (ph >= 1) {
+            if (live && wm == 0 && lane == 0) tkt = atomicAdd(a.claim, 1);
             f16x8 rres[4][2];
-            const int pidx = blockIdx.x + (ph - 1) * gridDim.x;
+            const int pidx = p_prev;
             const int tx = pidx % tiles_x, ty = (pidx / tiles_x) % tiles_y, b = pidx / (tiles_x * tiles_y);
             const int yw = ty * TH + wm * 4, x = tx * TW + fr;
             const long rowpix = ((long)b * H + yw) * W + tx * TW;
@@ -1260,7 +1268,7 @@
                     rres[mi][1] = *reinterpret_cast<const f16x8*>(rp + 8);
                 }
             }
-            if (ph + 1 < NP) dma_patch(blockIdx.x + (ph + 1) * gridDim.x);
+            if (p_next < npatch) dma_patch(p_next);
             if (ACT) {
 #pragma unroll
                 for (int ni = 0; ni < NI; ++ni)
@@ -1315,10 +1323,16 @@
                 }
             }
             CY_WAIT_VM(0);
-        }
+            if (live && wm == 0 && lane == 0) tk[ph & 1] = (int)gridDim.x + tkt;
+        } else if (wm == 0 && lane == 0) {
+            tk[0] = (int)gridDim.x + atomicAdd(a.claim, 1);
+        }
+        asm volatile("s_waitcnt lgkmcnt(0)" ::: "memory");
         __builtin_amdgcn_sched_barrier(0);
         __builtin_amdgcn_s_barrier();
         __builtin_amdgcn_sched_barrier(0);
+        if (!live) break;
+        p_prev = p_cur; p_cur = p_next; p_next = __builtin_amdgcn_readfirstlane(tk[ph & 1]);
     }
 }
 
@@ -1334,6 +1348,7 @@
         hipFuncSetAttribute(reinterpret_cast<const void*>(conv3x3_c64_kernel<KC, false, true>), hipFuncAttributeMaxDynamicSharedMemorySize, (int)lds);
         attr_set = true;
     }
+    if (!a.claim) return hipErrorInvalidValue;
     const int npatch = a.B * ((a.Hi + 15) / 16) * ((a.Wi + 15) / 16);
     const int grid = npatch < 256 ? npatch : 256;
     if (a.act && a.res) hipLaunchKernelGGL((conv3x3_c64_kernel<KC, true, true>), dim3(grid), dim3(512), lds, s, a);
@@ -1933,6 +1948,7 @@
         }
     };
     float* const bias_lds = reinterpret_cast<float*>(smem + 2 * P_BYTES + RING * W_BYTES);
+    volatile int* const tk_lds = reinterpret_cast<volatile int*>(smem + 2 * P_BYTES + RING * W_BYTES + 4096);
     auto dma_bias = [&](int slot, int n0) {
         if (wave != 0) return;
         dma_piece(rsb, (lds_ptr_t*)(bias_lds + slot * 512), lane * 16 < BN * 4 ? (unsigned)(n0 * 4 + lane * 16) : CY_OOB, 0);
@@ -2019,8 +2035,9 @@
 #pragma unroll 1
     for (;;) {
         const int b = pb_, y0 = py0, x0 = px0, n0 = pn0;
-        const int vn = v + (int)gridDim.x;
-        const bool next = vn < total;
+        if (wave == 7 && lane == 63) woff = (unsigned)atomicAdd(a.claim, 1);
+        int vn = 0;
+        bool next = false;
         if (stamps) {
             const unsigned long long t = stamp_real();
             if (n == 2 && tid == 0) {
@@ -2037,9 +2054,10 @@
 #pragma unroll 1
         for (int cp = 0; cp < pairs; ++cp) {
             const bool more = cp + 1 < pairs;
-            const bool chain = more || next;
 #pragma unroll
             for (int st = 0; st < NST; ++st) {
+                if (st == 1 && !more) { vn = (int)gridDim.x + __builtin_amdgcn_readfirstlane(*tk_lds); next = vn < total; }
+                const bool chain = more || next;
                 const bool has_w = st + 2 < NST || chain;
                 if (st + 2 < NST) dma_stage((st + 2) % 3, 2 * cp, 2 * (st + 2), n0);
                 else if (more) dma_stage((st + 2) % 3, 2 * cp + 2, 2 * (st + 2 - NST), n0);
@@ -2049,6 +2067,7 @@
                 if (st == 5 && more) dma_patch(0, 2 * cp + 2, b, y0, x0);
                 if (st == 5 && !more && next) dma_patch(0, 0, pb_, py0, px0);
                 stage_compute(st);
+                if (st == 0 && !more && wave == 7 && lane == 63) *tk_lds = (int)woff;
                 asm volatile("s_waitcnt lgkmcnt(0)" ::: "memory");
                 if (st == 0 || st == 1) { CY_WAIT_VM(WPS + PROUNDS); }
                 else if (st == 5 || st == 6) { if (chain) { CY_WAIT_VM(WPS + PROUNDS); } else { CY_WAIT_VM(WPS); } }
@@ -2178,7 +2197,8 @@
 template <int STRIP, bool SPLIT = false>
 static hipError_t launch_widep_t(const ConvArgs& a, hipStream_t s, int total, const StripGeo& sg) {
     constexpr int PR = 18 * 34, NPC = (PR + 15) / 16, PROUNDS = STRIP ? STRIP : (NPC + 3) / 4;
-    const size_t lds = 2 * PROUNDS * 4 * 1024 + 3 * 2 * 128 * 64 + 4096;
+    const size_t lds = 2 * PROUNDS * 4 * 1024 + 3 * 2 * 128 * 64 + 4096 + 16;
+    if (!a.claim) return hipErrorInvalidValue;
     static bool attr_set = false;
     if (!attr_set) {
         hipFuncSetAttribute(reinterpret_cast<const void*>(conv3x3_widep_kernel<SPLIT, false, STRIP>), hipFuncAttributeMaxDynamicSharedMemorySize, (int)lds);
@@ -3252,13 +3272,13 @@
 
 __global__ __launch_bounds__(512) void stem_down2_kernel(const StemDownArgs a) {
     extern __shared__ __attribute__((aligned(16))) char smem[];
+    __shared__ volatile int tk[4];
     const int tid = threadIdx.x, lane = tid & 63, fr = lane & 15, fq = lane >> 4;
     const int wave = __builtin_amdgcn_readfirstlane(tid >> 6);
     const int grp = wave >> 2, w4 = wave & 3, wn = w4 & 1, wm = w4 >> 1;
     char* const buf = smem + grp * S2_BUF;
     const int tiles_x = (a.Wo + S2_TW - 1) / S2_TW, tiles_y = (a.Ho + S2_TH - 1) / S2_TH;
     const int npatch = a.B * tiles_y * tiles_x;
-    const int NP = (int)blockIdx.x < npatch ? (npatch - 1 - (int)blockIdx.x) / (int)gridDim.x + 1 : 0;
     const auto rsi = __builtin_amdgcn_make_buffer_rsrc(const_cast<void*>(a.in), 0, a.in_bytes, 0x00020000);
     const auto rsw = __builtin_amdgcn_make_buffer_rsrc(const_cast<void*>(a.wgt32), 0, a.wgt32_bytes, 0x00020000);
 
@@ -3275,13 +3295,16 @@
     const int dh0 = t0 / 3 - 1, dw0 = t0 % 3 - 1, dh1 = t1 / 3 - 1, dw1 = t1 % 3 - 1;
     const int d0 = (dh0 * a.Wi + dw0) * 8, d1 = (dh1 * a.Wi + dw1) * 8, d2 = (a.Wi + 1) * 8;
 
-    auto coords = [&](int n, int& b, int& oy0, int& ox0) {
-        int id = (int)blockIdx.x + n * (int)gridDim.x;
+    auto coords = [&](int id, int& b, int& oy0, int& ox0) {
         const int tx = id % tiles_x; id /= tiles_x;
         oy0 = (id % tiles_y) * S2_TH; ox0 = tx * S2_TW; b = id / tiles_y;
     };
 
-    auto fill = [&](int n) {
+    const int G = (int)gridDim.x;
+    const bool claimer = w4 == 0 && lane == 0;
+    auto fill = [&](int n, int k) {
+        int tkt = 0;
+        if (claimer) tkt = atomicAdd(a.claim, k == 0 ? 2 : 1);
         int b, oy0, ox0;
         coords(n, b, oy0, ox0);
         const int sy0 = 2 * oy0 - 1, sx0 = 2 * ox0 - 1;
@@ -3312,6 +3335,10 @@
             q1[gi] = load_b64(rsi, ok1 ? (unsigned)(base + d1) : CY_OOB);
             q2[gi] = load_b64(rsi, (inmap && fq == 0) ? (unsigned)(base + d2) : CY_OOB);
         }
+        if (claimer) {
+            if (k == 0) { tk[1] = G + tkt; tk[2] = G + tkt + 1; }
+            else tk[(k + 2) & 3] = G + tkt;
+        }
 #pragma unroll
         for (int gi = 0; gi < NG; ++gi) {
             const int g = gi * 4 + w4, p = g * 16 + fr;
@@ -3403,14 +3430,18 @@
         __builtin_amdgcn_sched_barrier(0);
     };
     if (grp) phase_barrier();
+    int k = grp;
+    int id = grp ? __builtin_amdgcn_readfirstlane(tk[1]) : (int)blockIdx.x;
 #pragma unroll 1
-    for (int n = grp; n < NP; n += 2) {
-        fill(n);
+    while (id < npatch) {
+        fill(id, k);
         phase_barrier();
-        conv_store(n);
+        conv_store(id);
         phase_barrier();
-    }
-    if (((NP + grp) & 1) == 0) phase_barrier();
+        k += 2;
+        id = __builtin_amdgcn_readfirstlane(tk[k & 3]);
+    }
+    if (k == 0 || (k == 1 ? (int)blockIdx.x : __builtin_amdgcn_readfirstlane(tk[(k - 1) & 3])) < npatch) phase_barrier();
 }
 
 long stem_down_blocks(const StemDownArgs& a) {
@@ -3430,6 +3461,7 @@
     if (v == 2 || (v == 0 && np >= 512)) {
         static bool set2 = false;
         if (!set2) { hipFuncSetAttribute(reinterpret_cast<const void*>(stem_down2_kernel), hipFuncAttributeMaxDynamicSharedMemorySize, S2_LDS); set2 = true; }
+        if (!a.claim) return hipErrorInvalidValue;
         hipLaunchKernelGGL(stem_down2_kernel, dim3((unsigned)(np < 256 ? np : 256)), dim3(512), S2_LDS, s, b2);
         return hipGetLastError();
     }
diff --git a/caesar_yolo_amd/csrc/cy_kernels.h b/caesar_yolo_amd/csrc/cy_kernels.h
--- a/caesar_yolo_amd/csrc/cy_kernels.h
+++ b/caesar_yolo_amd/csrc/cy_kernels.h
@@ -30,6 +30,7 @@
     const float* oscale;
     const void* wgt2; uint32_t wgt2_bytes; const float* bias2; int act2, cout2;
     void* out2; int out2_ct, out2_coff;
+    int* claim;
 };
 
 struct StemArgs {
@@ -46,6 +47,7 @@
     void* out; int out_ct, out_coff;
     int H1, W1, Ho, Wo;
     int dbg;
+    int* claim;
 };
 
 struct BneckArgs {
diff --git a/caesar_yolo_amd/csrc/cy_runtime.hip b/caesar_yolo_amd/csrc/cy_runtime.hip
--- a/caesar_yolo_amd/csrc/cy_runtime.hip
+++ b/caesar_yolo_amd/csrc/cy_runtime.hip
@@ -56,6 +56,7 @@
     bool mosaic_dirty = true;
     const void* seen_mosaic[16] = {nullptr}; int n_seen = 0;
     int* counters = nullptr;
+    int* claim = nullptr; int claim_n = 0;
     double measure_ms = -1.0;
     double islands_ms = -1.0;
     bool profiling = false;
@@ -146,11 +147,21 @@
     }
     c->aug = false; c->acap = 0; c->acap_pow2 = 0;
     if (c->counters) { hipFree(c->counters); c->counters = nullptr; }
+    if (c->claim) { hipFree(c->claim); c->claim = nullptr; c->claim_n = 0; }
     if (c->s_pre) { hipStreamDestroy(c->s_pre); c->s_pre = nullptr; }
     if (c->s_post) { hipStreamDestroy(c->s_post); c->s_post = nullptr; }
     hipEvent_t* evs[] = {&c->ev_call, &c->ev_pre[0], &c->ev_pre[1], &c->ev_pre[2], &c->ev_fwd[0], &c->ev_fwd[1], &c->ev_fwd[2], &c->ev_post[0], &c->ev_post[1], &c->ev_post[2]};
     for (hipEvent_t* e : evs) if (*e) { hipEventDestroy(*e); *e = nullptr; }
     c->batches = 0; c->small_batches = 0;
+}
+
+int ensure_claim(cy_ctx* c, int n) {
+    if (c->claim && c->claim_n >= n) return CY_OK;
+    if (c->claim) { HIPCHK(c, hipFree(c->claim)); c->claim = nullptr; }
+    c->claim_n = (int)align_up((size_t)n, 64);
+    HIPCHK(c, hipMalloc(&c->claim, 4 * (size_t)c->claim_n * sizeof(int)));
+    HIPCHK(c, hipMemset(c->claim, 0, 4 * (size_t)c->claim_n * sizeof(int)));
+    return CY_OK;
 }
 
 struct Reader {
@@ -450,6 +461,8 @@
     }
     HIPCHK(c, hipMalloc(&c->counters, 4 * sizeof(int)));
     HIPCHK(c, hipMemset(c->counters, 0, 4 * sizeof(int)));
+    int rc_claim = ensure_claim(c, (int)plan.ops.size() + 1);
+    if (rc_claim) return rc_claim;
     int prio_lo = 0, prio_hi = 0;
     hipDeviceGetStreamPriorityRange(&prio_lo, &prio_hi);
     HIPCHK(c, hipStreamCreateWithPriority(&c->s_pre, hipStreamNonBlocking, prio_lo));
@@ -677,6 +690,9 @@
     };
     c->stem_fused_last = false;
     c->pw_fused_conv = -1;
+    int* const claim_blk = c->claim + (size_t)(ws == c->ws ? 0 : ws == c->ws2 ? 1 : 2) * c->claim_n;
+    int claim_used = 0;
+    HIPCHK(c, hipMemsetAsync(claim_blk, 0, (size_t)c->claim_n * sizeof(int), s));
     const int pw_env = env_knob("CY_FUSE_PW", 1);
 
     struct HeadPend { ConvArgs a; double flops; int conv; bool on; };
@@ -710,6 +726,7 @@
             a.wpk2 = reinterpret_cast<const char*>(c->dconv[o.conv].w) + 64 * 32 * 2; a.bias0 = c->dconv[o.conv].bias;
             a.wgt32 = c->dconv[n.conv].w32; a.wgt32_bytes = (uint32_t)c->dconv[n.conv].w32bytes; a.bias1 = c->dconv[n.conv].bias;
             a.out = tptr(n.out); a.out_ct = to.C; a.out_coff = n.out_coff;
+            a.claim = claim_blk + claim_used++;
             if (ti.C == 4 && (fuse_env > 1 || batch_invariant() || stem_down_blocks(a) >= 256)) {
                 HIPCHK(c, launch_stem_down(a, s));
                 prof_done(CONV_NUM_VARIANTS, 2.0 * B * a.H1 * a.W1 * 64 * 27.0 + 2.0 * B * a.Ho * a.Wo * 128.0 * 64 * 9);
@@ -786,6 +803,7 @@
                 a.out = d_pred; a.out_ct = 64 + p.nc; a.out_coff = o.pred_coff; a.out_bs = A; a.out_ro = a_off[o.pred_level]; a.out_f32 = 1;
             }
             if (o.res >= 0) { a.res = tptr(o.res); a.res_ct = cm * p.tensors[o.res].C; a.res_coff = o.res_coff; a.res_lo = p.tensors[o.res].C; }
+            a.claim = claim_blk + claim_used++;
             double flops = 2.0 * B * a.Ho * a.Wo * (double)a.Cout * a.Cin * a.k * a.k;
             if (pw_env && c->prec == PREC_F16 && next && next->conv >= 0 && c->dconv[next->conv].w2f && conv_variant(c->prec, a) == CONV_DIRECT_256 &&
                 pw_pair(p, (size_t)(&o - p.ops.data()))) {
@@ -920,6 +938,7 @@
     if (!c || !d_in || !h_w || !h_b || !d_out) return fail(c, CY_ERR_ARG, "null argument");
     if ((k != 1 && k != 3) || (s != 1 && s != 2) || Cin % 8 || B < 1) return fail(c, CY_ERR_ARG, "unsupported conv geometry");
     HIPCHK(c, hipSetDevice(c->device));
+    { const int rc = ensure_claim(c, 1); if (rc) return rc; }
     if (c->prec == PREC_F16X3) {
         hipStream_t st = (hipStream_t)stream;
         const int pad = k / 2, Ho = (Hi + 2 * pad - k) / s + 1, Wo = (Wi + 2 * pad - k) / s + 1, cp = (Cout + 127) / 128 * 128;
@@ -953,7 +972,9 @@
             a.B = B; a.Hi = Hi; a.Wi = Wi; a.Ho = Ho; a.Wo = Wo; a.Cin = Cin; a.Cout = Cout; a.k = k; a.s = s; a.act = act;
             a.out = xout; a.out_ct = 2 * Cout; a.out_lo = Cout; a.out_bs = Ho * Wo;
             if (d_res) { a.res = xres; a.res_ct = 2 * Cout; a.res_lo = Cout; }
-            e = launch_conv(c->prec, a, st);
+            a.claim = c->claim + 3 * (size_t)c->claim_n;
+            e = hipMemsetAsync(a.claim, 0, sizeof(int), st);
+            if (e == hipSuccess) e = launch_conv(c->prec, a, st);
         }
         if (e == hipSuccess) e = launch_x3_merge(xout, reinterpret_cast<float*>(d_out), (long)nout, Cout, st);
         const hipError_t e2 = hipStreamSynchronize(st);
@@ -990,7 +1011,9 @@
     a.Cin = Cin; a.Cout = Cout; a.k = k; a.s = s; a.act = act;
     a.out = d_out; a.out_ct = Cout; a.out_bs = a.Ho * a.Wo;
     if (d_res) { a.res = d_res; a.res_ct = Cout; }
-    hipError_t e = launch_conv(c->prec, a, (hipStream_t)stream);
+    a.claim = c->claim + 3 * (size_t)c->claim_n;
+    hipError_t e = hipMemsetAsync(a.claim, 0, sizeof(int), (hipStream_t)stream);
+    if (e == hipSuccess) e = launch_conv(c->prec, a, (hipStream_t)stream);
     hipError_t e2 = hipStreamSynchronize((hipStream_t)stream);
     hipFree(dw); hipFree(db); if (dw32) hipFree(dw32);
     if (e != hipSuccess) return fail(c, CY_ERR_HIP, hipGetErrorString(e));
```

After: 9138. No clear change (-0.1%).
